# Stability-AI/stable-audio-tools

Hardware: AMD Instinct MI355X
Metric: train-step samples/sec (47s@44.1kHz) (higher is better)
Workload: dtype f32(bf16x3)

## Files before the change

### include/sat_amd.h

```cpp
#ifndef SAT_AMD_H
#define SAT_AMD_H

#ifdef __cplusplus
extern "C" {
#endif

int sat_abi_version(void);
int sat_is_simulator(void);
const char* sat_last_error(void);


int sat_conv1d(const float* x, const float* w_packed, const float* bias, const float* alpha, const float* beta,
               const float* res, float* y, const float* x2, const float* alpha2, const float* beta2,
               float* part_da, float* part_db, int B, int Cin, int Cout, int Tin, int Tout, int K, int stride,
               int dil, int pad, int tanh_out, void* stream);
int sat_conv1d_partial_rows(int B, int Tout);

int sat_conv1d_bf16x3(const float* x, const short* w_hi, const short* w_lo, const float* bias, const float* snake_a,
                      const float* snake_ib, const float* res, float* y, const float* x2, const float* alpha2,
                      const float* beta2, float* part_da, float* part_db, int B, int Cin, int Cout, int Tin, int Tout,
                      int K, int stride, int dil, int pad, int tanh_out, void* stream);
int sat_conv1d_bf16x3_emit(const float* x, const short* w_hi, const short* w_lo, const float* bias, const float* snake_a,
                      const float* snake_ib, const float* res, float* y, const float* x2, const float* alpha2,
                      const float* beta2, float* part_da, float* part_db, int B, int Cin, int Cout, int Tin, int Tout,
                      int K, int stride, int dil, int pad, int tanh_out, void* em_hi, void* em_lo,
                           const float* em_a, const float* em_ib, int em_rows, void* stream);
int sat_residual_unit_fwd(const short* xp_hi, const short* xp_lo, int rows, const short* w7_hi, const short* w7_lo,
                          const float* bias1, const float* a2, const float* ib2, const short* w1_hi, const short* w1_lo,
                          const float* bias2, const float* x, float* h, float* y, int B, int C, int T, int K, int dil, int pad,
                          void* em_hi, void* em_lo, const float* em_a, const float* em_ib, int em_rows, void* stream);
int sat_convtr1d_bf16x3(const float* x, const short* w_hi, const short* w_lo, const float* bias, const float* snake_a,
                        const float* snake_ib, const float* res, float* y, const float* x2, const float* alpha2,
                        const float* beta2, float* part_da, float* part_db, int B, int Cin, int Cout, int Tin, int Tout,
                        int K, int stride, int pad, int tanh_out, void* stream);
int sat_conv1d_bf16x3_partial_rows(int B, int Tout, int K, int stride);

int sat_rows_pack(const float* x, float* buf, int B, int C, int T, int W, int kh, int dil_t, int pad_t, int pad_w, int pitch, int lead,
                  void* stream);
int sat_rows_pack_bwd(const float* dbuf, float* dx, int B, int C, int T, int W, int kh, int dil_t, int pad_t, int pad_w, int pitch,
                      int lead, void* stream);
int sat_rows_unpack(const float* y, float* out, int B, int C, int T, int W, int pad_w, int pitch, float slope, void* stream);
int sat_rows_unpack_bwd(const float* dout, const float* out, float* dy, int B, int C, int T, int W, int pad_w, int pitch, float slope,
                        void* stream);

int sat_disc_geom(int frames, int W, int* P, int* L, int* lead, int* rows);
int sat_disc_planes(const float* src, const float* out, const signed char* fm_sign, const float* fm_coef, float* dst, void* hi, void* lo, int B,
                    int C, int frames, int W, int pitched, float slope, void* stream);
int sat_disc_l1_blocks(void);
int sat_disc_l1_sum(const float* a, const float* b, float* partial, signed char* sign, long long n, void* stream);
long long sat_disc_pack_size(int Cout, int Cin, int kh, int kw, int mode);
int sat_disc_pack_weights(const float* w, short* wq, int Cout, int Cin, int kh, int kw, int mode, void* stream);
int sat_disc_conv(const void* xp_hi, const void* xp_lo, const void* wq, const float* bias, float* y, void* em_hi,
                  void* em_lo, int B, int Cin, int Cout, int frames, int W, int kh, int kw, int dil_t, float slope, const float* lk_src,
                  float lk_slope, void* stream);
int sat_disc_wgrad_nsplit(int B, int M, int Cin, int kh, int frames, int W);
int sat_disc_wgrad(const float* dy, const float* x, float* partial, int B, int M, int Cin, int frames, int W, int kh, int kw, int dil_t,
                   void* stream);

int sat_conv1d_k7_plane_rows(int Tin, int Tout, int pad);
int sat_conv1d_k7_planes(const float* x, const float* snake_a, const float* snake_ib, short* xp_hi, short* xp_lo, int B, int Cin, int Tin,
                         int rows, void* stream);
long long sat_pack_weights_k7q_size(int D0, int D1, int K, int mode);
int sat_pack_weights_k7q(const float* w, short* hi, short* lo, int D0, int D1, int K, int mode, void* stream);
int sat_conv1d_bf16x3_planesq(const short* xp_hi, const short* xp_lo, int rows, const short* w_hi, const short* w_lo, const float* bias,
                             const float* res, float* y, const float* x2, const float* alpha2, const float* beta2, float* part_da,
                             float* part_db, int B, int Cin, int Cout, int Tin, int Tout, int K, int dil, int pad, int tanh_out,
                             int flags, void* stream);
int sat_convtr1d_bf16x3_partial_rows(int B, int Tout, int stride, int pad);
int sat_pack_weights_bf16x3(const float* w, short* hi, short* lo, int D0, int D1, int K, int stride, int mode, void* stream);
long long sat_pack_weights_bf16x3_size(int D0, int D1, int K, int stride, int mode);
int sat_snake_consts(const float* alpha, const float* beta, float* a, float* ib, int C, void* stream);

int sat_convtr1d(const float* x, const float* w_packed, const float* bias, const float* alpha, const float* beta,
                 const float* res, float* y, const float* x2, const float* alpha2, const float* beta2,
                 float* part_da, float* part_db, int B, int Cin, int Cout, int Tin, int Tout, int K, int stride,
                 int pad, int tanh_out, void* stream);
int sat_convtr1d_partial_rows(int B, int Tout, int stride, int pad);

int sat_conv_wgrad(const float* lo, const float* hi, const float* alpha, const float* beta, int snake_on,
                   float* partial, long long so_m, long long so_n, long long so_k, int B, int M, int N, int Tlo,
                   int Thi, int K, int stride, int dil, int pad, void* stream);
int sat_conv_wgrad_nsplit(int B, int M, int N, int Tlo, int K, int stride, int dil);

int sat_conv_wgrad7_bf16x3(const float* dy, const float* x, const float* alpha, const float* beta, float* partial,
                           long long so_m, long long so_n, long long so_k, int B, int M, int N, int T, int dil, int pad,
                           float* dy_rowsum, void* stream);
int sat_conv_wgrad7_bf16x3_nsplit(int B, int M, int N, int T);
int sat_conv_wgrad7_bf16x3_fuses_rowsum(int B, int M, int N, int T);

int sat_conv_wgrad7_planes_ok(int B, int M, int N, int T, int dil, int pad, int rows_dy, int rows_act);
int sat_conv_wgrad7_planes_nsplit(int B, int M, int N, int T);
int sat_conv_wgrad7_planes(const short* dy_hi, const short* dy_lo, int rows_dy, const short* act_hi, const short* act_lo, int rows_act,
                           float* partial, long long so_m, long long so_n, long long so_k, int B, int M, int N, int T, int dil, int pad,
                           void* stream);
int sat_lds_read_tr16_probe(const short* image, const int* lane_off, short* out, void* stream);

int sat_conv_wgrad_bf16x3(const float* lo, const float* hi, const float* alpha, const float* beta, int snake_on,
                          float* partial, long long so_m, long long so_n, long long so_k, int B, int M, int N, int Tlo,
                          int Thi, int K, int stride, int pad, float* lo_rowsum, void* stream);
int sat_conv_wgrad_bf16x3_nsplit(int B, int M, int N, int Tlo, int K, int stride);

int sat_ru_k1_bwd_nsplit(int B, int C, int T);
int sat_ru_k1_pack(const float* w, short* hi, short* lo, int C, void* stream);
int sat_ru_k1_bwd(const float* dy, const float* h, const short* wt_hi, const short* wt_lo, const float* alpha2, const float* beta2,
                  float* dh, short* em_hi, short* em_lo, int em_rows, float* dw_partial, float* part, int B, int C, int T,
                  void* stream);

int sat_reduce_splits(const float* partial, float* out, long long count, int nsplit, float scale, int accumulate,
                      void* stream);
int sat_rowsum(const float* x, float* partial, int B, int C, int T, void* stream);
int sat_rowsum_nsplit(int T);

int sat_wn_fold(const float* v, const float* g, float* w, float* norm, int D0, int R, void* stream);
int sat_wn_grad(const float* v, const float* g, const float* norm, const float* dw, float* dv, float* dg, int D0,
                int R, void* stream);
int sat_wn_grad_splits(const float* partial, int nsplit, long long count, long long so_m, long long so_n, long long so_k,
                       const float* v, const float* g, const float* norm, float* dv, float* dg, int D0, int N, int K,
                       const float* bias_partial, int bias_cols, float* dbias, void* stream);
int sat_edge_conv_ok(int cin, int cout, int k, int stride, int dil, int pad);
int sat_edge_conv_partial_rows(int B, int T);
int sat_edge_conv(const float* x, const float* w, const float* bias, const float* alpha, const float* beta, float* y, const float* x2,
                  const float* alpha2, const float* beta2, float* part_da, float* part_db, short* em_hi, short* em_lo,
                  const float* em_alpha, const float* em_beta, int em_rows, int B, int Cin, int Cout, int T, int K, int pad, int mode,
                  int tanh_out, void* stream);
int sat_edge_conv_wgrad_nsplit(int B, int M, int N, int T);
int sat_edge_conv_wgrad(const float* dy, const float* x, const float* alpha, const float* beta, float* partial, float* rowsum, int B,
                        int M, int N, int T, int K, int pad, void* stream);
int sat_pack_weights(const float* w, float* out, int D0, int D1, int K, int S, int mode, void* stream);

int sat_vae_nblocks(long long n);
int sat_vae_sample_fwd(const float* pre, const float* noise, float* z, float* kl_partial, int B, int C, int T,
                       void* stream);
int sat_vae_sample_bwd(const float* pre, const float* noise, const float* dz, const float* dkl, float* dpre, int B,
                       int C, int T, void* stream);

int sat_fir(const float* x, const float* taps, float* y, int N, int T, int ntaps, int adjoint, void* stream);
int sat_stft_tiles(int n_fft, int hop, int T);
int sat_stft_fwd(const float* x, const float* y, const float* views, float* partial, int NI, int C, int T, int NV,
                 int n_fft, int hop, void* stream);
int sat_stft_bwd(const float* x, const float* y, const float* views, const float* coef, float* dy, int NI, int C,
                 int T, int NV, int n_fft, int hop, int wrt_x, void* stream);

int sat_adamw_step(float* p, const float* g, float* m, float* v, long long n, float lr, float beta1, float beta2,
                   float eps, float weight_decay, int step, float grad_scale, float* ema, float ema_decay,
                   void* stream);
int sat_adamw_step_dev(float* p, const float* g, float* m, float* v, long long n, const float* hyper, float beta1, float beta2,
                       float eps, float weight_decay, float* ema, void* stream);

int sat_multi_copy(const void* entries, int nent, void* stream);

int sat_allreduce_available(void);
int sat_allreduce_unique_id(void* id128);
int sat_allreduce_init(const void* id128, int world, int rank, void** comm);
int sat_allreduce_bucket(void* comm, void* buf, long long count, int dtype, int mode, void* stream);
int sat_allreduce_finalize(void* comm);

int sat_attn_prepare(const void* src, long long sb, long long sh, long long sn, short* rm_hi, short* rm_lo,
                     short* tr_hi, short* tr_lo, int B, int H, int N, int Np, int dtype, void* stream);
int sat_attention_fwd(const short* q_hi, const short* q_lo, const short* k_hi, const short* k_lo, const short* vt_hi,
                      const short* vt_lo, void* o, float* lse, int B, int H, int Hkv, int Nq, int Nk, int Nqp, int Nkp,
                      int head_dim, float scale, int dtype, void* stream);
int sat_attention_rowdot(const void* dout, const void* out, float* dsum, int B, int H, int Nq, int dtype, void* stream);
int sat_attention_bwd(const short* const* planes, const float* lse, const float* dsum, void* dq, void* dk, void* dv,
                      int B, int H, int Hkv, int Nq, int Nk, int Nqp, int Nkp, int head_dim, float scale, int dtype,
                      void* stream);
int sat_attention_cross_ok(int H, int Hkv, int Nk, int head_dim, int dtype);
int sat_attention_cross_fwd(const short* q_rm, const short* k_rm, const short* v_tr, void* o, float* lse, int B, int H, int Hkv,
                            int Nq, int Nk, int Nqp, int Nkp, int head_dim, float scale, void* stream);
long long sat_attention_cross_bwd_ws(int B, int H, int Hkv, int Nq, int Nk);
int sat_attention_cross_bwd(const short* const* planes, const float* lse, const float* dsum, void* dq, void* dk, void* dv,
                            void* ws, long long ws_bytes, int B, int H, int Hkv, int Nq, int Nk, int Nqp, int Nkp, int head_dim,
                            float scale, void* stream);

int sat_layernorm_fwd(const void* x, const float* gamma, const float* beta, const void* scale, const void* shift,
                      long long mod_stride, void* y, float* mean, float* rstd, int rows, int D, int rows_per_batch,
                      float eps, int dtype, void* stream);
int sat_layernorm_fwd_fp8(const void* x, const float* gamma, const float* beta, const void* scale, const void* shift,
                          long long mod_stride, void* q, float* qscale, int rows, int D, int rows_per_batch, float eps,
                          int dtype, void* stream);
int sat_layernorm_bwd_nblocks(int rows, int rows_per_batch);
int sat_layernorm_bwd(const void* dy, const void* x, const float* gamma, const float* beta, const void* scale,
                      long long mod_stride, const float* mean, const float* rstd, void* dx, float* part, int rows, int D,
                      int rows_per_batch, int dtype, void* stream);
int sat_layernorm_bwd_res(const void* dy, const void* x, const float* gamma, const float* beta, const void* scale,
                          long long mod_stride, const float* mean, const float* rstd, const void* dres, void* dx, float* part,
                          int rows, int D, int rows_per_batch, int dtype, void* stream);

int sat_rope_tables(const float* inv_freq, float* cs, int N, int half, float pos_scale, void* stream);
int sat_rope_apply(void* t, const float* cs, long long sb, long long sn, long long sh, int B, int N, int H, int half,
                   int tab_off, int transpose, int dtype, void* stream);

int sat_qk_norm_fwd(const void* x, long long xs, void* y, long long ys, const float* q_gamma, const float* q_beta,
                    const float* k_gamma, const float* k_beta, const float* cs, int tab_off, float* stat, int tokens, int ntok,
                    int nh, int hq, int mode, float eps, int dtype, void* stream);
int sat_qk_norm_bwd_nblocks(long long rows);
int sat_qk_norm_bwd(void* dy, long long ys, const void* x, long long xs, const float* q_gamma, const float* k_gamma,
                    const float* cs, int tab_off, const float* stat, float* part, int tokens, int ntok, int nh, int hq,
                    int mode, int dtype, void* stream);

int sat_swiglu(const void* xin, const void* dout, void* out, long long rows, int F, int backward, int dtype,
               void* stream);
int sat_gate_residual(const void* x, const void* gate, long long gstride, const void* res, void* y, int B, int N, int D,
                      int dtype, void* stream);
int sat_gate_residual_bwd_nchunks(int N);
int sat_gate_residual_bwd(const void* dy, const void* x, const void* gate, long long gstride, void* dx, float* part,
                          int B, int N, int D, int dtype, void* stream);

int sat_cfg_step(const void* out2, const void* x, void* y0, void* y1, int B, int C, int T, int ncond, float scale,
                 float phi, float c0x, float c0v, float c1x, float c1v, int dtype, void* stream);
int sat_sampler_step(const void* out2, const void* x, const void* prev, void* y0, void* y1, int B, int C, int T, int ncond,
                     float scale, float phi, const float* coef, int dtype, void* stream);
int sat_sampler_step_dev(const void* out2, const void* x, const void* prev, void* y0, void* y1, int B, int C, int T, int ncond,
                         float scale, float phi, const float* coef, int dtype, void* stream);
int sat_spec_frames(int n_fft, int hop, int T);
int sat_spec_fwd(const float* x, float* z, int NI, int C, int T, int n_fft, int hop, void* stream);
int sat_spec_bwd(const float* dz, float* dx, int NI, int C, int T, int n_fft, int hop, void* stream);


int sat_gemm_bf16(const void* A, long long lda, const void* B, long long ldb, void* C, long long ldc, const float* bias,
                  const void* res, long long ldr, const void* gate, long long ldg, int rows_per_gate, void* pre,
                  long long ldp, const void* zeros, int M, int N, int K, int epilogue, int out_f32, int splits, int tile,
                  void* stream);

int sat_gemm_qkv_bf16(const void* A, long long lda, const void* B, long long ldb, const float* rope_cs, int rope_off,
                      void* q_rm, void* k_rm, void* v_tr, const void* zeros, int nb, int ntok, int npad, int heads,
                      int K, int sec0, int nsec, int tile, void* stream);
int sat_gemm_qkv_norm_bf16(const void* A, long long lda, const void* B, long long ldb, const float* rope_cs, int rope_off,
                           void* q_rm, void* k_rm, void* v_tr, const void* zeros, int nb, int ntok, int npad, int heads,
                           int K, int sec0, int nsec, int tile, int mode, const float* q_gamma, const float* q_beta,
                           const float* k_gamma, const float* k_beta, float eps, void* stream);

int sat_splitk_epilogue(const float* slabs, int S, const float* bias, const void* res, long long ldr, void* out, long long ldo,
                        int M, int N, int out_f32, void* stream);

int sat_gemm_fp8(const void* A, long long lda, const void* B, long long ldb, void* C, long long ldc, const float* bias,
                 const void* res, long long ldr, const void* gate, long long ldg, int rows_per_gate, void* pre,
                 long long ldp, const void* zeros, const float* alpha, const float* row_alpha, const float* col_alpha, int M, int N,
                 int K, int epilogue, int out_f32, int tile, void* stream);
int sat_gemm_qkv_fp8(const void* A, long long lda, const void* B, long long ldb, const float* rope_cs, int rope_off,
                     void* q_rm, void* k_rm, void* v_tr, const void* zeros, const float* alpha, const float* row_alpha,
                     const float* col_alpha, int nb, int ntok, int npad, int heads, int K, int sec0, int nsec, int tile, void* stream);
int sat_absmax_scale_blocks(int R, int C);
int sat_absmax_scale(const void* src, long long lds, float* work, float* scales, int R, int C, int src_f32, void* stream);
int sat_quant_fp8(const void* src, long long lds, void* dst, long long ldd, const float* qscale, int R, int C, int src_f32,
                  void* stream);
int sat_quant_fp8_rows(const void* src, long long lds, void* dst, long long ldd, float* scale, int R, int C, int src_f32,
                       void* stream);

int sat_cast_bf16(const void* src, long long lds, void* dst, long long ldd, int R, int C, int Rpad, int src_f32,
                  int transpose, void* stream);
int sat_cast_bf16_tpair(const void* src_a, long long lds_a, void* dst_a, long long ldd_a, int Ra, int Ca, int Rpad_a, int a_f32,
                        const void* src_b, long long lds_b, void* dst_b, long long ldd_b, int Rb, int Cb, int Rpad_b, int b_f32,
                        void* stream);
int sat_cast_bf16_dual(const void* src, long long lds, void* dst, long long ldd, void* dst_t, long long ldd_t, int R, int C, int Rpad,
                       int src_f32, void* stream);

int sat_split_bf16x3(const float* src, long long lds, void* dst, long long ldd, int R, int C, int side, void* stream);

#ifdef __cplusplus
}
#endif
#endif
```

### stable_audio_tools_amd/_lib.py

```python
import ctypes
import os

_P = ctypes.c_void_p
_I = ctypes.c_int
_L = ctypes.c_longlong
_F = ctypes.c_float

SIGNATURES = {
    "sat_abi_version": (_I, []),
    "sat_is_simulator": (_I, []),
    "sat_last_error": (ctypes.c_char_p, []),
    "sat_conv1d": (_I, [_P] * 12 + [_I] * 10 + [_P]),
    "sat_conv1d_partial_rows": (_I, [_I, _I]),
    "sat_conv1d_bf16x3": (_I, [_P] * 13 + [_I] * 10 + [_P]),
    "sat_conv1d_bf16x3_emit": (_I, [_P] * 13 + [_I] * 10 + [_P] * 4 + [_I, _P]),
    "sat_convtr1d_bf16x3": (_I, [_P] * 13 + [_I] * 9 + [_P]),
    "sat_conv1d_bf16x3_partial_rows": (_I, [_I] * 4),
    "sat_rows_pack": (_I, [_P, _P] + [_I] * 10 + [_P]),
    "sat_rows_pack_bwd": (_I, [_P, _P] + [_I] * 10 + [_P]),
    "sat_rows_unpack": (_I, [_P, _P] + [_I] * 6 + [_F, _P]),
    "sat_rows_unpack_bwd": (_I, [_P, _P, _P] + [_I] * 6 + [_F, _P]),
    "sat_disc_geom": (_I, [_I, _I, _P, _P, _P, _P]),
    "sat_disc_planes": (_I, [_P] * 7 + [_I] * 5 + [_F, _P]),
    "sat_disc_l1_blocks": (_I, []),
    "sat_disc_l1_sum": (_I, [_P, _P, _P, _P, _L, _P]),
    "sat_disc_pack_size": (_L, [_I] * 5),
    "sat_disc_pack_weights": (_I, [_P] * 2 + [_I] * 5 + [_P]),
    "sat_disc_conv": (_I, [_P] * 7 + [_I] * 8 + [_F, _P, _F, _P]),
    "sat_disc_wgrad_nsplit": (_I, [_I] * 6),
    "sat_disc_wgrad": (_I, [_P] * 3 + [_I] * 8 + [_P]),
    "sat_conv1d_k7_plane_rows": (_I, [_I] * 3),
    "sat_conv1d_k7_planes": (_I, [_P] * 5 + [_I] * 4 + [_P]),
    "sat_conv1d_bf16x3_planesq": (_I, [_P, _P, _I] + [_P] * 10 + [_I] * 10 + [_P]),
    "sat_pack_weights_k7q": (_I, [_P, _P, _P, _I, _I, _I, _I, _P]),
    "sat_residual_unit_fwd": (_I, [_P, _P, _I] + [_P] * 11 + [_I] * 6 + [_P] * 4 + [_I, _P]),
    "sat_pack_weights_k7q_size": (_L, [_I, _I, _I, _I]),
    "sat_convtr1d_bf16x3_partial_rows": (_I, [_I] * 4),
    "sat_pack_weights_bf16x3": (_I, [_P, _P, _P, _I, _I, _I, _I, _I, _P]),
    "sat_pack_weights_bf16x3_size": (_L, [_I, _I, _I, _I, _I]),
    "sat_snake_consts": (_I, [_P, _P, _P, _P, _I, _P]),
    "sat_conv_wgrad7_bf16x3": (_I, [_P] * 5 + [_L] * 3 + [_I] * 6 + [_P, _P]),
    "sat_conv_wgrad7_bf16x3_nsplit": (_I, [_I] * 4),
    "sat_conv_wgrad7_bf16x3_fuses_rowsum": (_I, [_I] * 4),
    "sat_conv_wgrad7_planes_ok": (_I, [_I] * 8),
    "sat_conv_wgrad7_planes_nsplit": (_I, [_I] * 4),
    "sat_conv_wgrad7_planes": (_I, [_P, _P, _I, _P, _P, _I, _P] + [_L] * 3 + [_I] * 6 + [_P]),
    "sat_lds_read_tr16_probe": (_I, [_P] * 4),
    "sat_conv_wgrad_bf16x3": (_I, [_P] * 4 + [_I, _P] + [_L] * 3 + [_I] * 8 + [_P, _P]),
    "sat_conv_wgrad_bf16x3_nsplit": (_I, [_I] * 6),
    "sat_convtr1d": (_I, [_P] * 12 + [_I] * 9 + [_P]),
    "sat_convtr1d_partial_rows": (_I, [_I, _I, _I, _I]),
    "sat_conv_wgrad": (_I, [_P, _P, _P, _P, _I, _P, _L, _L, _L] + [_I] * 9 + [_P]),
    "sat_conv_wgrad_nsplit": (_I, [_I] * 7),
    "sat_reduce_splits": (_I, [_P, _P, _L, _I, _F, _I, _P]),
    "sat_ru_k1_bwd_nsplit": (_I, [_I] * 3),
    "sat_ru_k1_pack": (_I, [_P, _P, _P, _I, _P]),
    "sat_ru_k1_bwd": (_I, [_P] * 9 + [_I, _P, _P, _I, _I, _I, _P]),
    "sat_rowsum": (_I, [_P, _P, _I, _I, _I, _P]),
    "sat_rowsum_nsplit": (_I, [_I]),
    "sat_wn_fold": (_I, [_P, _P, _P, _P, _I, _I, _P]),
    "sat_wn_grad": (_I, [_P, _P, _P, _P, _P, _P, _I, _I, _P]),
    "sat_wn_grad_splits": (_I, [_P, _I, _L, _L, _L, _L, _P, _P, _P, _P, _P, _I, _I, _I, _P, _I, _P, _P]),
    "sat_pack_weights": (_I, [_P, _P, _I, _I, _I, _I, _I, _P]),
    "sat_vae_nblocks": (_I, [_L]),
    "sat_vae_sample_fwd": (_I, [_P, _P, _P, _P, _I, _I, _I, _P]),
    "sat_vae_sample_bwd": (_I, [_P, _P, _P, _P, _P, _I, _I, _I, _P]),
    "sat_multi_copy": (_I, [_P, _I, _P]),
    "sat_adamw_step": (_I, [_P, _P, _P, _P, _L, _F, _F, _F, _F, _F, _I, _F, _P, _F, _P]),
    "sat_adamw_step_dev": (_I, [_P, _P, _P, _P, _L, _P, _F, _F, _F, _F, _P, _P]),
    "sat_allreduce_available": (_I, []),
    "sat_allreduce_unique_id": (_I, [_P]),
    "sat_allreduce_init": (_I, [_P, _I, _I, _P]),
    "sat_allreduce_bucket": (_I, [_P, _P, _L, _I, _I, _P]),
    "sat_allreduce_finalize": (_I, [_P]),
    "sat_fir": (_I, [_P, _P, _P, _I, _I, _I, _I, _P]),
    "sat_stft_tiles": (_I, [_I, _I, _I]),
    "sat_stft_fwd": (_I, [_P, _P, _P, _P, _I, _I, _I, _I, _I, _I, _P]),
    "sat_stft_bwd": (_I, [_P, _P, _P, _P, _P, _I, _I, _I, _I, _I, _I, _I, _P]),
    "sat_spec_frames": (_I, [_I, _I, _I]),
    "sat_spec_fwd": (_I, [_P, _P, _I, _I, _I, _I, _I, _P]),
    "sat_spec_bwd": (_I, [_P, _P, _I, _I, _I, _I, _I, _P]),
    "sat_attn_prepare": (_I, [_P, _L, _L, _L, _P, _P, _P, _P, _I, _I, _I, _I, _I, _P]),
    "sat_attention_fwd": (_I, [_P] * 8 + [_I] * 8 + [_F, _I, _P]),
    "sat_attention_rowdot": (_I, [_P, _P, _P, _I, _I, _I, _I, _P]),
    "sat_attention_bwd": (_I, [_P] * 6 + [_I] * 8 + [_F, _I, _P]),
    "sat_edge_conv_ok": (_I, [_I] * 6),
    "sat_edge_conv_partial_rows": (_I, [_I] * 2),
    "sat_edge_conv": (_I, [_P] * 15 + [_I] * 9 + [_P]),
    "sat_edge_conv_wgrad_nsplit": (_I, [_I] * 4),
    "sat_edge_conv_wgrad": (_I, [_P] * 6 + [_I] * 6 + [_P]),
    "sat_attention_cross_ok": (_I, [_I] * 5),
    "sat_attention_cross_fwd": (_I, [_P] * 5 + [_I] * 8 + [_F, _P]),
    "sat_attention_cross_bwd_ws": (_L, [_I] * 5),
    "sat_attention_cross_bwd": (_I, [_P] * 7 + [_L] + [_I] * 8 + [_F, _P]),
    "sat_gemm_bf16": (_I, [_P, _L, _P, _L, _P, _L, _P, _P, _L, _P, _L, _I, _P, _L, _P] + [_I] * 7 + [_P]),
    "sat_gemm_qkv_bf16": (_I, [_P, _L, _P, _L, _P, _I, _P, _P, _P, _P] + [_I] * 8 + [_P]),
    "sat_gemm_qkv_norm_bf16": (_I, [_P, _L, _P, _L, _P, _I, _P, _P, _P, _P] + [_I] * 9 + [_P] * 4 + [_F, _P]),
    "sat_gemm_fp8": (_I, [_P, _L, _P, _L, _P, _L, _P, _P, _L, _P, _L, _I, _P, _L, _P, _P, _P, _P] + [_I] * 6 + [_P]),
    "sat_gemm_qkv_fp8": (_I, [_P, _L, _P, _L, _P, _I, _P, _P, _P, _P, _P, _P, _P] + [_I] * 8 + [_P]),
    "sat_quant_fp8": (_I, [_P, _L, _P, _L, _P, _I, _I, _I, _P]),
    "sat_quant_fp8_rows": (_I, [_P, _L, _P, _L, _P, _I, _I, _I, _P]),
    "sat_absmax_scale": (_I, [_P, _L, _P, _P, _I, _I, _I, _P]),
    "sat_absmax_scale_blocks": (_I, [_I, _I]),
    "sat_splitk_epilogue": (_I, [_P, _I, _P, _P, _L, _P, _L, _I, _I, _I, _P]),
    "sat_cast_bf16": (_I, [_P, _L, _P, _L, _I, _I, _I, _I, _I, _P]),
    "sat_cast_bf16_tpair": (_I, [_P, _L, _P, _L, _I, _I, _I, _I, _P, _L, _P, _L, _I, _I, _I, _I, _P]),
    "sat_cast_bf16_dual": (_I, [_P, _L, _P, _L, _P, _L, _I, _I, _I, _I, _P]),
    "sat_split_bf16x3": (_I, [_P, _L, _P, _L, _I, _I, _I, _P]),
    "sat_layernorm_fwd": (_I, [_P] * 5 + [_L] + [_P] * 3 + [_I] * 3 + [_F, _I, _P]),
    "sat_layernorm_fwd_fp8": (_I, [_P] * 5 + [_L] + [_P] * 2 + [_I] * 3 + [_F, _I, _P]),
    "sat_layernorm_bwd_nblocks": (_I, [_I, _I]),
    "sat_layernorm_bwd": (_I, [_P] * 5 + [_L] + [_P] * 4 + [_I] * 4 + [_P]),
    "sat_layernorm_bwd_res": (_I, [_P] * 5 + [_L] + [_P] * 5 + [_I] * 4 + [_P]),
    "sat_rope_tables": (_I, [_P, _P, _I, _I, _F, _P]),
    "sat_rope_apply": (_I, [_P, _P, _L, _L, _L] + [_I] * 7 + [_P]),
    "sat_qk_norm_fwd": (_I, [_P, _L, _P, _L, _P, _P, _P, _P, _P, _I, _P] + [_I] * 5 + [_F, _I, _P]),
    "sat_qk_norm_bwd_nblocks": (_I, [_L]),
    "sat_qk_norm_bwd": (_I, [_P, _L, _P, _L, _P, _P, _P, _I, _P, _P] + [_I] * 6 + [_P]),
    "sat_swiglu": (_I, [_P, _P, _P, _L, _I, _I, _I, _P]),
    "sat_gate_residual": (_I, [_P, _P, _L, _P, _P, _I, _I, _I, _I, _P]),
    "sat_gate_residual_bwd_nchunks": (_I, [_I]),
    "sat_cfg_step": (_I, [_P, _P, _P, _P, _I, _I, _I, _I, _F, _F, _F, _F, _F, _F, _I, _P]),
    "sat_sampler_step": (_I, [_P, _P, _P, _P, _P, _I, _I, _I, _I, _F, _F, _P, _I, _P]),
    "sat_sampler_step_dev": (_I, [_P, _P, _P, _P, _P, _I, _I, _I, _I, _F, _F, _P, _I, _P]),
    "sat_gate_residual_bwd": (_I, [_P, _P, _P, _L, _P, _P, _I, _I, _I, _I, _P]),
}

LIB_PATH = os.path.join(os.path.dirname(os.path.abspath(__file__)), "csrc", "libsat_amd.so")


def bind(cdll):
    for name, (res, args) in SIGNATURES.items():
        fn = getattr(cdll, name)
        fn.restype = res
        fn.argtypes = args
    return cdll


_lib = None


def load():
    global _lib
    if _lib is not None:
        return _lib
    if not os.path.exists(LIB_PATH):
        raise RuntimeError(
            f"stable_audio_tools_amd: HIP library not built: {LIB_PATH} is missing. "
            "Run `python -c 'import __graft_entry__ as g; g.build()'` (hipcc --offload-arch=gfx950). "
            "There is no CPU fallback.")
    try:
        cdll = ctypes.CDLL(LIB_PATH)
    except OSError as e:
        raise RuntimeError(f"stable_audio_tools_amd: cannot load {LIB_PATH}: {e}. There is no CPU fallback.") from e
    bind(cdll)
    if cdll.sat_is_simulator():
        raise RuntimeError("stable_audio_tools_amd: refusing to use a simulator build as the product library")
    _lib = cdll
    return _lib
```

### stable_audio_tools_amd/csrc/conv1d_bf16x3.hip

```cpp
#include "conv_common.h"
#include <type_traits>

#define SAT_K7P_LEAD_ROWS 32
#define SAT_BF_AROWS1 192
#define SAT_BF_AROWSN 136

struct SatConvBfLaunch {
    SatConvParams p;
    const short* w_hi;
    const short* w_lo;
    int cout_pad;
    int cin_v, cout_v;
    int sin_log2;
    int sout_log2;
    int in_shift, out_shift;
    int nq;
    const short* xp_hi = nullptr;
    const short* xp_lo = nullptr;
    int xp_rows = 0, xp_c8 = 0;
    int wq = 0;
    int stagger = 0;
    int persist = 0;
    int dma_in_mfma = 0;
    short* em_hi = nullptr;
    short* em_lo = nullptr;
    const float* em_a = nullptr;
    const float* em_ib = nullptr;
    int em_rows = 0, em_c8 = 0;
    const short* ru_w1_hi = nullptr;
    const short* ru_w1_lo = nullptr;
    const float* ru_bias2 = nullptr;
    const float* ru_a2 = nullptr;
    const float* ru_ib2 = nullptr;
    float* ru_h = nullptr;
};

SAT_DEVICE void sat_split2(float x, short* hi, short* lo) {
    const short h = sat_f32_to_bf16(x);
    *hi = h;
    *lo = sat_f32_to_bf16(x - sat_bf16_to_f32(h));
}

template <int NG, int CS, bool GATHER>
__global__ void __launch_bounds__(256)
#if !defined(SAT_HIPEMU)
__attribute__((amdgpu_waves_per_eu(NG == 4 ? 3 : 2)))
#endif
sat_conv1d_bf16x3_kernel(SatConvBfLaunch a) {
    constexpr int KT = NG / CS;
    constexpr int KROW = NG * 8 + 8;
    constexpr int AROWS = (CS == 1) ? SAT_BF_AROWS1 : SAT_BF_AROWSN;
    constexpr int WPS = 4 / CS;
    constexpr int NU = (CS == 1) ? 1 : 128 / (64 * WPS);
    const SatConvParams& p = a.p;
    constexpr int W_BYTES = 2 * SAT_CO_T * KROW * 2, A_BYTES = 2 * CS * AROWS * 8 * 2, T_BYTES = 4 * 32 * 68 * 4;
    constexpr int POOL = (W_BYTES + A_BYTES) > T_BYTES ? (W_BYTES + A_BYTES) : T_BYTES;
    __shared__ __attribute__((aligned(16))) char lds_pool[POOL];
    short (*w_lds)[SAT_CO_T][KROW] = reinterpret_cast<short (*)[SAT_CO_T][KROW]>(lds_pool);
    short (*a_lds)[CS][AROWS][8] = reinterpret_cast<short (*)[CS][AROWS][8]>(lds_pool + W_BYTES);
    __shared__ float red_lds[2][2][SAT_CO_T];
    __shared__ float ep_lds[5][SAT_CO_T];
    constexpr int SN_MAX = (NG == 4) ? 1024 : 2048;
    __shared__ float sn_lds[2][SN_MAX];

    const int tid = threadIdx.x;
    const int lane = tid & 63, wave = tid >> 6;
    const int l31 = lane & 31, hi = lane >> 5;
    int co_tile, win;
    sat_xcd_tile(blockIdx.x + gridDim.x * (blockIdx.y + gridDim.y * blockIdx.z), gridDim.y, gridDim.x * gridDim.z, &co_tile, &win);
    const int b = win / (int)gridDim.x, t_tile = win - b * (int)gridDim.x;
    const int t0 = t_tile * SAT_T_T;
    const int co0 = co_tile * SAT_CO_T;
    const int co_w = (wave >> 1) * 64, t_w = (wave & 1) * 64;
    const int K = p.K, dil = p.dil;
    const int nrows = SAT_T_T + (K - 1) * dil;
    const int q_in0 = t0 - p.pad;
    const int si = GATHER ? a.sin_log2 : 0, so = a.sout_log2;
    const int smask_i = (1 << si) - 1, smask_o = (1 << so) - 1;
    const float* xb = p.x + (size_t)b * p.Cin * p.Tin;
    const bool wave_on = (co0 + co_w) < a.cout_v;
    const bool mi1_on = (co0 + co_w + 32) < a.cout_v;
    const bool has_snake = p.alpha != nullptr;

    f32x16 acc[2][2];
#pragma unroll
    for (int i = 0; i < 2; ++i)
#pragma unroll
        for (int j = 0; j < 2; ++j)
#pragma unroll
            for (int r = 0; r < 16; ++r) acc[i][j][r] = 0.0f;

    if (tid < SAT_CO_T) {
        const int m = co0 + tid;
        const bool ok = m < a.cout_v;
        const int co = m >> so;
        ep_lds[0][tid] = (ok && p.bias) ? p.bias[co] : 0.0f;
        ep_lds[1][tid] = (ok && p.x2) ? expf(p.alpha2[co]) : 1.0f;
        ep_lds[2][tid] = (ok && p.x2) ? expf(p.beta2[co]) : 1.0f;
        ep_lds[3][tid] = (ok && a.em_a) ? a.em_a[co] : 0.0f;
        ep_lds[4][tid] = (ok && a.em_a) ? a.em_ib[co] : 0.0f;
    }
    if (has_snake) {
        const int nsn = p.Cin < SN_MAX ? p.Cin : SN_MAX;
        for (int i = tid; i < nsn; i += 256) {
            sn_lds[0][i] = p.alpha[i];
            sn_lds[1][i] = p.beta[i];
        }
    }
    __syncthreads();

    const int nchunks = (a.cin_v + 8 * CS - 1) / (8 * CS);
    const int cs_w = SAT_UNIFORM(wave / WPS);
    const int row0 = (wave % WPS) * 64 + lane;
    const int nhalo = (CS > 1) ? (nrows - SAT_T_T) * 8 : 0;
    const bool halo_on = (CS > 1) && (wave % WPS) == 0 && lane < nhalo;
    const int h_row = SAT_T_T + (lane >> 3), h_e = lane & 7;
    constexpr bool DEEP = (NG == 8 && CS == 4);
    constexpr int NSET = DEEP ? 2 : 1;
    float av[NSET][NU][8];
    float hv[NSET];
    bf16x8 wv[NG];
#pragma unroll
    for (int s_ = 0; s_ < NSET; ++s_) hv[s_] = 0.0f;
    auto load_elem = [&](int v, int row, bool* okp) -> float {
        int ch = v >> si;
        ch = ch < p.Cin ? ch : p.Cin - 1;
        const int tin = ((q_in0 + row) << si) + (v & smask_i) - (GATHER ? a.in_shift : 0);
        const bool ok = (unsigned)tin < (unsigned)p.Tin;
        *okp = ok;
        return xb[(size_t)ch * p.Tin + (ok ? tin : 0)];
    };
    unsigned okm[NSET];
#pragma unroll
    for (int s_ = 0; s_ < NSET; ++s_) okm[s_] = 0u;
    auto issue_loads = [&](int c, auto set_c) {
        constexpr int ST = decltype(set_c)::value;
        const int v0 = (c * CS + cs_w) * 8;
        unsigned m = 0u;
#pragma unroll
        for (int u = 0; u < NU; ++u) {
            const int row = row0 + u * 64 * WPS;
            if (CS == 1 && row >= nrows) continue;
#pragma unroll
            for (int e = 0; e < 8; ++e) {
                bool ok;
                av[ST][u][e] = load_elem(v0 + e, row, &ok);
                m |= ok ? (1u << (u * 8 + e)) : 0u;
            }
        }
        static_assert(NU * 8 < 31, "the in-range flags of a staging set are one 32-bit mask (bit 31: the halo element)");
        if (CS > 1 && halo_on) {
            bool ok;
            hv[ST] = load_elem(v0 + h_e, h_row, &ok);
            m |= ok ? (1u << 31) : 0u;
        }
        okm[ST] = m;
    };
    auto issue_w = [&](int c) {
#pragma unroll
        for (int u = 0; u < NG; ++u) {
            const int idx = tid + u * 256;
            const int part = idx % NG, co = (idx / NG) & 127, pl = idx / (NG * 128);
            const short* src = (pl ? a.w_lo : a.w_hi) + (((size_t)c * a.cout_pad + co0 + co) * NG + part) * 8;
            wv[u] = *reinterpret_cast<const bf16x8*>(src);
        }
    };
    auto write_lds = [&](int c, auto set_c) {
        constexpr int ST = decltype(set_c)::value;
        const int v0 = (c * CS + cs_w) * 8;
        float sa[8], sib[8];
        if (has_snake) {
#pragma unroll
            for (int e = 0; e < 8; ++e) {
                int ch = (v0 + e) >> si;
                ch = ch < p.Cin ? ch : p.Cin - 1;
                sa[e] = sn_lds[0][ch];
                sib[e] = sn_lds[1][ch];
            }
        }
#pragma unroll
        for (int u = 0; u < NU; ++u) {
            const int row = row0 + u * 64 * WPS;
            if (CS == 1 && row >= nrows) continue;
            uint32_t ph[4], pl[4];
#pragma unroll
            for (int e = 0; e < 8; e += 2) {
                float o0 = (okm[ST] >> (u * 8 + e)) & 1u ? av[ST][u][e] : 0.0f, o1 = (okm[ST] >> (u * 8 + e + 1)) & 1u ? av[ST][u][e + 1] : 0.0f;
                if (has_snake) {
                    o0 = sat_snake(o0, sa[e], sib[e]);
                    o1 = sat_snake(o1, sa[e + 1], sib[e + 1]);
                }
                sat_split2_pk(o0, o1, &ph[e >> 1], &pl[e >> 1]);
            }
            *reinterpret_cast<u32x4*>(&a_lds[0][cs_w][row][0]) = u32x4{ph[0], ph[1], ph[2], ph[3]};
            *reinterpret_cast<u32x4*>(&a_lds[1][cs_w][row][0]) = u32x4{pl[0], pl[1], pl[2], pl[3]};
        }
        if (CS > 1 && halo_on) {
            float o = (okm[ST] >> 31) & 1u ? hv[ST] : 0.0f;
            if (has_snake) {
                int ch = (v0 + h_e) >> si;
                ch = ch < p.Cin ? ch : p.Cin - 1;
                o = sat_snake(o, sn_lds[0][ch], sn_lds[1][ch]);
            }
            short h, l;
            sat_split2(o, &h, &l);
            a_lds[0][cs_w][h_row][h_e] = h;
            a_lds[1][cs_w][h_row][h_e] = l;
        }
#pragma unroll
        for (int u = 0; u < NG; ++u) {
            const int idx = tid + u * 256;
            const int part = idx % NG, co = (idx / NG) & 127, pl = idx / (NG * 128);
            *reinterpret_cast<bf16x8*>(&w_lds[pl][co][part * 8]) = wv[u];
        }
    };
    auto mfma_chunk = [&]() {
        if (wave_on) {
            SAT_MFMA_PRIO(1);
#pragma unroll
            for (int ks = 0; ks < NG / 2; ++ks) {
                const int g = 2 * ks + hi;
                const int cs = g / KT;
                int tap = g - cs * KT;
                if (tap >= K) tap = K - 1;
                bf16x8 wa[2][2], xa[2][2];
#pragma unroll
                for (int pl = 0; pl < 2; ++pl) {
                    wa[0][pl] = *reinterpret_cast<const bf16x8*>(&w_lds[pl][co_w + l31][g * 8]);
                    wa[1][pl] = *reinterpret_cast<const bf16x8*>(&w_lds[pl][co_w + 32 + l31][g * 8]);
                    xa[0][pl] = *reinterpret_cast<const bf16x8*>(&a_lds[pl][cs][t_w + l31 + tap * dil][0]);
                    xa[1][pl] = *reinterpret_cast<const bf16x8*>(&a_lds[pl][cs][t_w + 32 + l31 + tap * dil][0]);
                }
#pragma unroll
                for (int mi = 0; mi < 2; ++mi) {
                    if (mi == 1 && !mi1_on) break;
#pragma unroll
                    for (int ni = 0; ni < 2; ++ni) {
                        acc[mi][ni] = sat_mfma_32x32x16_bf16(wa[mi][0], xa[ni][0], acc[mi][ni]);
                        acc[mi][ni] = sat_mfma_32x32x16_bf16(wa[mi][0], xa[ni][1], acc[mi][ni]);
                        acc[mi][ni] = sat_mfma_32x32x16_bf16(wa[mi][1], xa[ni][0], acc[mi][ni]);
                    }
                }
            }
            SAT_MFMA_PRIO(0);
        }
    };
    using SatSet0 = std::integral_constant<int, 0>;
    using SatSet1 = std::integral_constant<int, NSET - 1>;
    issue_loads(0, SatSet0{});
    issue_w(0);
    if constexpr (DEEP) {
        if (nchunks > 1) issue_loads(1, SatSet1{});
        for (int c = 0; c < nchunks; c += 2) {
            write_lds(c, SatSet0{});
            __syncthreads();
            if (c + 1 < nchunks) issue_w(c + 1);
            SAT_SCHED_FENCE();
            if (c + 2 < nchunks) issue_loads(c + 2, SatSet0{});
            SAT_SCHED_FENCE();
            mfma_chunk();
            __syncthreads();
            if (c + 1 < nchunks) {
                write_lds(c + 1, SatSet1{});
                __syncthreads();
                if (c + 2 < nchunks) issue_w(c + 2);
                SAT_SCHED_FENCE();
                if (c + 3 < nchunks) issue_loads(c + 3, SatSet1{});
                SAT_SCHED_FENCE();
                mfma_chunk();
                __syncthreads();
            }
        }
    } else {
        for (int c = 0; c < nchunks; ++c) {
            write_lds(c, SatSet0{});
            __syncthreads();
            if (c + 1 < nchunks) {
                issue_loads(c + 1, SatSet0{});
                issue_w(c + 1);
            }
            mfma_chunk();
            __syncthreads();
        }
    }

    const bool bwd = (p.x2 != nullptr);
    if (bwd) {
        for (int i = tid; i < 2 * 2 * SAT_CO_T; i += 256) (&red_lds[0][0][0])[i] = 0.0f;
        __syncthreads();
    }
    const bool vec4 = so == 0 && a.out_shift == 0 && (p.Tout & 3) == 0 &&
                      (((uintptr_t)p.y | (uintptr_t)p.x2 | (uintptr_t)p.res) & 15) == 0;
    if (vec4) {
        if (!bwd) __syncthreads();
        float (*tile)[68] = reinterpret_cast<float (*)[68]>(lds_pool) + wave * 32;
        const int lr = lane >> 4, t4 = (lane & 15) * 4;
#pragma unroll
        for (int mi = 0; mi < 2; ++mi) {
            const bool half_on = wave_on && (mi == 0 || mi1_on);
            if (mi == 1) __syncthreads();
            if (half_on) {
#pragma unroll
                for (int ni = 0; ni < 2; ++ni)
#pragma unroll
                    for (int r = 0; r < 16; ++r) tile[(r & 3) + 8 * (r >> 2) + 4 * hi][ni * 32 + l31] = acc[mi][ni][r];
            }
            __syncthreads();
            if (half_on) {
                const int tg = t0 + t_w + t4;
                f32x4 xv[8], rv[8];
                if (co0 + SAT_CO_T <= p.Cout && t0 + SAT_T_T <= p.Tout) {
                    const size_t o0 = ((size_t)b * p.Cout + co0 + co_w + mi * 32 + lr) * p.Tout + tg;
#pragma unroll
                    for (int j = 0; j < 8; ++j) {
                        xv[j] = f32x4{0.f, 0.f, 0.f, 0.f};
                        rv[j] = f32x4{0.f, 0.f, 0.f, 0.f};
                        if (bwd) xv[j] = *reinterpret_cast<const f32x4*>(p.x2 + o0 + (size_t)(j * 4) * p.Tout);
                        if (p.res) rv[j] = *reinterpret_cast<const f32x4*>(p.res + o0 + (size_t)(j * 4) * p.Tout);
                    }
                } else
#pragma unroll
                for (int j = 0; j < 8; ++j) {
                    const int co = co0 + co_w + mi * 32 + j * 4 + lr;
                    const bool ok = co < p.Cout && tg < p.Tout;
                    const size_t o = ((size_t)b * p.Cout + (ok ? co : 0)) * p.Tout + (ok ? tg : 0);
                    xv[j] = (bwd && ok) ? *reinterpret_cast<const f32x4*>(p.x2 + o) : f32x4{0.f, 0.f, 0.f, 0.f};
                    rv[j] = (p.res && ok) ? *reinterpret_cast<const f32x4*>(p.res + o) : f32x4{0.f, 0.f, 0.f, 0.f};
                }
#pragma unroll
                for (int j = 0; j < 8; ++j) {
                    const int row = j * 4 + lr;
                    const int col = co_w + mi * 32 + row;
                    const int co = co0 + col;
                    const bool ok = co < p.Cout && tg < p.Tout;
                    const f32x4 av = *reinterpret_cast<const f32x4*>(&tile[row][t4]);
                    const float bias = ep_lds[0][col];
                    const float a2 = ep_lds[1][col], b2 = ep_lds[2][col];
                    float pda = 0.f, pdb = 0.f;
                    f32x4 ov;
#pragma unroll
                    for (int e = 0; e < 4; ++e) {
                        float v = av[e] + bias;
                        if (bwd) {
                            const SatSnakeGrad g = sat_snake_grad(xv[j][e], a2, b2);
                            pda += v * g.dla;
                            pdb += v * g.dlb;
                            v *= g.dx;
                        }
                        v += rv[j][e];
                        if (p.tanh_out) v = tanhf(v);
                        ov[e] = v;
                    }
                    if (ok) *reinterpret_cast<f32x4*>(p.y + ((size_t)b * p.Cout + co) * p.Tout + tg) = ov;
                    if (a.em_hi) {
                        f32x4 ev = ov;
                        if (a.em_a) {
                            const float ea = ep_lds[3][col], eib = ep_lds[4][col];
#pragma unroll
                            for (int e = 0; e < 4; ++e) ev[e] = sat_snake(ov[e], ea, eib);
                        }
                        if (!ok) ev = f32x4{0.f, 0.f, 0.f, 0.f};
                        *reinterpret_cast<f32x4*>(&tile[row][t4]) = ev;
                    }
                    if (bwd) {
                        if (!ok) { pda = 0.f; pdb = 0.f; }
#pragma unroll
                        for (int m = 8; m >= 1; m >>= 1) {
                            pda += __shfl_xor(pda, m);
                            pdb += __shfl_xor(pdb, m);
                        }
                        if ((lane & 15) == 0) {
                            red_lds[0][wave & 1][col] = pda;
                            red_lds[1][wave & 1][col] = pdb;
                        }
                    }
                }
                if (a.em_hi) {
                    sat_wave_sync();
#pragma unroll
                    for (int it = 0; it < 4; ++it) {
                        const int tt = lane, g = it;
                        const int c8i = ((co0 + co_w + mi * 32) >> 3) + g;
                        const int tq = t0 + t_w + tt;
                        float v8[8];
#pragma unroll
                        for (int e = 0; e < 8; ++e) v8[e] = tile[g * 8 + e][tt];
                        uint32_t h[4], l[4];
#pragma unroll
                        for (int e = 0; e < 4; ++e) sat_split2_pk(v8[2 * e], v8[2 * e + 1], &h[e], &l[e]);
                        if (c8i < a.em_c8 && tq < p.Tout) {
                            const size_t o = (((size_t)b * a.em_c8 + c8i) * a.em_rows + SAT_K7P_LEAD_ROWS + tq) * 8;
                            *reinterpret_cast<u32x4*>(a.em_hi + o) = u32x4{h[0], h[1], h[2], h[3]};
                            *reinterpret_cast<u32x4*>(a.em_lo + o) = u32x4{l[0], l[1], l[2], l[3]};
                        }
                    }
                }
            }
        }
    } else
    if (wave_on && so >= 1 && ((t0 << so) - a.out_shift) >= 0 && (((t0 + SAT_T_T - 1) << so) + smask_o - a.out_shift) < p.Tout) {
        auto ep_vec = [&](auto lg_c) {
            constexpr int GL = 1 << decltype(lg_c)::value, NGP = 4 / GL;
            typedef float vecu __attribute__((ext_vector_type(GL), aligned(4)));
#pragma unroll
            for (int mi = 0; mi < 2; ++mi) {
                if (mi == 1 && !mi1_on) break;
                vecu xv[4][NGP][2], rv[4][NGP][2];
#pragma unroll
                for (int rg = 0; rg < 4; ++rg)
#pragma unroll
                    for (int gp = 0; gp < NGP; ++gp) {
                        const int m = co0 + co_w + mi * 32 + 8 * rg + 4 * hi + gp * GL;
                        const bool m_ok = m < a.cout_v;
                        const int co = m_ok ? m >> so : 0;
#pragma unroll
                        for (int ni = 0; ni < 2; ++ni) {
                            const int q = t0 + t_w + ni * 32 + l31;
                            const size_t o = ((size_t)b * p.Cout + co) * p.Tout + ((q << so) + (m & smask_o) - a.out_shift);
#pragma unroll
                            for (int e = 0; e < GL; ++e) { xv[rg][gp][ni][e] = 0.0f; rv[rg][gp][ni][e] = 0.0f; }
                            if (bwd) xv[rg][gp][ni] = *reinterpret_cast<const vecu*>(p.x2 + o);
                            if (p.res) rv[rg][gp][ni] = *reinterpret_cast<const vecu*>(p.res + o);
                        }
                    }
#pragma unroll
                for (int rg = 0; rg < 4; ++rg)
#pragma unroll
                    for (int gp = 0; gp < NGP; ++gp) {
                        const int col0 = co_w + mi * 32 + 8 * rg + 4 * hi + gp * GL;
                        const int m = co0 + col0;
                        const bool m_ok = m < a.cout_v;
                        const int co = m_ok ? m >> so : 0;
                        float pda[GL], pdb[GL];
#pragma unroll
                        for (int e = 0; e < GL; ++e) { pda[e] = 0.f; pdb[e] = 0.f; }
#pragma unroll
                        for (int ni = 0; ni < 2; ++ni) {
                            const int q = t0 + t_w + ni * 32 + l31;
                            vecu ov;
#pragma unroll
                            for (int e = 0; e < GL; ++e) {
                                const int col = col0 + e;
                                float v = acc[mi][ni][rg * 4 + gp * GL + e] + ep_lds[0][col];
                                if (bwd) {
                                    const SatSnakeGrad g = sat_snake_grad(xv[rg][gp][ni][e], ep_lds[1][col], ep_lds[2][col]);
                                    pda[e] += v * g.dla;
                                    pdb[e] += v * g.dlb;
                                    v *= g.dx;
                                }
                                v += rv[rg][gp][ni][e];
                                if (p.tanh_out) v = tanhf(v);
                                ov[e] = v;
                            }
                            if (m_ok) *reinterpret_cast<vecu*>(p.y + ((size_t)b * p.Cout + co) * p.Tout + ((q << so) + (m & smask_o) - a.out_shift)) = ov;
                        }
                        if (bwd) {
#pragma unroll
                            for (int e = 0; e < GL; ++e) {
                                const float sa_ = sat_half_sum(m_ok ? pda[e] : 0.f), sb_ = sat_half_sum(m_ok ? pdb[e] : 0.f);
                                if (l31 == 0) {
                                    red_lds[0][wave & 1][col0 + e] = sa_;
                                    red_lds[1][wave & 1][col0 + e] = sb_;
                                }
                            }
                        }
                    }
            }
        };
        if (so >= 2) ep_vec(std::integral_constant<int, 2>{});
        else ep_vec(std::integral_constant<int, 1>{});
    } else
    if (wave_on) {
#pragma unroll
        for (int mi = 0; mi < 2; ++mi) {
            if (mi == 1 && !mi1_on) break;
            float xv[16][2], rv[16][2];
            unsigned okb = 0u;
#pragma unroll
            for (int r = 0; r < 16; ++r) {
                const int col = co_w + mi * 32 + (r & 3) + 8 * (r >> 2) + 4 * hi;
                const int m = co0 + col;
                const bool m_ok = m < a.cout_v;
                const int co = m >> so;
#pragma unroll
                for (int ni = 0; ni < 2; ++ni) {
                    const int q = t0 + t_w + ni * 32 + l31;
                    const int t = (q << so) + (m & smask_o) - a.out_shift;
                    const bool ok = m_ok && t >= 0 && t < p.Tout;
                    okb |= ok ? (1u << (2 * r + ni)) : 0u;
                    const size_t o = ((size_t)b * p.Cout + (ok ? co : 0)) * p.Tout + (ok ? t : 0);
                    xv[r][ni] = bwd ? p.x2[o] : 0.0f;
                    rv[r][ni] = p.res ? p.res[o] : 0.0f;
                }
            }
#pragma unroll
            for (int r = 0; r < 16; ++r) {
                const int col = co_w + mi * 32 + (r & 3) + 8 * (r >> 2) + 4 * hi;
                const int m = co0 + col;
                const int co = m >> so;
                const float bias = ep_lds[0][col];
                const float a2 = ep_lds[1][col], b2 = ep_lds[2][col];
                float pda = 0.f, pdb = 0.f;
#pragma unroll
                for (int ni = 0; ni < 2; ++ni) {
                    const int q = t0 + t_w + ni * 32 + l31;
                    const int t = (q << so) + (m & smask_o) - a.out_shift;
                    const bool ok = (okb >> (2 * r + ni)) & 1u;
                    float v = acc[mi][ni][r] + bias;
                    if (bwd) {
                        const SatSnakeGrad g = sat_snake_grad(xv[r][ni], a2, b2);
                        pda += ok ? v * g.dla : 0.0f;
                        pdb += ok ? v * g.dlb : 0.0f;
                        v *= g.dx;
                    }
                    v += rv[r][ni];
                    if (p.tanh_out) v = tanhf(v);
                    if (ok) p.y[((size_t)b * p.Cout + co) * p.Tout + t] = v;
                }
                if (bwd) {
                    pda = sat_half_sum(pda);
                    pdb = sat_half_sum(pdb);
                    if (l31 == 0) {
                        red_lds[0][wave & 1][col] = pda;
                        red_lds[1][wave & 1][col] = pdb;
                    }
                }
            }
        }
    }
    if (bwd) {
        __syncthreads();
        const int m = co0 + tid;
        if (tid < SAT_CO_T && (tid & smask_o) == 0 && m < a.cout_v) {
            float sa = 0.f, sb = 0.f;
            for (int r = 0; r <= smask_o; ++r) {
                sa += red_lds[0][0][tid + r] + red_lds[0][1][tid + r];
                sb += red_lds[1][0][tid + r] + red_lds[1][1][tid + r];
            }
            const size_t row = (size_t)b * gridDim.x + t_tile;
            const size_t nrows_p = (size_t)p.B * gridDim.x;
            p.part_da[(size_t)(m >> so) * nrows_p + row] = sa;
            p.part_db[(size_t)(m >> so) * nrows_p + row] = sb;
        }
    }
}

struct SatBfPlan { int ng, cs, kv; };
static bool sat_bf_plan(int K, int stride, int mode, SatBfPlan* pl) {
    if (mode == 2 || stride > 1) {
        if (K != 2 * stride || (stride & (stride - 1)) || stride > 64) return false;
        *pl = SatBfPlan{8, 4, 2};
        return true;
    }
    if (stride != 1 || K < 1 || K > 8) return false;
    if (K == 1) *pl = SatBfPlan{4, 4, 1};
    else if (K == 2) *pl = SatBfPlan{8, 4, K};
    else if (K <= 4) *pl = SatBfPlan{8, 2, K};
    else *pl = SatBfPlan{8, 1, K};
    return true;
}
static int sat_log2i(int s) { int l = 0; while ((1 << l) < s) ++l; return l; }

struct SatPackBfParams {
    const float* w;
    short* hi;
    short* lo;
    int D0, D1, K, S, mode, ng, cs, kv, m_v, v_v, out_pad;
    long long total;
};
__global__ void __launch_bounds__(256) sat_pack_bf16x3_kernel(SatPackBfParams p) {
    const long long o = (long long)blockIdx.x * 256 + threadIdx.x;
    if (o >= p.total) return;
    const int e = (int)(o & 7);
    long long q = o >> 3;
    const int g = (int)(q % p.ng);
    q /= p.ng;
    const int m = (int)(q % p.out_pad), chunk = (int)(q / p.out_pad);
    const int kt = p.ng / p.cs;
    const int v = (chunk * p.cs + g / kt) * 8 + e, tap = g % kt;
    float val = 0.0f;
    if (tap < p.kv && m < p.m_v && v < p.v_v) {
        if (p.mode == 0) val = p.w[((size_t)m * p.D1 + v / p.S) * p.K + tap * p.S + v % p.S];
        else if (p.mode == 1) val = p.w[((size_t)v * p.D1 + m) * p.K + (p.K - 1 - tap)];
        else val = p.w[((size_t)v * p.D1 + m / p.S) * p.K + (m % p.S) + (tap == 0 ? p.S : 0)];
    }
    short h, l;
    sat_split2(val, &h, &l);
    p.hi[o] = h;
    p.lo[o] = l;
}

static bool sat_pack_bf_geometry(int D0, int D1, int K, int stride, int mode, SatPackBfParams* p) {
    SatBfPlan pl;
    if (mode < 0 || mode > 2 || D0 <= 0 || D1 <= 0 || !sat_bf_plan(K, stride, mode, &pl)) return false;
    if (mode == 1 && stride != 1) return false;
    p->D0 = D0; p->D1 = D1; p->K = K; p->S = stride; p->mode = mode;
    p->ng = pl.ng; p->cs = pl.cs; p->kv = pl.kv;
    if (mode == 0) { p->m_v = D0; p->v_v = D1 * stride; }
    else if (mode == 1) { p->m_v = D1; p->v_v = D0; }
    else { p->m_v = D1 * stride; p->v_v = D0; }
    p->out_pad = sat_cdiv(p->m_v, SAT_CO_T) * SAT_CO_T;
    p->total = (long long)sat_cdiv(p->v_v, 8 * pl.cs) * p->out_pad * pl.ng * 8;
    return true;
}
extern "C" long long sat_pack_weights_bf16x3_size(int D0, int D1, int K, int stride, int mode) {
    SatPackBfParams p{};
    return sat_pack_bf_geometry(D0, D1, K, stride, mode, &p) ? p.total : -1;
}
extern "C" int sat_pack_weights_bf16x3(const float* w, short* hi, short* lo, int D0, int D1, int K, int stride, int mode, void* stream) {
    SatPackBfParams p{};
    if (!sat_pack_bf_geometry(D0, D1, K, stride, mode, &p)) {
        sat_set_error("sat_pack_weights_bf16x3: needs stride 1 with K <= 8, or K == 2*stride with a power-of-two stride; mode 0|1|2");
        return 1;
    }
    p.w = w; p.hi = hi; p.lo = lo;
    SAT_LAUNCH(sat_pack_bf16x3_kernel, dim3((unsigned)sat_cdivll(p.total, 256)), dim3(256), stream, p);
    return sat_check_launch("sat_pack_weights_bf16x3");
}

struct SatSnakeConstParams { const float* alpha; const float* beta; float* a; float* ib; int C; };
__global__ void __launch_bounds__(256) sat_snake_consts_kernel(SatSnakeConstParams p) {
    const int i = blockIdx.x * 256 + threadIdx.x;
    if (i >= p.C) return;
    p.a[i] = expf(p.alpha[i]);
    p.ib[i] = 1.0f / (expf(p.beta[i]) + 1e-9f);
}
extern "C" int sat_snake_consts(const float* alpha, const float* beta, float* a, float* ib, int C, void* stream) {
    if (C <= 0) { sat_set_error("sat_snake_consts: empty"); return 1; }
    SatSnakeConstParams p{alpha, beta, a, ib, C};
    SAT_LAUNCH(sat_snake_consts_kernel, dim3(sat_cdiv(C, 256)), dim3(256), stream, p);
    return sat_check_launch("sat_snake_consts");
}

#include "conv1d_bf16x3_k7.h"
#include "conv1d_planes.h"
#include "conv1d_bf16x3_k7q.h"

static int sat_bf_launch(const char* what, SatConvBfLaunch& a, const SatBfPlan& pl, void* stream) {
    if (pl.ng == 8 && pl.cs == 1 && a.sin_log2 == 0 && a.sout_log2 == 0) {
        if (a.xp_hi && a.wq) sat_bf_launch_k7q(a, stream);
        else sat_bf_launch_k7(a, stream);
        return sat_check_launch(what);
    }
    if (a.p.alpha && a.p.Cin > ((pl.ng == 4) ? 1024 : 2048)) {
        sat_set_error("conv1d_bf16x3: an activated input of more than 2048 channels (1024 for K <= 4 at stride 1) is not served by the bf16x3 kernels (ops.use_bf16x3 = False takes the fp32-MFMA ones)");
        return 1;
    }
    dim3 grid(sat_cdiv(a.nq, SAT_T_T), a.cout_pad / SAT_CO_T, a.p.B);
    if (a.sin_log2 > 0) { SAT_LAUNCH((sat_conv1d_bf16x3_kernel<8, 4, true>), grid, dim3(256), stream, a); }
    else if (pl.ng == 8 && pl.cs == 1) { SAT_LAUNCH((sat_conv1d_bf16x3_kernel<8, 1, false>), grid, dim3(256), stream, a); }
    else if (pl.ng == 8 && pl.cs == 2) { SAT_LAUNCH((sat_conv1d_bf16x3_kernel<8, 2, false>), grid, dim3(256), stream, a); }
    else if (pl.ng == 8 && pl.cs == 4) { SAT_LAUNCH((sat_conv1d_bf16x3_kernel<8, 4, false>), grid, dim3(256), stream, a); }
    else { SAT_LAUNCH((sat_conv1d_bf16x3_kernel<4, 4, false>), grid, dim3(256), stream, a); }
    return sat_check_launch(what);
}

static int sat_conv1d_bf16x3_impl(const char* what, const float* x, const short* w_hi, const short* w_lo, const float* bias,
                                  const float* snake_a, const float* snake_ib, const float* res, float* y,
                                  const float* x2, const float* alpha2, const float* beta2, float* part_da,
                                  float* part_db, int B, int Cin, int Cout, int Tin, int Tout, int K, int stride, int dil,
                                  int pad, int tanh_out, short* em_hi, short* em_lo, const float* em_a, const float* em_ib, int em_rows,
                                  void* stream) {
    if (B <= 0 || Cin <= 0 || Cout <= 0 || Tin <= 0 || Tout <= 0) { sat_set_error("sat_conv1d_bf16x3: empty shape"); return 1; }
    SatBfPlan pl;
    if (!sat_bf_plan(K, stride, 0, &pl) || dil < 1 || (stride > 1 && dil != 1)) {
        sat_set_error("sat_conv1d_bf16x3: needs stride 1 with K <= 8, or K == 2*stride (power-of-two stride, dilation 1)");
        return 1;
    }
    if ((pl.kv - 1) * dil > (pl.cs == 1 ? 62 : SAT_BF_AROWSN - SAT_T_T)) { sat_set_error("sat_conv1d_bf16x3: receptive field too large for the LDS slab"); return 1; }
    if ((snake_a == nullptr) != (snake_ib == nullptr)) { sat_set_error("sat_conv1d_bf16x3: snake constants must both be given"); return 1; }
    if (x2 && (!alpha2 || !beta2 || !part_da || !part_db)) { sat_set_error("sat_conv1d_bf16x3: backward epilogue needs alpha2/beta2/partials"); return 1; }
    SatConvBfLaunch a;
    a.p = SatConvParams{x, nullptr, bias, snake_a, snake_ib, res, y, x2, alpha2, beta2, part_da, part_db,
                        B, Cin, Cout, Tin, Tout, pl.kv, 1, dil, stride == 1 ? pad : 0, tanh_out};
    a.w_hi = w_hi;
    a.w_lo = w_lo;
    a.cout_v = Cout;
    a.cout_pad = sat_cdiv(Cout, SAT_CO_T) * SAT_CO_T;
    a.cin_v = Cin * stride;
    a.sin_log2 = sat_log2i(stride);
    a.sout_log2 = 0;
    a.in_shift = stride == 1 ? 0 : pad;
    a.out_shift = 0;
    a.nq = Tout;
    if (em_hi) {
        const bool generic = !(pl.ng == 8 && pl.cs == 1);
        const bool vec4 = (Tout & 3) == 0 && (((uintptr_t)y | (uintptr_t)x2 | (uintptr_t)res) & 15) == 0;
        if (!generic || !vec4 || !em_lo || (em_a == nullptr) != (em_ib == nullptr) || em_rows < SAT_K7P_LEAD_ROWS + Tout ||
            (((uintptr_t)em_hi | (uintptr_t)em_lo) & 15)) {
            sat_set_error("sat_conv1d_bf16x3_emit: emission needs K <= 4 or a strided conv, Tout % 4 == 0, 16-byte aligned tensors, rows >= 32 + Tout");
            return 1;
        }
        a.em_hi = em_hi; a.em_lo = em_lo; a.em_a = em_a; a.em_ib = em_ib; a.em_rows = em_rows; a.em_c8 = sat_cdiv(Cout, 8);
    }
    return sat_bf_launch(what, a, pl, stream);
}
extern "C" int sat_conv1d_bf16x3(const float* x, const short* w_hi, const short* w_lo, const float* bias,
                                 const float* snake_a, const float* snake_ib, const float* res, float* y,
                                 const float* x2, const float* alpha2, const float* beta2, float* part_da,
                                 float* part_db, int B, int Cin, int Cout, int Tin, int Tout, int K, int stride, int dil,
                                 int pad, int tanh_out, void* stream) {
    return sat_conv1d_bf16x3_impl("sat_conv1d_bf16x3", x, w_hi, w_lo, bias, snake_a, snake_ib, res, y, x2, alpha2, beta2, part_da, part_db,
                                  B, Cin, Cout, Tin, Tout, K, stride, dil, pad, tanh_out, nullptr, nullptr, nullptr, nullptr, 0, stream);
}
extern "C" int sat_conv1d_bf16x3_emit(const float* x, const short* w_hi, const short* w_lo, const float* bias,
                                      const float* snake_a, const float* snake_ib, const float* res, float* y,
                                      const float* x2, const float* alpha2, const float* beta2, float* part_da,
                                      float* part_db, int B, int Cin, int Cout, int Tin, int Tout, int K, int stride, int dil,
                                      int pad, int tanh_out, void* em_hi, void* em_lo, const float* em_a, const float* em_ib, int em_rows,
                                      void* stream) {
    if (!em_hi) { sat_set_error("sat_conv1d_bf16x3_emit: planes missing"); return 1; }
    return sat_conv1d_bf16x3_impl("sat_conv1d_bf16x3_emit", x, w_hi, w_lo, bias, snake_a, snake_ib, res, y, x2, alpha2, beta2, part_da, part_db,
                                  B, Cin, Cout, Tin, Tout, K, stride, dil, pad, tanh_out, (short*)em_hi, (short*)em_lo, em_a, em_ib, em_rows, stream);
}

extern "C" int sat_conv1d_k7_plane_rows(int Tin, int Tout, int pad) {
    if (Tin <= 0 || Tout <= 0 || pad < 0 || pad > SAT_K7P_LEAD) return -1;
    const int need = sat_cdiv(Tout, SAT_K7_T) * SAT_K7_T - pad + SAT_K7_AROWS;
    const int body = need > Tin ? need : Tin;
    return SAT_K7P_LEAD + sat_cdiv(body, 64) * 64;
}
extern "C" int sat_conv1d_k7_planes(const float* x, const float* snake_a, const float* snake_ib, short* xp_hi, short* xp_lo, int B,
                                    int Cin, int Tin, int rows, void* stream) {
    if (B <= 0 || Cin <= 0 || Tin <= 0 || rows < SAT_K7P_LEAD + Tin) { sat_set_error("sat_conv1d_k7_planes: bad shape"); return 1; }
    if ((snake_a == nullptr) != (snake_ib == nullptr)) { sat_set_error("sat_conv1d_k7_planes: snake constants must both be given"); return 1; }
    SatK7PlaneParams p{x, snake_a, snake_ib, xp_hi, xp_lo, B, Cin, Tin, rows, sat_cdiv(Cin, 8)};
    SAT_LAUNCH(sat_k7_planes_kernel, dim3(sat_cdiv(rows, 256), p.c8, B), dim3(256), stream, p);
    return sat_check_launch("sat_conv1d_k7_planes");
}
extern "C" int sat_conv1d_bf16x3_planesq(const short* xp_hi, const short* xp_lo, int rows, const short* w_hi, const short* w_lo,
                                         const float* bias, const float* res, float* y, const float* x2, const float* alpha2,
                                         const float* beta2, float* part_da, float* part_db, int B, int Cin, int Cout, int Tin, int Tout,
                                         int K, int dil, int pad, int tanh_out, int flags, void* stream) {
    if (B <= 0 || Cin <= 0 || Cout <= 0 || Tin <= 0 || Tout <= 0) { sat_set_error("sat_conv1d_bf16x3_planesq: empty shape"); return 1; }
    if (K < 5 || K > SAT_K7Q_TAPS || dil < 1 || (K - 1) * dil > 62) {
        sat_set_error("sat_conv1d_bf16x3_planesq: needs stride 1, 5 <= K <= 7, (K-1)*dil <= 62");
        return 1;
    }
    if (rows < sat_conv1d_k7_plane_rows(Tin, Tout, pad)) { sat_set_error("sat_conv1d_bf16x3_planesq: rows must be >= sat_conv1d_k7_plane_rows(Tin, Tout, pad)"); return 1; }
    if (x2 && (!alpha2 || !beta2 || !part_da || !part_db)) { sat_set_error("sat_conv1d_bf16x3_planesq: backward epilogue needs alpha2/beta2/partials"); return 1; }
    SatConvBfLaunch a;
    a.p = SatConvParams{nullptr, nullptr, bias, nullptr, nullptr, res, y, x2, alpha2, beta2, part_da, part_db,
                        B, Cin, Cout, Tin, Tout, K, 1, dil, pad, tanh_out};
    a.w_hi = w_hi;
    a.w_lo = w_lo;
    a.cout_v = Cout;
    a.cout_pad = sat_cdiv(Cout, SAT_CO_T) * SAT_CO_T;
    a.cin_v = Cin;
    a.sin_log2 = 0;
    a.sout_log2 = 0;
    a.in_shift = 0;
    a.out_shift = 0;
    a.nq = Tout;
    a.xp_hi = xp_hi;
    a.xp_lo = xp_lo;
    a.xp_rows = rows;
    a.xp_c8 = sat_cdiv(Cin, 8);
    a.wq = 1;
    a.dma_in_mfma = (flags & 4) ? 1 : 0;
    a.persist = (flags & 1) ? 0 : ((flags & 2) ? 2 : 1);
    SatBfPlan pl{8, 1, K};
    return sat_bf_launch("sat_conv1d_bf16x3_planesq", a, pl, stream);
}

extern "C" int sat_residual_unit_fwd(const short* xp_hi, const short* xp_lo, int rows, const short* w7_hi, const short* w7_lo,
                                     const float* bias1, const float* a2, const float* ib2, const short* w1_hi, const short* w1_lo,
                                     const float* bias2, const float* x, float* h, float* y, int B, int C, int T, int K, int dil, int pad,
                                     void* em_hi, void* em_lo, const float* em_a, const float* em_ib, int em_rows, void* stream) {
    if (B <= 0 || C <= 0 || T <= 0 || C > SAT_K7_CO) { sat_set_error("sat_residual_unit_fwd: needs 1 <= C <= 128"); return 1; }
    if (K < 5 || K > SAT_K7Q_TAPS || dil < 1 || (K - 1) * dil > 62 || 2 * pad != (K - 1) * dil) {
        sat_set_error("sat_residual_unit_fwd: needs 5 <= K <= 7, (K-1)*dil <= 62, 'same' padding");
        return 1;
    }
    if (rows < sat_conv1d_k7_plane_rows(T, T, pad)) { sat_set_error("sat_residual_unit_fwd: rows must be >= sat_conv1d_k7_plane_rows(T, T, pad)"); return 1; }
    if (!xp_hi || !xp_lo || !w7_hi || !w7_lo || !w1_hi || !w1_lo || !a2 || !ib2 || !x || !y) { sat_set_error("sat_residual_unit_fwd: missing operand"); return 1; }
    if ((T & 3) || (((uintptr_t)y | (uintptr_t)x) & 15)) { sat_set_error("sat_residual_unit_fwd: T % 4 == 0 and 16-byte aligned x / y"); return 1; }
    SatConvBfLaunch a;
    a.p = SatConvParams{nullptr, nullptr, bias1, nullptr, nullptr, x, y, nullptr, nullptr, nullptr, nullptr, nullptr,
                        B, C, C, T, T, K, 1, dil, pad, 0};
    a.w_hi = w7_hi;
    a.w_lo = w7_lo;
    a.cout_v = C;
    a.cout_pad = SAT_CO_T;
    a.cin_v = C;
    a.sin_log2 = 0; a.sout_log2 = 0; a.in_shift = 0; a.out_shift = 0;
    a.nq = T;
    a.xp_hi = xp_hi; a.xp_lo = xp_lo; a.xp_rows = rows; a.xp_c8 = sat_cdiv(C, 8);
    a.wq = 1;
    a.ru_w1_hi = w1_hi; a.ru_w1_lo = w1_lo; a.ru_bias2 = bias2; a.ru_a2 = a2; a.ru_ib2 = ib2; a.ru_h = h;
    if (em_hi) {
        if (!em_lo || (em_a == nullptr) != (em_ib == nullptr) || em_rows < SAT_K7P_LEAD_ROWS + T || (((uintptr_t)em_hi | (uintptr_t)em_lo) & 15)) {
            sat_set_error("sat_residual_unit_fwd: bad emission planes");
            return 1;
        }
        a.em_hi = (short*)em_hi; a.em_lo = (short*)em_lo; a.em_a = em_a; a.em_ib = em_ib; a.em_rows = em_rows; a.em_c8 = sat_cdiv(C, 8);
    }
    SatBfPlan pl{8, 1, K};
    return sat_bf_launch("sat_residual_unit_fwd", a, pl, stream);
}

extern "C" int sat_convtr1d_bf16x3(const float* x, const short* w_hi, const short* w_lo, const float* bias,
                                   const float* snake_a, const float* snake_ib, const float* res, float* y,
                                   const float* x2, const float* alpha2, const float* beta2, float* part_da,
                                   float* part_db, int B, int Cin, int Cout, int Tin, int Tout, int K, int stride,
                                   int pad, int tanh_out, void* stream) {
    if (B <= 0 || Cin <= 0 || Cout <= 0 || Tin <= 0 || Tout <= 0) { sat_set_error("sat_convtr1d_bf16x3: empty shape"); return 1; }
    SatBfPlan pl;
    if (!sat_bf_plan(K, stride, 2, &pl) || pad < 0) { sat_set_error("sat_convtr1d_bf16x3: needs K == 2*stride with a power-of-two stride"); return 1; }
    if ((snake_a == nullptr) != (snake_ib == nullptr)) { sat_set_error("sat_convtr1d_bf16x3: snake constants must both be given"); return 1; }
    if (x2 && (!alpha2 || !beta2 || !part_da || !part_db)) { sat_set_error("sat_convtr1d_bf16x3: backward epilogue needs alpha2/beta2/partials"); return 1; }
    SatConvBfLaunch a;
    a.p = SatConvParams{x, nullptr, bias, snake_a, snake_ib, res, y, x2, alpha2, beta2, part_da, part_db,
                        B, Cin, Cout, Tin, Tout, 2, 1, 1, 1, tanh_out};
    a.w_hi = w_hi;
    a.w_lo = w_lo;
    a.cout_v = Cout * stride;
    a.cout_pad = sat_cdiv(a.cout_v, SAT_CO_T) * SAT_CO_T;
    a.cin_v = Cin;
    a.sin_log2 = 0;
    a.sout_log2 = sat_log2i(stride);
    a.in_shift = 0;
    a.out_shift = pad;
    a.nq = sat_cdiv(Tout + pad, stride);
    return sat_bf_launch("sat_convtr1d_bf16x3", a, pl, stream);
}
extern "C" int sat_conv1d_bf16x3_partial_rows(int B, int Tout, int K, int stride) {
    SatBfPlan pl;
    if (B <= 0 || Tout <= 0 || !sat_bf_plan(K, stride, 0, &pl)) return -1;
    const bool k7 = pl.ng == 8 && pl.cs == 1 && stride == 1;
    return B * sat_cdiv(Tout, k7 ? SAT_K7_T : SAT_T_T);
}
extern "C" int sat_convtr1d_bf16x3_partial_rows(int B, int Tout, int stride, int pad) {
    if (B <= 0 || Tout <= 0 || stride < 1 || pad < 0) return -1;
    return B * sat_cdiv(sat_cdiv(Tout + pad, stride), SAT_T_T);
}
```

### stable_audio_tools_amd/csrc/conv_wgrad_bf16x3.hip

```cpp
#include "conv_common.h"
#include <type_traits>

#define SAT_WB_TT 64
#define SAT_WB_LOROW (SAT_WB_TT + 8)
#define SAT_WB_HIROW 136

struct SatWgBfParams {
    const float* dy;
    const float* x;
    const float* alpha;
    const float* beta;
    float* out;
    long long so_split, so_m, so_n, so_k;
    int B, M, N, T, pad;
    int chunks_per_split, nchunks, nT;
    float* rowsum;
    int nsplit;
};

SAT_DEVICE unsigned sat_umulhi(unsigned a, unsigned b) { return (unsigned)(((unsigned long long)a * b) >> 32); }
SAT_DEVICE float sat_row16_sum(float4 q) {
    float s = (q.x + q.y) + (q.z + q.w);
#pragma unroll
    for (int m = 1; m <= 8; m <<= 1) s += __shfl_xor(s, m);
// ... 24 lines not shown
    const int l31 = lane & 31, hi = lane >> 5;
    int mn_tile, split;
    sat_xcd_tile(blockIdx.x + gridDim.x * (blockIdx.y + gridDim.y * blockIdx.z), gridDim.x * gridDim.y, gridDim.z, &mn_tile, &split);
    const int m0 = (mn_tile % (int)gridDim.x) * SAT_CO_T, n0 = (mn_tile / (int)gridDim.x) * 32;
    const int m_w = wave * 32;
    const bool wave_on = (m0 + m_w) < p.M;

    f32x16 acc[7];
#pragma unroll
    for (int k = 0; k < 7; ++k)
#pragma unroll
        for (int r = 0; r < 16; ++r) acc[k][r] = 0.0f;

    const bool want_rs = p.rowsum != nullptr && n0 == 0;
    float rs[8] = {0.f, 0.f, 0.f, 0.f, 0.f, 0.f, 0.f, 0.f};

    if (tid < 32) {
        const int c = n0 + tid;
        float sa = 1.f, sib = 0.f;
        if (p.alpha && c < p.N) {
            sa = expf(p.alpha[c]);
            sib = 1.0f / (expf(p.beta[c]) + 1e-9f);
        }
        sn_a[tid] = sa;
        sn_ib[tid] = sib;
    }
    for (int i = tid; i < 2 * 32 * SAT_WB_HIROW; i += 256) (&hi_lds[0][0][0])[i] = 0;
    __syncthreads();

    const int c_begin = split * p.chunks_per_split;
    int c_end = c_begin + p.chunks_per_split;
    if (c_end > p.nchunks) c_end = p.nchunks;
    constexpr int HSPAN = SAT_WB_TT + 6 * DIL;

    for (int ch = c_begin; ch < c_end; ++ch) {
        const int b = ch / p.nT;
        const int tt0 = (ch - b * p.nT) * SAT_WB_TT;
        {
            const float* src = p.dy + (size_t)b * p.M * p.T;
            for (int half = 0; half < 2; ++half) {
            float4 v[4];
#pragma unroll
            for (int u = 0; u < 4; ++u) {
                const int idx = tid + (half * 4 + u) * 256;
                const int row = idx >> 4, c4 = (idx & 15) * 4;
                const int m = m0 + row, t = tt0 + c4;
                float4 q = make_float4(0.f, 0.f, 0.f, 0.f);
                if (m < p.M) {
                    const float* s = src + (size_t)m * p.T + t;
                    if (t + 3 < p.T && ((p.T & 3) == 0)) {
                        q = *reinterpret_cast<const float4*>(s);
                    } else {
                        if (t + 0 < p.T) q.x = s[0];
                        if (t + 1 < p.T) q.y = s[1];
                        if (t + 2 < p.T) q.z = s[2];
                        if (t + 3 < p.T) q.w = s[3];
                    }
                }
                v[u] = q;
            }
#pragma unroll
            for (int u = 0; u < 4; ++u) {
                const int idx = tid + (half * 4 + u) * 256;
                const int row = idx >> 4, c4 = (idx & 15) * 4;
                if (want_rs) rs[half * 4 + u] += sat_row16_sum(v[u]);
                uint32_t h0, h1, l0, l1;
                sat_split2_pk(v[u].x, v[u].y, &h0, &l0);
                sat_split2_pk(v[u].z, v[u].w, &h1, &l1);
                typedef uint32_t u2 __attribute__((ext_vector_type(2)));
                *reinterpret_cast<u2*>(&lo_lds[0][row][c4]) = u2{h0, h1};
                *reinterpret_cast<u2*>(&lo_lds[1][row][c4]) = u2{l0, l1};
            }
            }
        }
        {
            const float* src = p.x + (size_t)b * p.N * p.T;
            const int th0 = tt0 - p.pad;
            constexpr int HP = HSPAN / 2;
            constexpr int TOTAL = 32 * HP;
            for (int base = tid; base < TOTAL; base += 8 * 256) {
                float v[8][2];
#pragma unroll
                for (int u = 0; u < 8; ++u) {
                    const int idx = base + u * 256;
                    const int row = idx / HP, col = (idx - row * HP) * 2;
                    const int n = n0 + row, t = th0 + col;
                    const bool ok = idx < TOTAL && n < p.N;
                    const float* s = src + (size_t)(ok ? n : 0) * p.T;
                    v[u][0] = (ok && t >= 0 && t < p.T) ? s[t] : 0.0f;
                    v[u][1] = (ok && t + 1 >= 0 && t + 1 < p.T) ? s[t + 1] : 0.0f;
                }
#pragma unroll
                for (int u = 0; u < 8; ++u) {
                    const int idx = base + u * 256;
                    if (idx < TOTAL) {
                        const int row = idx / HP, col = (idx - row * HP) * 2;
                        float o0 = v[u][0], o1 = v[u][1];
                        if (p.alpha) {
                            const float sa = sn_a[row], sib = sn_ib[row];
                            o0 = sat_snake(o0, sa, sib);
                            o1 = sat_snake(o1, sa, sib);
                        }
                        uint32_t h, l;
                        sat_split2_pk(o0, o1, &h, &l);
                        *reinterpret_cast<uint32_t*>(&hi_lds[0][row][col]) = h;
                        *reinterpret_cast<uint32_t*>(&hi_lds[1][row][col]) = l;
                    }
                }
            }
        }
        __syncthreads();
        if (wave_on) {
#pragma unroll
            for (int ks = 0; ks < SAT_WB_TT / 16; ++ks) {
                const int tb = 16 * ks + 8 * hi;
                bf16x8 af[2];
                af[0] = *reinterpret_cast<const bf16x8*>(&lo_lds[0][m_w + l31][tb]);
                af[1] = *reinterpret_cast<const bf16x8*>(&lo_lds[1][m_w + l31][tb]);
#pragma unroll
                for (int pl = 0; pl < 2; ++pl) {
                    u32x4 cw[NCH];
#if !defined(SAT_HIPEMU)
                    asm volatile("" ::: "memory");
#endif
#pragma unroll
                    for (int j = 0; j < NCH; ++j) cw[j] = *reinterpret_cast<const u32x4*>(&hi_lds[pl][l31][tb + 8 * j]);
#pragma unroll
                    for (int k = 0; k < 7; ++k) {
                        const int off = k * DIL;
                        const int wbase = (off >> 3) * 4 + ((off & 7) >> 1);
                        const bool odd = (off & 1) != 0;
                        u32x4 r;
#pragma unroll
                        for (int i = 0; i < 4; ++i) {
                            const int w0 = wbase + i, w1 = wbase + i + 1;
                            const unsigned a0 = cw[w0 >> 2][w0 & 3];
                            if (odd) {
                                const unsigned a1 = cw[w1 >> 2][w1 & 3];
                                r[i] = sat_alignbit(a1, a0, 16);
                            } else {
                                r[i] = a0;
                            }
                        }
                        const bf16x8 bf = __builtin_bit_cast(bf16x8, r);
                        acc[k] = sat_mfma_32x32x16_bf16(af[0], bf, acc[k]);
                        if (pl == 0) acc[k] = sat_mfma_32x32x16_bf16(af[1], bf, acc[k]);
                    }
                }
            }
        }
        __syncthreads();
    }

    if (want_rs && (tid & 15) == 0) {
#pragma unroll
        for (int i = 0; i < 8; ++i) {
            const int m = m0 + (tid >> 4) + 16 * i;
            if (m < p.M) p.rowsum[(size_t)m * p.nsplit + split] = rs[i];
        }
    }
    if (wave_on) {
        float* ob = p.out + (size_t)split * p.so_split;
        const int n = n0 + l31;
#pragma unroll
        for (int k = 0; k < 7; ++k)
#pragma unroll
            for (int r = 0; r < 16; ++r) {
                const int m = m0 + m_w + (r & 3) + 8 * (r >> 2) + 4 * hi;
                if (m < p.M && n < p.N) ob[(size_t)m * p.so_m + (size_t)n * p.so_n + (size_t)k * p.so_k] = acc[k][r];
            }
    }
}

#include "conv_wgrad7_bf16x3_pipe.h"

struct SatWgBfPlan { int nsplit, cps, nchunks, nT; bool pipe; };
static void sat_wgbf_plan(int B, int M, int N, int T, SatWgBfPlan* pl) {
    pl->nT = sat_cdiv(T, SAT_WB_TT);
    pl->nchunks = B * pl->nT;
    pl->pipe = N >= SAT_WP_NI && (T & 3) == 0;
    const int tiles = sat_cdiv(M, SAT_CO_T) * sat_cdiv(N, pl->pipe ? SAT_WP_NI : 32);
    int want = 512 / tiles;
    if (want > pl->nchunks) want = pl->nchunks;
    if (want < 1) want = 1;
    if (want > 512) want = 512;
    pl->cps = sat_cdiv(pl->nchunks, want);
    pl->nsplit = sat_cdiv(pl->nchunks, pl->cps);
}
extern "C" int sat_conv_wgrad7_bf16x3_nsplit(int B, int M, int N, int T) {
    SatWgBfPlan pl;
    sat_wgbf_plan(B, M, N, T, &pl);
    return pl.nsplit;
}
extern "C" int sat_conv_wgrad7_bf16x3_fuses_rowsum(int B, int M, int N, int T) {
    SatWgBfPlan pl;
    sat_wgbf_plan(B, M, N, T, &pl);
    return pl.pipe ? 0 : 1;
}
extern "C" int sat_conv_wgrad7_bf16x3(const float* dy, const float* x, const float* alpha, const float* beta, float* partial,
                                      long long so_m, long long so_n, long long so_k, int B, int M, int N, int T, int dil,
                                      int pad, float* dy_rowsum, void* stream) {
    if (B <= 0 || M <= 0 || N <= 0 || T <= 0) { sat_set_error("sat_conv_wgrad7_bf16x3: empty shape"); return 1; }
    if (dil != 1 && dil != 3 && dil != 9) { sat_set_error("sat_conv_wgrad7_bf16x3: dilation must be 1, 3 or 9 (the Oobleck ResidualUnits)"); return 1; }
    if ((alpha == nullptr) != (beta == nullptr)) { sat_set_error("sat_conv_wgrad7_bf16x3: alpha/beta must both be given"); return 1; }
    SatWgBfPlan pl;
    sat_wgbf_plan(B, M, N, T, &pl);
    SatWgBfParams p{dy, x, alpha, beta, partial, (long long)M * N * 7, so_m, so_n, so_k, B, M, N, T, pad, pl.cps, pl.nchunks, pl.nT,
                    dy_rowsum, pl.nsplit};
    if (pl.pipe) {
        dim3 grid(sat_cdiv(M, SAT_CO_T), sat_cdiv(N, SAT_WP_NI), pl.nsplit);
        if (dy_rowsum) { sat_set_error("sat_conv_wgrad7_bf16x3: this shape's kernel does not fuse the row sums (sat_conv_wgrad7_bf16x3_fuses_rowsum)"); return 1; }
        if (dil == 1) SAT_LAUNCH((sat_wgrad7_bf16x3_pipe_kernel<1>), grid, dim3(SAT_WP_NT), stream, p);
        else if (dil == 3) SAT_LAUNCH((sat_wgrad7_bf16x3_pipe_kernel<3>), grid, dim3(SAT_WP_NT), stream, p);
        else SAT_LAUNCH((sat_wgrad7_bf16x3_pipe_kernel<9>), grid, dim3(SAT_WP_NT), stream, p);
        return sat_check_launch("sat_conv_wgrad7_bf16x3");
    }
    dim3 grid(sat_cdiv(M, SAT_CO_T), sat_cdiv(N, 32), pl.nsplit);
    if (dil == 1) SAT_LAUNCH(sat_wgrad7_bf16x3_kernel<1>, grid, dim3(256), stream, p);
    else if (dil == 3) SAT_LAUNCH(sat_wgrad7_bf16x3_kernel<3>, grid, dim3(256), stream, p);
    else SAT_LAUNCH(sat_wgrad7_bf16x3_kernel<9>, grid, dim3(256), stream, p);
    return sat_check_launch("sat_conv_wgrad7_bf16x3");
}

#include "conv_wgrad7_planes.h"

struct SatTrProbeParams { const short* image; const int* lane_off; short* out; };
__global__ void __launch_bounds__(64) sat_lds_read_tr16_probe_kernel(SatTrProbeParams p) {
    __shared__ __attribute__((aligned(16))) short img[1024];
    const int lane = threadIdx.x;
    for (int i = lane; i < 1024; i += 64) img[i] = p.image[i];
    __syncthreads();
    const bf16x4 v = sat_lds_read_tr16_b64(reinterpret_cast<const char*>(img) + p.lane_off[lane]);
#pragma unroll
    for (int e = 0; e < 4; ++e) p.out[4 * lane + e] = v[e];
}
extern "C" int sat_lds_read_tr16_probe(const short* image, const int* lane_off, short* out, void* stream) {
    if (!image || !lane_off || !out) { sat_set_error("sat_lds_read_tr16_probe: missing buffer"); return 1; }
    SatTrProbeParams p{image, lane_off, out};
    SAT_LAUNCH(sat_lds_read_tr16_probe_kernel, dim3(1), dim3(64), stream, p);
    return sat_check_launch("sat_lds_read_tr16_probe");
}

extern "C" int sat_conv_wgrad7_planes_ok(int B, int M, int N, int T, int dil, int pad, int rows_dy, int rows_act) {
    if (B <= 0 || M <= 0 || N < SAT_WQ_NI || T <= 0) return 0;
    if ((dil != 1 && dil != 3 && dil != 9) || pad < 0 || pad > SAT_WQ_LEAD) return 0;
    const int nT = sat_cdiv(T, SAT_WB_TT);
    if (rows_dy < SAT_WQ_LEAD + nT * SAT_WB_TT) return 0;
    if (rows_act < SAT_WQ_LEAD + (nT - 1) * SAT_WB_TT - pad + 128) return 0;
    if (rows_act < SAT_WQ_LEAD + T + 6 * dil - pad) return 0;
    return 1;
}
static void sat_wgpl_plan(int B, int M, int N, int T, SatWgBfPlan* pl) {
    pl->nT = sat_cdiv(T, SAT_WB_TT);
    pl->nchunks = B * pl->nT;
    pl->pipe = true;
    const int tiles = sat_cdiv(M, SAT_CO_T) * sat_cdiv(N, SAT_WQ_NI);
    int want = 512 / tiles;
    if (want > pl->nchunks) want = pl->nchunks;
    if (want < 1) want = 1;
    pl->cps = sat_cdiv(pl->nchunks, want);
    pl->nsplit = sat_cdiv(pl->nchunks, pl->cps);
}
extern "C" int sat_conv_wgrad7_planes_nsplit(int B, int M, int N, int T) {
    if (B <= 0 || M <= 0 || N <= 0 || T <= 0) return -1;
    SatWgBfPlan pl;
    sat_wgpl_plan(B, M, N, T, &pl);
    return pl.nsplit;
}
extern "C" int sat_conv_wgrad7_planes(const short* dy_hi, const short* dy_lo, int rows_dy, const short* act_hi, const short* act_lo,
                                      int rows_act, float* partial, long long so_m, long long so_n, long long so_k, int B, int M, int N,
                                      int T, int dil, int pad, void* stream) {
    if (!dy_hi || !dy_lo || !act_hi || !act_lo || !partial) { sat_set_error("sat_conv_wgrad7_planes: missing buffer"); return 1; }
    if (!sat_conv_wgrad7_planes_ok(B, M, N, T, dil, pad, rows_dy, rows_act)) {
        sat_set_error("sat_conv_wgrad7_planes: shape outside the kernel's contract (sat_conv_wgrad7_planes_ok)");
        return 1;
    }
    if ((((uintptr_t)dy_hi | (uintptr_t)dy_lo | (uintptr_t)act_hi | (uintptr_t)act_lo) & 15) != 0) { sat_set_error("sat_conv_wgrad7_planes: planes must be 16-byte aligned"); return 1; }
    SatWgBfPlan pl;
    sat_wgpl_plan(B, M, N, T, &pl);
    SatWgPlParams p{dy_hi, dy_lo, act_hi, act_lo, partial, (long long)M * N * 7, so_m, so_n, so_k, B, M, N, T, pad, rows_dy, rows_act,
                    sat_cdiv(M, 8), sat_cdiv(N, 8), pl.cps, pl.nchunks, pl.nT};
    dim3 grid(sat_cdiv(M, SAT_CO_T), sat_cdiv(N, SAT_WQ_NI), pl.nsplit);
    if (dil == 1) SAT_LAUNCH((sat_wgrad7_planes_kernel<1>), grid, dim3(SAT_WQ_NT), stream, p);
    else if (dil == 3) SAT_LAUNCH((sat_wgrad7_planes_kernel<3>), grid, dim3(SAT_WQ_NT), stream, p);
    else SAT_LAUNCH((sat_wgrad7_planes_kernel<9>), grid, dim3(SAT_WQ_NT), stream, p);
    return sat_check_launch("sat_conv_wgrad7_planes");
}

#define SAT_WS_TT 64
#define SAT_WS_LOROW (SAT_WS_TT + 8)
#define SAT_WS_HIROW (SAT_WS_TT + 8)

struct SatWgSmallParams {
    const float* lo;
    const float* hi;
    const float* alpha;
    const float* beta;
    float* out;
    long long so_split, so_m, so_n, so_k;
    int B, M, N, Tlo, Thi, pad, snake_on, s_log2;
    int chunks_per_split, nchunks, nT;
    float* rowsum;
    int nsplit;
};

template <int NT>
__global__ void __launch_bounds__(256)
#if !defined(SAT_HIPEMU)
__attribute__((amdgpu_waves_per_eu(2, 2)))
#endif
sat_wgrad_small_bf16x3_kernel(SatWgSmallParams p) {
    constexpr int NCH = NT;
    __shared__ __attribute__((aligned(16))) short lo_lds[2][SAT_CO_T][SAT_WS_LOROW];
    __shared__ __attribute__((aligned(16))) short hi_lds[2][SAT_CO_T][SAT_WS_HIROW];
    __shared__ float sn_a[SAT_CO_T], sn_ib[SAT_CO_T];

    const int tid = threadIdx.x, lane = tid & 63, wave = tid >> 6;
    const int l31 = lane & 31, hi = lane >> 5;
    const int sl = p.s_log2, S = 1 << sl;
    int mn_tile, split;
    sat_xcd_tile(blockIdx.x + gridDim.x * (blockIdx.y + gridDim.y * blockIdx.z), gridDim.x * gridDim.y, gridDim.z, &mn_tile, &split);
    const int m0 = (mn_tile % (int)gridDim.x) * SAT_CO_T, v0 = (mn_tile / (int)gridDim.x) * SAT_CO_T;
    const int n_base = v0 >> sl, nc = SAT_CO_T >> sl;
    const int NV = p.N << sl;
    const int m_w = (wave >> 1) * 64, v_w = (wave & 1) * 64;
    const bool wave_on = (m0 + m_w) < p.M && (v0 + v_w) < NV;
    const bool snake_lo = p.alpha && p.snake_on == 1, snake_hi = p.alpha && p.snake_on == 2;

    f32x16 acc[2][2][NT];
#pragma unroll
    for (int i = 0; i < 2; ++i)
#pragma unroll
        for (int j = 0; j < 2; ++j)
#pragma unroll
            for (int k = 0; k < NT; ++k)
#pragma unroll
                for (int r = 0; r < 16; ++r) acc[i][j][k][r] = 0.0f;

    const bool want_rs = p.rowsum != nullptr && v0 == 0;
    float rsum[8] = {0.f, 0.f, 0.f, 0.f, 0.f, 0.f, 0.f, 0.f};

    if (tid < SAT_CO_T) {
        float sa = 1.f, sib = 0.f;
        const int c = snake_lo ? m0 + tid : n_base + tid;
        const bool ok = snake_lo ? c < p.M : (snake_hi && tid < nc && c < p.N);
        if (ok) {
            sa = expf(p.alpha[c]);
            sib = 1.0f / (expf(p.beta[c]) + 1e-9f);
        }
        sn_a[tid] = sa;
        sn_ib[tid] = sib;
    }
    __syncthreads();

    const int c_begin = split * p.chunks_per_split;
    int c_end = c_begin + p.chunks_per_split;
    if (c_end > p.nchunks) c_end = p.nchunks;
    const int rs = (SAT_WS_TT + NT - 1) << sl;
    const int up = rs >> 1;
    const int total_units = nc * up;

    auto mfma_stage = [&]() {
        if (wave_on) {
            SAT_MFMA_PRIO(1);
#pragma unroll
            for (int ks = 0; ks < SAT_WS_TT / 16; ++ks) {
                const int tb = 16 * ks + 8 * hi;
                bf16x8 af[2][2];
#pragma unroll
                for (int mi = 0; mi < 2; ++mi)
#pragma unroll
                    for (int pl = 0; pl < 2; ++pl)
                        af[mi][pl] = *reinterpret_cast<const bf16x8*>(&lo_lds[pl][m_w + mi * 32 + l31][tb]);
#pragma unroll
                for (int ni = 0; ni < 2; ++ni) {
#pragma unroll
                    for (int pl = 0; pl < 2; ++pl) {
                        u32x4 cw[NCH];
#pragma unroll
                        for (int j = 0; j < NCH; ++j) cw[j] = *reinterpret_cast<const u32x4*>(&hi_lds[pl][v_w + ni * 32 + l31][tb + 8 * j]);
#pragma unroll
                        for (int j = 0; j < NT; ++j) {
                            u32x4 r = cw[0];
                            if (j == 1) {
                                r[0] = sat_alignbit(cw[0][1], cw[0][0], 16);
                                r[1] = sat_alignbit(cw[0][2], cw[0][1], 16);
                                r[2] = sat_alignbit(cw[0][3], cw[0][2], 16);
                                r[3] = sat_alignbit(cw[NCH - 1][0], cw[0][3], 16);
                            }
                            const bf16x8 bf = __builtin_bit_cast(bf16x8, r);
#pragma unroll
                            for (int mi = 0; mi < 2; ++mi) {
                                acc[mi][ni][j] = sat_mfma_32x32x16_bf16(af[mi][0], bf, acc[mi][ni][j]);
                                if (pl == 0) acc[mi][ni][j] = sat_mfma_32x32x16_bf16(af[mi][1], bf, acc[mi][ni][j]);
                            }
                        }
                    }
                }
            }
            SAT_MFMA_PRIO(0);
        }
    };

    const bool fast1 = (NT == 1) && sl == 0 && p.pad == 0 && (p.Tlo & 3) == 0 && p.Thi == p.Tlo;
    if (fast1) {
        float4 vlo[8], vhi[8];
        const int row0 = tid >> 4, c4 = (tid & 15) * 4;
        auto issue = [&](int ch) {
            const int b = ch / p.nT;
            const int tt0 = (ch - b * p.nT) * SAT_WS_TT;
            const float* slo = p.lo + (size_t)b * p.M * p.Tlo;
            const float* shi = p.hi + (size_t)b * p.N * p.Thi;
            const bool t_ok = tt0 + c4 < p.Tlo;
#pragma unroll
            for (int u = 0; u < 8; ++u) {
                const int m = m0 + row0 + 16 * u, n = v0 + row0 + 16 * u;
                const bool okm = t_ok && m < p.M, okn = t_ok && n < p.N;
                const float4 a = *reinterpret_cast<const float4*>(slo + (size_t)(okm ? m : 0) * p.Tlo + (okm ? tt0 + c4 : 0));
                const float4 c = *reinterpret_cast<const float4*>(shi + (size_t)(okn ? n : 0) * p.Thi + (okn ? tt0 + c4 : 0));
                vlo[u] = okm ? a : make_float4(0.f, 0.f, 0.f, 0.f);
                vhi[u] = okn ? c : make_float4(0.f, 0.f, 0.f, 0.f);
            }
        };
        auto convert = [&]() {
            typedef uint32_t u2 __attribute__((ext_vector_type(2)));
#pragma unroll
            for (int u = 0; u < 8; ++u) {
                const int row = row0 + 16 * u;
                float4 q = vlo[u];
                if (want_rs) rsum[u] += sat_row16_sum(q);
                if (snake_lo) {
                    const float sa = sn_a[row], sib = sn_ib[row];
                    q.x = sat_snake(q.x, sa, sib); q.y = sat_snake(q.y, sa, sib);
                    q.z = sat_snake(q.z, sa, sib); q.w = sat_snake(q.w, sa, sib);
                }
                uint32_t h0, h1, l0, l1;
                sat_split2_pk(q.x, q.y, &h0, &l0);
                sat_split2_pk(q.z, q.w, &h1, &l1);
                *reinterpret_cast<u2*>(&lo_lds[0][row][c4]) = u2{h0, h1};
                *reinterpret_cast<u2*>(&lo_lds[1][row][c4]) = u2{l0, l1};
                q = vhi[u];
                if (snake_hi) {
                    const float sa = sn_a[row], sib = sn_ib[row];
                    q.x = sat_snake(q.x, sa, sib); q.y = sat_snake(q.y, sa, sib);
                    q.z = sat_snake(q.z, sa, sib); q.w = sat_snake(q.w, sa, sib);
                }
                sat_split2_pk(q.x, q.y, &h0, &l0);
                sat_split2_pk(q.z, q.w, &h1, &l1);
                *reinterpret_cast<u2*>(&hi_lds[0][row][c4]) = u2{h0, h1};
                *reinterpret_cast<u2*>(&hi_lds[1][row][c4]) = u2{l0, l1};
            }
        };
        issue(c_begin);
        for (int ch = c_begin; ch < c_end; ++ch) {
            convert();
            __syncthreads();
            if (ch + 1 < c_end) issue(ch + 1);
            mfma_stage();
            __syncthreads();
        }
    } else if ((NT == 2) && sl >= 1 && sl <= 3 && (p.Tlo & 3) == 0) {
        typedef float f4u __attribute__((ext_vector_type(4), aligned(4)));
        typedef uint32_t u2 __attribute__((ext_vector_type(2)));
        constexpr int NQ = 9;
        const int qpc = 33 << (sl - 1);
        const unsigned magic = 0xffffffffu / (unsigned)qpc + 1u;
        const int total_q = nc * qpc;
        const int qcl = sl >= 2 ? sl - 2 : 0, qc = 1 << qcl;
        auto load_quads = [&](int tv, const float* shi, int th0, bool interior, f4u* vq, auto ib, auto ie) {
            constexpr int IB = decltype(ib)::value, IE = decltype(ie)::value;
#pragma unroll
            for (int i = IB; i < IE; ++i) {
                f4u v = {0.f, 0.f, 0.f, 0.f};
                if (i < NQ - 1 || wave == 0) {
                    const int Q = tv + 256 * i;
                    const int cl = (int)sat_umulhi((unsigned)Q, magic), q = Q - cl * qpc;
                    const int n = n_base + cl, t = th0 + 4 * q;
                    const float* sp = shi + (size_t)(n < p.N ? n : p.N - 1) * p.Thi;
                    if (interior) {
                        v = *reinterpret_cast<const f4u*>(sp + t);
                    } else {
#pragma unroll
                        for (int e = 0; e < 4; ++e) {
                            const int te = t + e;
                            const int tc = te < 0 ? 0 : (te < p.Thi ? te : p.Thi - 1);
                            const float x = sp[tc];
                            v[e] = (te == tc) ? x : 0.0f;
                        }
                    }
                    if (n >= p.N) v = f4u{0.f, 0.f, 0.f, 0.f};
                }
                vq[i - IB] = v;
            }
        };
        auto store_quads = [&](int tv, const f4u* vq, auto ib, auto ie) {
            constexpr int IB = decltype(ib)::value, IE = decltype(ie)::value;
#pragma unroll
            for (int i = IB; i < IE; ++i) {
                const int Q = tv + 256 * i;
                if (i == NQ - 1 && Q >= total_q) break;
                const int cl = (int)sat_umulhi((unsigned)Q, magic), q = Q - cl * qpc;
                f4u o = vq[i - IB];
                if (snake_hi) {
                    const float sa = sn_a[cl], sib = sn_ib[cl];
#pragma unroll
                    for (int e = 0; e < 4; ++e) o[e] = sat_snake(o[e], sa, sib);
                }
                uint32_t h01, l01, h23, l23;
                sat_split2_pk(o[0], o[1], &h01, &l01);
                sat_split2_pk(o[2], o[3], &h23, &l23);
                int row, col;
                uint32_t wh0, wh1, wl0, wl1;
                if (sl == 1) {
                    row = cl << 1;
                    col = 2 * q;
                    wh0 = (h01 & 0xffffu) | (h23 << 16); wh1 = (h01 >> 16) | (h23 & 0xffff0000u);
                    wl0 = (l01 & 0xffffu) | (l23 << 16); wl1 = (l01 >> 16) | (l23 & 0xffff0000u);
                } else {
                    const int colq = q >> qcl, part = q & (qc - 1);
                    const bool odd = colq & 1;
                    const uint32_t rh = __shfl_xor(odd ? h01 : h23, qc), rl = __shfl_xor(odd ? l01 : l23, qc);
                    row = (cl << sl) + 4 * part + (odd ? 2 : 0);
                    col = colq & ~1;
                    if (!odd) {
                        wh0 = (h01 & 0xffffu) | (rh << 16); wh1 = (h01 >> 16) | (rh & 0xffff0000u);
                        wl0 = (l01 & 0xffffu) | (rl << 16); wl1 = (l01 >> 16) | (rl & 0xffff0000u);
                    } else {
                        wh0 = (rh & 0xffffu) | (h23 << 16); wh1 = (rh >> 16) | (h23 & 0xffff0000u);
                        wl0 = (rl & 0xffffu) | (l23 << 16); wl1 = (rl >> 16) | (l23 & 0xffff0000u);
                    }
                }
                *reinterpret_cast<uint32_t*>(&hi_lds[0][row][col]) = wh0;
                *reinterpret_cast<uint32_t*>(&hi_lds[0][row + 1][col]) = wh1;
                *reinterpret_cast<uint32_t*>(&hi_lds[1][row][col]) = wl0;
                *reinterpret_cast<uint32_t*>(&hi_lds[1][row + 1][col]) = wl1;
            }
        };
        using I0 = std::integral_constant<int, 0>; using IN = std::integral_constant<int, NQ>;
        f4u vq[NQ];
        auto issue_hi = [&](int ch) {
            const int b = ch / p.nT;
            const int tt0 = (ch - b * p.nT) * SAT_WS_TT;
            const int th0 = (tt0 << sl) - p.pad;
            const bool interior = th0 >= 0 && th0 + (66 << sl) <= p.Thi;
            int tv = tid;
#if !defined(SAT_HIPEMU)
            asm volatile("" : "+v"(tv));
#endif
            load_quads(tv, p.hi + (size_t)b * p.N * p.Thi, th0, interior, vq, I0{}, IN{});
        };
#if !defined(SAT_WGS_NOCARRY)
        issue_hi(c_begin);
#endif
        for (int ch = c_begin; ch < c_end; ++ch) {
            const int b = ch / p.nT;
            const int tt0 = (ch - b * p.nT) * SAT_WS_TT;
            const float* slo = p.lo + (size_t)b * p.M * p.Tlo;
            int tv = tid;
#if !defined(SAT_HIPEMU)
            asm volatile("" : "+v"(tv));
#endif
            const int row0 = tv >> 4, c4 = (tv & 15) * 4;
            float4 vlo[8];
#if defined(SAT_WGS_NOCARRY)
            issue_hi(ch);
#endif
            {
                const bool t_ok = tt0 + c4 < p.Tlo;
#pragma unroll
                for (int u = 0; u < 8; ++u) {
                    const int m = m0 + row0 + 16 * u;
                    const bool okm = t_ok && m < p.M;
                    const float4 a = *reinterpret_cast<const float4*>(slo + (size_t)(okm ? m : 0) * p.Tlo + (okm ? tt0 + c4 : 0));
                    vlo[u] = okm ? a : make_float4(0.f, 0.f, 0.f, 0.f);
                }
            }
            SAT_SCHED_FENCE();
            store_quads(tv, vq, I0{}, IN{});
            SAT_SCHED_FENCE();
#pragma unroll
            for (int u = 0; u < 8; ++u) {
                const int row = row0 + 16 * u;
                float4 q = vlo[u];
                if (want_rs) rsum[u] += sat_row16_sum(q);
                if (snake_lo) {
                    const float sa = sn_a[row], sib = sn_ib[row];
                    q.x = sat_snake(q.x, sa, sib); q.y = sat_snake(q.y, sa, sib);
                    q.z = sat_snake(q.z, sa, sib); q.w = sat_snake(q.w, sa, sib);
                }
                uint32_t h0, h1, l0, l1;
                sat_split2_pk(q.x, q.y, &h0, &l0);
                sat_split2_pk(q.z, q.w, &h1, &l1);
                *reinterpret_cast<u2*>(&lo_lds[0][row][c4]) = u2{h0, h1};
                *reinterpret_cast<u2*>(&lo_lds[1][row][c4]) = u2{l0, l1};
            }
            __syncthreads();
#if !defined(SAT_WGS_NOCARRY)
            if (ch + 1 < c_end) issue_hi(ch + 1);
#endif
            mfma_stage();
            __syncthreads();
        }
    } else
    for (int ch = c_begin; ch < c_end; ++ch) {
        const int b = ch / p.nT;
        const int tt0 = (ch - b * p.nT) * SAT_WS_TT;
        {
            const float* src = p.lo + (size_t)b * p.M * p.Tlo;
            for (int half = 0; half < 2; ++half) {
                float4 v[4];
#pragma unroll
                for (int u = 0; u < 4; ++u) {
                    const int idx = tid + (half * 4 + u) * 256;
                    const int row = idx >> 4, c4 = (idx & 15) * 4;
                    const int m = m0 + row, t = tt0 + c4;
                    float4 q = make_float4(0.f, 0.f, 0.f, 0.f);
                    if (m < p.M) {
                        const float* s = src + (size_t)m * p.Tlo + t;
                        if (t + 3 < p.Tlo && ((p.Tlo & 3) == 0)) {
                            q = *reinterpret_cast<const float4*>(s);
                        } else {
                            if (t + 0 < p.Tlo) q.x = s[0];
                            if (t + 1 < p.Tlo) q.y = s[1];
                            if (t + 2 < p.Tlo) q.z = s[2];
                            if (t + 3 < p.Tlo) q.w = s[3];
                        }
                    }
                    v[u] = q;
                }
#pragma unroll
                for (int u = 0; u < 4; ++u) {
                    const int idx = tid + (half * 4 + u) * 256;
                    const int row = idx >> 4, c4 = (idx & 15) * 4;
                    float4 q = v[u];
                    if (want_rs) rsum[half * 4 + u] += sat_row16_sum(q);
                    if (snake_lo) {
                        const float sa = sn_a[row], sib = sn_ib[row];
                        q.x = sat_snake(q.x, sa, sib);
                        q.y = sat_snake(q.y, sa, sib);
                        q.z = sat_snake(q.z, sa, sib);
                        q.w = sat_snake(q.w, sa, sib);
                    }
                    uint32_t h0, h1, l0, l1;
                    sat_split2_pk(q.x, q.y, &h0, &l0);
                    sat_split2_pk(q.z, q.w, &h1, &l1);
                    typedef uint32_t u2 __attribute__((ext_vector_type(2)));
                    *reinterpret_cast<u2*>(&lo_lds[0][row][c4]) = u2{h0, h1};
                    *reinterpret_cast<u2*>(&lo_lds[1][row][c4]) = u2{l0, l1};
                }
            }
        }
        {
            const float* src = p.hi + (size_t)b * p.N * p.Thi;
            const int th0 = (tt0 << sl) - p.pad;
            for (int base = tid; base < total_units; base += 8 * 256) {
                float v[8][2];
#pragma unroll
                for (int u = 0; u < 8; ++u) {
                    const int idx = base + u * 256;
                    const int cl = idx / up, uu = (idx - cl * up) * 2;
                    const int n = n_base + cl, t = th0 + uu;
                    const bool ok = idx < total_units && n < p.N;
                    const float* s = src + (size_t)(ok ? n : 0) * p.Thi;
                    v[u][0] = (ok && t >= 0 && t < p.Thi) ? s[t] : 0.0f;
                    v[u][1] = (ok && t + 1 >= 0 && t + 1 < p.Thi) ? s[t + 1] : 0.0f;
                }
#pragma unroll
                for (int u = 0; u < 8; ++u) {
                    const int idx = base + u * 256;
                    if (idx < total_units) {
                        const int cl = idx / up, uu = (idx - cl * up) * 2;
                        float o0 = v[u][0], o1 = v[u][1];
                        if (snake_hi) {
                            const float sa = sn_a[cl], sib = sn_ib[cl];
                            o0 = sat_snake(o0, sa, sib);
                            o1 = sat_snake(o1, sa, sib);
                        }
                        uint32_t h, l;
                        sat_split2_pk(o0, o1, &h, &l);
                        if (sl == 0) {
                            *reinterpret_cast<uint32_t*>(&hi_lds[0][cl][uu]) = h;
                            *reinterpret_cast<uint32_t*>(&hi_lds[1][cl][uu]) = l;
                        } else {
                            const int row = (cl << sl) + (uu & (S - 1)), col = uu >> sl;
                            hi_lds[0][row][col] = (short)(h & 0xffffu);
                            hi_lds[0][row + 1][col] = (short)(h >> 16);
                            hi_lds[1][row][col] = (short)(l & 0xffffu);
                            hi_lds[1][row + 1][col] = (short)(l >> 16);
                        }
                    }
                }
            }
        }
        __syncthreads();
        mfma_stage();
        __syncthreads();
    }

    if (want_rs && (tid & 15) == 0) {
#pragma unroll
        for (int i = 0; i < 8; ++i) {
            const int m = m0 + (tid >> 4) + 16 * i;
            if (m < p.M) p.rowsum[(size_t)m * p.nsplit + split] = rsum[i];
        }
    }
    if (wave_on) {
        float* ob = p.out + (size_t)split * p.so_split;
#pragma unroll
        for (int mi = 0; mi < 2; ++mi)
#pragma unroll
            for (int ni = 0; ni < 2; ++ni) {
                const int v = v0 + v_w + ni * 32 + l31;
                const int n = v >> sl, ph = v & (S - 1);
#pragma unroll
                for (int j = 0; j < NT; ++j)
#pragma unroll
                    for (int r = 0; r < 16; ++r) {
                        const int m = m0 + m_w + mi * 32 + (r & 3) + 8 * (r >> 2) + 4 * hi;
                        if (m < p.M && n < p.N)
                            ob[(size_t)m * p.so_m + (size_t)n * p.so_n + (size_t)(j * S + ph) * p.so_k] = acc[mi][ni][j][r];
                    }
            }
    }
}

static bool sat_wgs_plan(int B, int M, int N, int Tlo, int K, int stride, SatWgBfPlan* pl, int* s_log2, int* nt) {
    if (B <= 0 || M <= 0 || N <= 0 || Tlo <= 0) return false;
    if (K == 1 && stride == 1) { *s_log2 = 0; *nt = 1; }
    else if (K == 2 * stride && stride >= 2 && stride <= 64 && (stride & (stride - 1)) == 0) {
        int l = 0;
        while ((1 << l) < stride) ++l;
        *s_log2 = l;
        *nt = 2;
    } else return false;
    pl->nT = sat_cdiv(Tlo, SAT_WS_TT);
    pl->nchunks = B * pl->nT;
    const int tiles = sat_cdiv(M, SAT_CO_T) * sat_cdiv(N << *s_log2, SAT_CO_T);
    int want = 512 / tiles;
    if (want > pl->nchunks) want = pl->nchunks;
    if (want < 1) want = 1;
    if (want > 1024) want = 1024;
    pl->cps = sat_cdiv(pl->nchunks, want);
    pl->nsplit = sat_cdiv(pl->nchunks, pl->cps);
    return true;
}
extern "C" int sat_conv_wgrad_bf16x3_nsplit(int B, int M, int N, int Tlo, int K, int stride) {
    SatWgBfPlan pl;
    int sl, nt;
    return sat_wgs_plan(B, M, N, Tlo, K, stride, &pl, &sl, &nt) ? pl.nsplit : -1;
}
extern "C" int sat_conv_wgrad_bf16x3(const float* lo, const float* hi, const float* alpha, const float* beta, int snake_on,
                                     float* partial, long long so_m, long long so_n, long long so_k, int B, int M, int N,
                                     int Tlo, int Thi, int K, int stride, int pad, float* lo_rowsum, void* stream) {
    SatWgBfPlan pl;
    int sl, nt;
    if (!sat_wgs_plan(B, M, N, Tlo, K, stride, &pl, &sl, &nt)) {
        sat_set_error("sat_conv_wgrad_bf16x3: needs K == 1 (stride 1) or K == 2*stride with a power-of-two stride");
        return 1;
    }
    if (Thi <= 0 || pad < 0) { sat_set_error("sat_conv_wgrad_bf16x3: bad shape"); return 1; }
    if (alpha && (snake_on != 1 && snake_on != 2)) { sat_set_error("sat_conv_wgrad_bf16x3: snake_on must be 1 (lo) or 2 (hi)"); return 1; }
    if ((alpha == nullptr) != (beta == nullptr)) { sat_set_error("sat_conv_wgrad_bf16x3: alpha/beta must both be given"); return 1; }
    SatWgSmallParams p{lo, hi, alpha, beta, partial, (long long)M * N * K, so_m, so_n, so_k,
                       B, M, N, Tlo, Thi, pad, alpha ? snake_on : 0, sl, pl.cps, pl.nchunks, pl.nT, lo_rowsum, pl.nsplit};
    dim3 grid(sat_cdiv(M, SAT_CO_T), sat_cdiv(N << sl, SAT_CO_T), pl.nsplit);
    if (nt == 1) SAT_LAUNCH(sat_wgrad_small_bf16x3_kernel<1>, grid, dim3(256), stream, p);
    else SAT_LAUNCH(sat_wgrad_small_bf16x3_kernel<2>, grid, dim3(256), stream, p);
    return sat_check_launch("sat_conv_wgrad_bf16x3");
}
```

### stable_audio_tools_amd/functional.py

```python
import torch

from . import ops as _ops_mod
from .ops import PACK_CONV_DGRAD, PACK_CONV_FWD, PACK_POLYPHASE


def _ops(ops):
    return ops if ops is not None else _ops_mod.get_ops()


class SumAllFn(torch.autograd.Function):

    @staticmethod
    def forward(ctx, x, ops=None):
        ctx.in_shape, ctx.in_dtype = x.shape, x.dtype
        return _ops(ops).sum_all(x.detach())

    @staticmethod
    def backward(ctx, g):
        return g.to(ctx.in_dtype).expand(ctx.in_shape), None


def sum_all(x, ops=None):
    return SumAllFn.apply(x, ops)


def mean_all(x, ops=None):
    return SumAllFn.apply(x, ops) / x.numel()


class DerivedCache:

    def __init__(self):
        self.items = {}

    def get(self, name, sources, make):
        from . import _caches
        if not _caches.trackable(*sources):
            return make()
        key = tuple((t.data_ptr(), _caches.version_of(t), t.device) for t in sources if t is not None) + _caches.epoch_of(*sources)
        hit = self.items.get(name)
        if hit is None or hit[0] != key:
            hit = (key, make())
            self.items[name] = hit
        return hit[1]


def _cached(cache, name, sources, make):
    return make() if cache is None else cache.get(name, sources, make)


class WeightNormFn(torch.autograd.Function):
    @staticmethod
    def forward(ctx, v, g, ops=None):
        ops = _ops(ops)
        v = v.contiguous()
        gf = g.contiguous().view(-1)
        w, norm = ops.wn_fold(v, gf)
        ctx.save_for_backward(v, gf, norm)
        ctx.ops = ops
        ctx.g_shape = g.shape
        return w

    @staticmethod
    def backward(ctx, dw):
        v, gf, norm = ctx.saved_tensors
        dv, dg = ctx.ops.wn_grad(v, gf, norm, dw.contiguous())
        return dv, dg.view(ctx.g_shape), None


def _conv_dgrad(ops, dy, w, k, stride, dil, pad, cin, tin, dsnake, res=None, out=None, emit=None):
    if stride == 1:
        if (res is None and out is None and not emit and ops.edge_ok(w.shape[0], cin, k, 1, dil, (k - 1) * dil - pad) and tin == dy.shape[2]
                and (dsnake is None or w.shape[0] <= 2)):
            return ops.edge_conv(dy, w, (k - 1) * dil - pad, mode=1, dsnake=dsnake)
        if ops.bf16x3_ok(k, 1, dil):
            q = ops.k7q_applicable(w.shape[0], k, 1, dil, (k - 1) * dil - pad, cin)
            return ops.conv1d_bf16x3(dy, ops.pack_bf16x3(w, mode=1, q=q), cin, k, 1, dil, (k - 1) * dil - pad, tout=tin,
                                     dsnake=dsnake, res=res, out=out, emit=emit)
        wpb = ops.pack(w, PACK_CONV_DGRAD)
        return ops.conv1d(dy, wpb, cin, k, 1, dil, (k - 1) * dil - pad, tout=tin, dsnake=dsnake, res=res, out=out)
    if out is not None:
        raise NotImplementedError("_conv_dgrad(out=...) is only plumbed through the stride-1 kernels")
    if ops.bf16x3_ok(k, stride, dil, transposed=True):
        return ops.convtr1d_bf16x3(dy, ops.pack_bf16x3(w, mode=2, stride=stride), cin, k, stride, pad, tout=tin,
                                   dsnake=dsnake, res=res)
    wpb = ops.pack(w, PACK_POLYPHASE, stride)
    return ops.convtr1d(dy, wpb, cin, k, stride, pad, tout=tin, dsnake=dsnake, res=res)


def _conv_wgrad(ops, dy, x, k, stride, dil, pad, snake, bias_grad=False, raw=False):
    if ops.edge_ok(x.shape[1], dy.shape[1], k, stride, dil, pad) and dy.shape[2] == x.shape[2] and (snake is None or dy.shape[1] <= 2):
        return ops.edge_conv_wgrad(dy, x, k, pad, snake=snake, dy_rowsum=bias_grad, raw=raw)
    if ops.wgrad7_bf16x3_ok(x.shape[1], k, stride, dil):
        return ops.conv_wgrad7_bf16x3(dy, x, dil, pad, snake=snake, dy_rowsum=bias_grad, raw=raw)
    return ops.conv_wgrad(dy, x, k, stride, dil, pad, snake=snake, snake_on=2, lo_rowsum=bias_grad, raw=raw)


def _wn_forward(ops, v, g):
    v = v.contiguous()
    gf = g.contiguous().view(-1)
    w, norm = ops.wn_fold(v, gf)
    return w, (v, gf, norm)


def _wn_backward(ops, slabs, saved, g_shape, bias_partial=None):
    v, gf, norm = saved
    out = ops.wn_grad_splits(slabs, v, gf, norm, bias_partial=bias_partial)
    return (out[0], out[1].view(g_shape)) + tuple(out[2:])


def _conv_fwd(ops, x, w, stride, dil, pad, bias=None, snake=None, res=None, tanh_out=False, dsnake=None, tout=None, cache=None, emit=None,
              keep_planes=False):
    cout, cin, k = w.shape
    if (res is None and ops.edge_ok(cin, cout, k, stride, dil, pad) and (tout is None or tout == x.shape[2])
            and (snake is None or cout <= 2) and (dsnake is None or cin <= 2) and (not emit or cin <= 2)):
        y = ops.edge_conv(x, w, pad, bias=bias, snake=snake, tanh_out=tanh_out, dsnake=dsnake, emit=emit)
    elif ops.bf16x3_ok(k, stride, dil):
        q = ops.k7q_applicable(cin, k, stride, dil, pad, cout)
        planes = _cached(cache, "pack_fwd_q" if q else "pack_fwd", (w,), lambda: ops.pack_bf16x3(w, stride=stride, q=q))
        sconsts = _cached(cache, "snake", snake, lambda: ops.snake_consts(snake[0], snake[1])) if snake is not None else None
        return ops.conv1d_bf16x3(x, planes, cout, k, stride, dil, pad, tout=tout, bias=bias,
                                 snake=snake, res=res, tanh_out=tanh_out, dsnake=dsnake, sconsts=sconsts, emit=emit, keep_planes=keep_planes)
    else:
        y = ops.conv1d(x, _cached(cache, "pack_fwd32", (w,), lambda: ops.pack(w, PACK_CONV_FWD)), cout, k, stride, dil, pad, tout=tout,
                       bias=bias, snake=snake, res=res, tanh_out=tanh_out, dsnake=dsnake)
    return (y, None) if keep_planes else y


def _convtr_fwd(ops, x, w, stride, pad, bias=None, snake=None, cache=None):
    cin, cout, k = w.shape
    if ops.bf16x3_ok(k, stride, 1, transposed=True):
        planes = _cached(cache, "pack_tr", (w,), lambda: ops.pack_bf16x3(w, mode=2, stride=stride))
        sconsts = _cached(cache, "snake", snake, lambda: ops.snake_consts(snake[0], snake[1])) if snake is not None else None
        return ops.convtr1d_bf16x3(x, planes, cout, k, stride, pad, bias=bias, snake=snake, sconsts=sconsts)
    return ops.convtr1d(x, _cached(cache, "pack_tr32", (w,), lambda: ops.pack(w, PACK_POLYPHASE, stride)), cout, k, stride, pad,
                        bias=bias, snake=snake)


class SnakeConv1dFn(torch.autograd.Function):

    @staticmethod
    def forward(ctx, x, alpha, beta, w, bias, res, stride, dil, pad, tanh_out, ops=None, cache=None, next_snake=None, g=None):
        ops = _ops(ops)
        x = x.contiguous()
        wn = ()
        if g is not None:
            w, wn = _wn_forward(ops, w, g)
        w = w.contiguous()
        cout, cin, k = w.shape
        snake = (alpha.contiguous(), beta.contiguous()) if alpha is not None else None
        emit = None
        if next_snake is not None and not tanh_out:
            tout_ = (x.shape[2] + 2 * pad - dil * (k - 1) - 1) // stride + 1
            if ((ops.emit_ok(cout, k, stride, tout_, next_snake[2]) and ops.bf16x3_ok(k, stride, dil))
                    or (res is None and snake is None and ops.edge_emit_ok(cin, cout, k, stride, dil, pad, next_snake[2]))):
                emit = (next_snake[0].detach(), next_snake[1].detach())
        y = _conv_fwd(ops, x, w, stride, dil, pad, bias=bias, snake=snake,
                      res=res.contiguous() if res is not None else None, tanh_out=tanh_out, cache=cache, emit=emit)
        ctx.ops = ops
        ctx.cfg = (stride, dil, pad, tanh_out, bias is not None, res is not None, alpha is not None)
        ctx.g_shape = g.shape if g is not None else None
        ctx.save_for_backward(x, alpha, beta, w, y if tanh_out else None, *wn)
        return y

    @staticmethod
    def backward(ctx, dy):
        ops = ctx.ops
        stride, dil, pad, tanh_out, has_bias, has_res, has_snake = ctx.cfg
        x, alpha, beta, w, y = ctx.saved_tensors[:5]
        wn = ctx.saved_tensors[5:]
        cout, cin, k = w.shape
        dy = dy.contiguous()
        if tanh_out:
            dy = dy * (1.0 - y * y)
        snake = (alpha, beta) if has_snake else None
        dres = dy if has_res else None
        dw = dbias = dg = None
        if ctx.needs_input_grad[3] or (wn and ctx.needs_input_grad[13]):
            dw = _conv_wgrad(ops, dy, x, k, stride, dil, pad, snake, bias_grad=has_bias, raw=bool(wn))
            if has_bias:
                dw, dbias = dw
            if wn:
                dw, dg, *rest = _wn_backward(ops, dw, wn, ctx.g_shape, bias_partial=dbias)
                if has_bias:
                    dbias = rest[0]
        elif has_bias:
            dbias = ops.rowsum(dy)
        dx = da = db = None
        if has_snake:
            dx, da, db = _conv_dgrad(ops, dy, w, k, stride, dil, pad, cin, x.shape[2], (x, alpha, beta))
        elif ctx.needs_input_grad[0]:
            dx = _conv_dgrad(ops, dy, w, k, stride, dil, pad, cin, x.shape[2], None)
        return dx, da, db, dw, dbias, dres, None, None, None, None, None, None, None, dg


class SnakeConvTr1dFn(torch.autograd.Function):

    @staticmethod
    def forward(ctx, x, alpha, beta, w, bias, stride, pad, ops=None, cache=None, g=None):
        ops = _ops(ops)
        x = x.contiguous()
        wn = ()
        if g is not None:
            w, wn = _wn_forward(ops, w, g)
        w = w.contiguous()
        cin, cout, k = w.shape
        snake = (alpha.contiguous(), beta.contiguous()) if alpha is not None else None
        y = _convtr_fwd(ops, x, w, stride, pad, bias=bias, snake=snake, cache=cache)
        ctx.ops = ops
        ctx.cfg = (stride, pad, bias is not None, alpha is not None)
        ctx.g_shape = g.shape if g is not None else None
        ctx.save_for_backward(x, alpha, beta, w, *wn)
        return y

    @staticmethod
    def backward(ctx, dy):
        ops = ctx.ops
        stride, pad, has_bias, has_snake = ctx.cfg
        x, alpha, beta, w = ctx.saved_tensors[:4]
        wn = ctx.saved_tensors[4:]
        cin, cout, k = w.shape
        dy = dy.contiguous()
        snake = (alpha, beta) if has_snake else None
        dbias = ops.rowsum(dy) if has_bias else None
        dw = ops.conv_wgrad(x, dy, k, stride, 1, pad, snake=snake, snake_on=1, raw=bool(wn))
        dg = None
        if wn:
            dw, dg = _wn_backward(ops, dw, wn, ctx.g_shape)
        dx = da = db = None
        if has_snake:
            dx, da, db = _conv_fwd(ops, dy, w, stride, 1, pad, dsnake=(x, alpha, beta), tout=x.shape[2])
        elif ctx.needs_input_grad[0]:
            dx = _conv_fwd(ops, dy, w, stride, 1, pad, tout=x.shape[2])
        return dx, da, db, dw, dbias, None, None, None, None, dg


class ResidualUnitFn(torch.autograd.Function):

    @staticmethod
    def forward(ctx, x, a1, b1, w1, bias1, a2, b2, w2, bias2, dil, ops=None, recompute=False, caches=None, next_snake=None, fuse=False,
                g1=None, g2=None):
        ops = _ops(ops)
        x = x.contiguous()
        wn1 = wn2 = ()
        if g1 is not None:
            w1, wn1 = _wn_forward(ops, w1, g1)
        if g2 is not None:
            w2, wn2 = _wn_forward(ops, w2, g2)
        w1 = w1.contiguous()
        w2 = w2.contiguous()
        c = x.shape[1]
        k1 = w1.shape[2]
        pad = dil * (k1 - 1) // 2
        c1, c2 = caches if caches is not None else (None, None)
        emit = ctx.k7_planes = None
        if next_snake is not None and ops.emit_ok(c, w2.shape[2], 1, x.shape[2], next_snake[2]):
            emit = (next_snake[0].detach(), next_snake[1].detach())
        if fuse and w2.shape[2] == 1 and w1.shape[0] == c and ops.ru_fused_ok(c, k1, dil, x.shape[2]):
            w7q = _cached(c1, "pack_q7", (w1,), lambda: ops.pack_k7q(w1))
            w1q = _cached(c2, "pack_q1", (w2,), lambda: ops.pack_k7q(w2))
            sc = None
            if c1 is not None and c2 is not None:
                sc = (_cached(c1, "snake", (a1, b1), lambda: ops.snake_consts(a1, b1)), _cached(c2, "snake", (a2, b2), lambda: ops.snake_consts(a2, b2)))
            h, y = ops.residual_unit_fwd(x, (a1, b1), w7q, bias1, (a2, b2), w1q, bias2, k1, dil, keep_h=ctx is not None and not recompute and fuse != "nokeep",
                                         emit=emit, sconsts=sc)
        else:
            keep = bool(ops.wgrad7_planes and not recompute and any(ctx.needs_input_grad))
            h = _conv_fwd(ops, x, w1, 1, dil, pad, bias=bias1, snake=(a1, b1), cache=c1, keep_planes=keep)
            if keep:
                h, ctx.k7_planes = h
            y = _conv_fwd(ops, h, w2, 1, 1, 0, bias=bias2, snake=(a2, b2), res=x, cache=c2, emit=emit)
        ctx.ops = ops
        ctx.dil = dil
        ctx.recompute = bool(recompute)
        ctx.g_shapes = (g1.shape if g1 is not None else None, g2.shape if g2 is not None else None)
        ctx.save_for_backward(x, None if recompute else h, a1, b1, w1, a2, b2, w2, bias1 if recompute else None, *wn1, *wn2)
        return y

    @staticmethod
    def backward(ctx, dy):
        ops = ctx.ops
        x, h, a1, b1, w1, a2, b2, w2, bias1 = ctx.saved_tensors[:9]
        gs1, gs2 = ctx.g_shapes
        rest = ctx.saved_tensors[9:]
        wn1 = rest[:3] if gs1 is not None else ()
        wn2 = rest[len(wn1):] if gs2 is not None else ()
        dil = ctx.dil
        c = x.shape[1]
        k1, k2 = w1.shape[2], w2.shape[2]
        pad1 = dil * (k1 - 1) // 2
        t = x.shape[2]
        dy = dy.contiguous()
        if ctx.recompute:
            h = _conv_fwd(ops, x, w1, 1, dil, pad1, bias=bias1, snake=(a1, b1))
        want_emit = ops.emit_ok(w1.shape[0], k2, 1, t, dil) and ops.k7q_applicable(w1.shape[0], k1, 1, dil, pad1, c)
        kept = ctx.k7_planes if not ctx.recompute and want_emit and ops.kept_planes_valid(ctx.k7_planes, x, (a1, b1), dil, pad1) else None
        skip_dh = False

        def wgrad1(dh, bias_grad):
            dw = ops.conv_wgrad7_from_planes(dh, kept, x, (a1, b1), dil, pad1, raw=bool(wn1))
            if dw is None:
                return _conv_wgrad(ops, dh, x, k1, 1, dil, pad1, (a1, b1), bias_grad=bias_grad, raw=bool(wn1))
            return (dw, ops.rowsum(dh, partial=bool(wn1))) if bias_grad else dw
        if k2 == 1 and w2.shape[0] == c and w1.shape[0] == c and ops.ru_k1_bwd_ok(dy.shape[0], c, t):
            skip_dh = bool(kept is not None and ops.ru_k1_bwd_skip_dh)
            dh, da2, db2, dw2, dbias2, dbias1 = ops.ru_k1_bwd(dy, h, w2, (a2, b2), emit=want_emit, raw=bool(wn2), skip_dh=skip_dh)
            try:
                dw1 = wgrad1(dh, False)
                if skip_dh:
                    dx, da1, db1 = _conv_dgrad(ops, dh, w1, k1, 1, dil, pad1, c, t, (x, a1, b1), res=dy)
            finally:
                ops.dh_written()
        else:
            dw2, dbias2 = ops.conv_wgrad(dy, h, k2, 1, 1, 0, snake=(a2, b2), snake_on=2, lo_rowsum=True, raw=bool(wn2))
            dh, da2, db2 = _conv_dgrad(ops, dy, w2, k2, 1, 1, 0, c, t, (h, a2, b2), emit=want_emit)
            dw1, dbias1 = wgrad1(dh, True)
        dg1 = dg2 = None
        if wn1:
            if dbias1.dim() == 2:
                dw1, dg1, dbias1 = _wn_backward(ops, dw1, wn1, gs1, bias_partial=dbias1)
            else:
                dw1, dg1 = _wn_backward(ops, dw1, wn1, gs1)
        if wn2:
            if dbias2.dim() == 2:
                dw2, dg2, dbias2 = _wn_backward(ops, dw2, wn2, gs2, bias_partial=dbias2)
            else:
                dw2, dg2 = _wn_backward(ops, dw2, wn2, gs2)
        if not skip_dh:
            dx, da1, db1 = _conv_dgrad(ops, dh, w1, k1, 1, dil, pad1, c, t, (x, a1, b1), res=dy)
        return dx, da1, db1, dw1, dbias1, da2, db2, dw2, dbias2, None, None, None, None, None, None, dg1, dg2


class VaeSampleFn(torch.autograd.Function):

    @staticmethod
    def forward(ctx, pre, noise, ops=None):
        ops = _ops(ops)
        pre = pre.contiguous()
        noise = noise.contiguous()
        z, kl = ops.vae_sample_fwd(pre, noise)
        ctx.ops = ops
        ctx.save_for_backward(pre, noise)
        return z, kl

    @staticmethod
    def backward(ctx, dz, dkl):
        pre, noise = ctx.saved_tensors
        dpre = ctx.ops.vae_sample_bwd(pre, noise, dz.contiguous() if dz is not None else None,
                                      dkl.contiguous() if dkl is not None else None)
        return dpre, None, None
```

### stable_audio_tools_amd/ops.py

```python
import ctypes

import torch

from . import _caches, _lib

PACK_CONV_FWD = 0
PACK_CONV_DGRAD = 1
PACK_POLYPHASE = 2


def _ptr(t):
    if t is None:
        return None
    return ctypes.c_void_p(t.data_ptr())


def _keep_zeros(shape, dtype, device):
    with torch.inference_mode(False):
        return torch.zeros(shape, dtype=dtype, device=device)


def _keep_empty(shape, dtype, device):
    with torch.inference_mode(False):
        return torch.empty(shape, dtype=dtype, device=device)


class WgradSlabs:
    __slots__ = ("partial", "nsplit", "dims", "strides")

    def __init__(self, partial, nsplit, dims, strides):
        self.partial, self.nsplit, self.dims, self.strides = partial, int(nsplit), tuple(int(d) for d in dims), tuple(int(x) for x in strides)

    @property
    def count(self):
        return self.partial.shape[1]

    def reduce(self, ops):
        m, n, k = self.dims
        part = self.partial if self.count == m * n * k else self.partial[:, :m * n * k].contiguous()
        flat = ops._reduce_rows(part, self.nsplit, m * n * k)
        if self.strides == (n * k, k, 1):
            return flat.view(m, n, k)
        if self.strides == (n, 1, m * n):
            return flat.view(k, m, n).permute(1, 2, 0).contiguous()
        raise ValueError("WgradSlabs.reduce: unknown slab layout %s" % (self.strides,))


def _snake_key(snake):
    return None if snake is None else (snake[0].data_ptr(), snake[1].data_ptr(), _caches.version_of(snake[0]), _caches.version_of(snake[1]))


class Planes:
    __slots__ = ("hi", "lo", "rows", "own", "gen", "ptr", "shape", "ver", "snake")

    def __init__(self, hi, lo, rows, own=None):
        self.hi, self.lo, self.rows, self.own, self.gen = hi, lo, rows, own, own.gen if own is not None else None
        self.ptr = self.shape = self.ver = self.snake = None

    def __getitem__(self, name):
        return getattr(self, name)

    def of(self, x, snake):
        self.ptr, self.shape, self.ver, self.snake = x.data_ptr(), tuple(x.shape), _caches.version_of(x), _snake_key(snake)
        return self

    def holds(self, x, snake):
        return (self.ptr == x.data_ptr() and self.shape == tuple(x.shape) and _caches.trackable(x) and self.ver == _caches.version_of(x)
                and self.snake == _snake_key(snake) and (self.own is None or self.gen == self.own.gen))


class OwnedPlanes:
    __slots__ = ("hi", "lo", "rows", "gen", "stream")

    def __init__(self, n, rows, device, stream):
        self.hi, self.lo, self.rows, self.gen, self.stream = _keep_zeros(n, torch.int16, device), _keep_zeros(n, torch.int16, device), rows, 0, stream

    def rewrite(self):
        self.gen += 1
        return Planes(self.hi, self.lo, self.rows, self)


class SatOps:
    def __init__(self, cdll):
        self.lib = cdll
        self.simulator = bool(cdll.sat_is_simulator())
        self._planes = {}
        self._own_planes = {}
        self._emitted = None
        self._dh_unwritten = None
        self._zpage = None
        self._disc_pool, self._disc_gen, self._disc_geoms = {}, {}, {}
        self._disc_emitted = None

    def _stream(self, t):
        if self.simulator:
            return None
        return ctypes.c_void_p(torch.cuda.current_stream(t.device).cuda_stream)

    def _workspace(self, key, shape, dtype, device, zero=False, grow=False):
        shape = (shape,) if isinstance(shape, int) else tuple(shape)
        ws = self._planes.get(key)
        if ws is None or ws.device != device or (ws.numel() < shape[0] if grow else tuple(ws.shape) != shape):
            ws = self._planes[key] = (_keep_zeros if zero else _keep_empty)(shape, dtype, device)
        return ws

    def _chk(self, status):
        if status != 0:
            raise RuntimeError(self.lib.sat_last_error().decode())

    def _f32(self, *tensors):
        for t in tensors:
            if t is None:
                continue
            if t.dtype != torch.float32:
                raise TypeError(f"expected float32 tensor, got {t.dtype}")
            if not t.is_contiguous():
                raise ValueError("expected contiguous tensor")
            if not self.simulator and not t.is_cuda:
                raise RuntimeError("stable_audio_tools_amd kernels need CUDA(HIP) tensors; there is no CPU path")

    def wn_fold(self, v, g):
        self._f32(v, g)
        d0 = v.shape[0]
        r = v.numel() // d0
        w = torch.empty_like(v)
        norm = torch.empty(d0, dtype=torch.float32, device=v.device)
        self._chk(self.lib.sat_wn_fold(_ptr(v), _ptr(g), _ptr(w), _ptr(norm), d0, r, self._stream(v)))
        return w, norm

    def wn_grad(self, v, g, norm, dw):
        self._f32(v, g, norm, dw)
        d0 = v.shape[0]
        r = v.numel() // d0
        dv = torch.empty_like(v)
        dg = torch.empty_like(g)
        self._chk(self.lib.sat_wn_grad(_ptr(v), _ptr(g), _ptr(norm), _ptr(dw), _ptr(dv), _ptr(dg), d0, r, self._stream(v)))
        return dv, dg

    wn_fused = True

    def wn_grad_splits(self, slabs, v, g, norm, bias_partial=None):
        self._f32(v, g, norm, slabs.partial, bias_partial)
        m, n, k = slabs.dims
        if tuple(v.shape) != (m, n, k):
            raise ValueError("wn_grad_splits: slabs of a %s weight gradient for a %s weight" % ((m, n, k), tuple(v.shape)))
        dv = torch.empty_like(v)
        dg = torch.empty_like(g)
        dbias, cols = None, 0
        if bias_partial is not None:
            if bias_partial.dim() != 2 or bias_partial.shape[0] != m:
                raise ValueError("wn_grad_splits: bias_partial must be (D0, R)")
            cols = bias_partial.shape[1]
            dbias = torch.empty(m, dtype=torch.float32, device=v.device)
        so_m, so_n, so_k = slabs.strides
        self._chk(self.lib.sat_wn_grad_splits(_ptr(slabs.partial), slabs.nsplit, slabs.count, so_m, so_n, so_k, _ptr(v), _ptr(g), _ptr(norm),
                                              _ptr(dv), _ptr(dg), m, n, k, _ptr(bias_partial), cols, _ptr(dbias), self._stream(v)))
        return (dv, dg) if bias_partial is None else (dv, dg, dbias)

    def pack(self, w, mode, stride=1):
        self._f32(w)
        d0, d1, k = w.shape
        out = torch.empty(w.numel(), dtype=torch.float32, device=w.device)
        self._chk(self.lib.sat_pack_weights(_ptr(w), _ptr(out), d0, d1, k, stride, mode, self._stream(w)))
        return out

    def _reduce_rows(self, partial, rows, count, scale=1.0):
        out = torch.empty(count, dtype=torch.float32, device=partial.device)
        self._chk(self.lib.sat_reduce_splits(_ptr(partial), _ptr(out), count, rows, scale, 0, self._stream(partial)))
        return out

    def _sum_pair(self, pda, pdb):
        c, r = pda.shape
        both = self.rowsum(pda._base.view(1, 2 * c, r) if pda._base is not None else torch.stack([pda, pdb]).view(1, 2 * c, r))
        return both[:c], both[c:]

    def _sum_last(self, partial):
        c, r = partial.shape
        return self.rowsum(partial.view(1, c, r))

    def _dsnake_args(self, dsnake, cout, rows, device):
        if dsnake is None:
            return None, None, None, None, None
        x2, a2, b2 = dsnake
        self._f32(x2, a2, b2)
        return (x2, a2, b2, *torch.empty(2, cout, rows, dtype=torch.float32, device=device).unbind(0))

    def _dsnake_result(self, y, pda, pdb):
        return y if pda is None else (y, *self._sum_pair(pda, pdb))

    def conv1d(self, x, w_packed, cout, k, stride=1, dil=1, pad=0, tout=None, bias=None, snake=None, res=None,
               tanh_out=False, dsnake=None, out=None):
        b, cin, tin = x.shape
        if tout is None:
            tout = (tin + 2 * pad - dil * (k - 1) - 1) // stride + 1
        alpha, beta = snake if snake is not None else (None, None)
        self._f32(x, w_packed, bias, alpha, beta, res)
        y = self._conv_out(out, b, cout, tout, x.device)
        rows = self.lib.sat_conv1d_partial_rows(b, tout) if dsnake is not None else 0
        x2, a2, b2, pda, pdb = self._dsnake_args(dsnake, cout, rows, x.device)
        self._chk(self.lib.sat_conv1d(_ptr(x), _ptr(w_packed), _ptr(bias), _ptr(alpha), _ptr(beta), _ptr(res), _ptr(y),
                                      _ptr(x2), _ptr(a2), _ptr(b2), _ptr(pda), _ptr(pdb),
                                      b, cin, cout, tin, tout, k, stride, dil, pad, int(tanh_out), self._stream(x)))
        return self._dsnake_result(y, pda, pdb)

    use_bf16x3 = True

    edge_convs = True

    def edge_ok(self, cin, cout, k, stride, dil, pad):
        return bool(self.edge_convs) and bool(self.lib.sat_edge_conv_ok(cin, cout, k, stride, dil, pad))

    def edge_conv(self, x, w, pad, mode=0, bias=None, snake=None, tanh_out=False, dsnake=None, emit=None):
        b, cin, t = x.shape
        k = w.shape[2]
        cout = w.shape[0] if mode == 0 else w.shape[1]
        alpha, beta = snake if snake is not None else (None, None)
        self._f32(x, w, bias, alpha, beta)
        y = torch.empty(b, cout, t, dtype=torch.float32, device=x.device)
        rows = self.lib.sat_edge_conv_partial_rows(b, t) if dsnake is not None else 0
        x2, a2, b2, pda, pdb = self._dsnake_args(dsnake, cout, rows, x.device)
        ep, ela, elb = self._emit_args(emit, b, cout, t, x.device, self._stream(x), consts=False)
        self._chk(self.lib.sat_edge_conv(_ptr(x), _ptr(w), _ptr(bias), _ptr(alpha), _ptr(beta), _ptr(y), _ptr(x2), _ptr(a2), _ptr(b2),
                                         _ptr(pda), _ptr(pdb), _ptr(ep.hi), _ptr(ep.lo), _ptr(ela), _ptr(elb), ep.rows, b, cin, cout, t, k, pad, mode,
                                         int(tanh_out), self._stream(x)))
        self._emit_done(emit, y, ep)
        return self._dsnake_result(y, pda, pdb)

    def edge_conv_wgrad(self, dy, x, k, pad, snake=None, dy_rowsum=False, raw=False):
        b, m, t = dy.shape
        n = x.shape[1]
        alpha, beta = snake if snake is not None else (None, None)
        self._f32(dy, x, alpha, beta)
        nsplit = self.lib.sat_edge_conv_wgrad_nsplit(b, m, n, t)
        partial = torch.empty(nsplit, m * n * k, dtype=torch.float32, device=dy.device)
        fused = dy_rowsum and n <= 2
        rs = torch.empty(m, nsplit, dtype=torch.float32, device=dy.device) if fused else None
        self._chk(self.lib.sat_edge_conv_wgrad(_ptr(dy), _ptr(x), _ptr(alpha), _ptr(beta), _ptr(partial), _ptr(rs), b, m, n, t, k, pad,
                                               self._stream(dy)))
        return self._wgrad_result(WgradSlabs(partial, nsplit, (m, n, k), (n * k, k, 1)), raw, dy, dy_rowsum, rs)

    def _wgrad_result(self, slabs, raw, dy, dy_rowsum, rs):
        dw = slabs if raw else slabs.reduce(self)
        if not dy_rowsum:
            return dw
        if raw:
            return dw, (rs if rs is not None else self.rowsum(dy, partial=True))
        return dw, (self._sum_last(rs) if rs is not None else self.rowsum(dy))

    def bf16x3_ok(self, k, stride, dil, transposed=False):
        if not self.use_bf16x3:
            return False
        if transposed or stride > 1:
            return k == 2 * stride and stride & (stride - 1) == 0 and dil == 1
        return k == 1 or (2 <= k <= 4 and dil == 1) or (5 <= k <= 8 and (k - 1) * dil <= 62)

    k7q = True
    k7q_persist = True
    k7q_dma_in_mfma = True
    k7q_min_cin = 64
    k7q_min_cout = 128
    k7q_wide_cin = 512

    def k7q_applicable(self, cin, k, stride, dil, pad, cout=None):
        return (self.k7q and self.use_bf16x3 and stride == 1 and 5 <= k <= 7 and 0 <= pad <= 32
                and (k - 1) * dil <= 62 and cin >= self.k7q_min_cin
                and (cout is None or cout >= self.k7q_min_cout or cin >= self.k7q_wide_cin))

    def pack_bf16x3(self, w, mode=0, stride=1, q=False):
        if q:
            if stride != 1:
                raise RuntimeError("sat_pack_weights_k7q: unsupported shape")
            return (*self.pack_k7q(w, mode), "q")
        self._f32(w)
        d0, d1, k = w.shape
        n = self.lib.sat_pack_weights_bf16x3_size(d0, d1, k, stride, mode)
        if n <= 0:
            raise RuntimeError("sat_pack_weights_bf16x3: unsupported shape")
        hi = torch.empty(n, dtype=torch.int16, device=w.device)
        lo = torch.empty(n, dtype=torch.int16, device=w.device)
        self._chk(self.lib.sat_pack_weights_bf16x3(_ptr(w), _ptr(hi), _ptr(lo), d0, d1, k, stride, mode, self._stream(w)))
        return hi, lo

    def snake_consts(self, alpha, beta):
        self._f32(alpha, beta)
        a = torch.empty_like(alpha)
        ib = torch.empty_like(beta)
        self._chk(self.lib.sat_snake_consts(_ptr(alpha), _ptr(beta), _ptr(a), _ptr(ib), alpha.numel(), self._stream(alpha)))
        return a, ib

    def _conv_out(self, out, b, cout, tout, device):
        if out is None:
            return torch.empty(b, cout, tout, dtype=torch.float32, device=device)
        if tuple(out.shape) != (b, cout, tout) or not out.is_contiguous():
            raise ValueError("conv out= must be a dense (B, Cout, Tout) tensor")
        self._f32(out)
        return out

    def _bf16x3_call(self, fn, rows, x, w_planes, cout, tout, dims, bias, snake, res, tanh_out, dsnake, out=None, sconsts=None, emit=None):
        b, cin, tin = x.shape
        self._f32(x, bias, res)
        sa = sib = None
        if snake is not None:
            sa, sib = sconsts if sconsts is not None else self.snake_consts(snake[0], snake[1])
        y = self._conv_out(out, b, cout, tout, x.device)
        x2, a2, b2, pda, pdb = self._dsnake_args(dsnake, cout, rows, x.device)
        ep, ea, eib = self._emit_args(emit, b, cout, tout, x.device, self._stream(x))
        args = (_ptr(x), _ptr(w_planes[0]), _ptr(w_planes[1]), _ptr(bias), _ptr(sa), _ptr(sib),
                _ptr(res), _ptr(y), _ptr(x2), _ptr(a2), _ptr(b2), _ptr(pda), _ptr(pdb),
                b, cin, cout, tin, tout, *dims, int(tanh_out))
        if emit:
            self._chk(self.lib.sat_conv1d_bf16x3_emit(*args, _ptr(ep.hi), _ptr(ep.lo), _ptr(ea), _ptr(eib), ep.rows, self._stream(x)))
        else:
            self._chk(fn(*args, self._stream(x)))
        self._emit_done(emit, y, ep)
        return self._dsnake_result(y, pda, pdb)

    ru_fused = True

    def ru_fused_ok(self, c, k, dil, t):
        return (self.ru_fused and self.use_bf16x3 and self.k7q and self.k7q_min_cin <= c <= 128
                and 5 <= k <= 7 and (k - 1) * dil <= 62 and (k - 1) * dil % 2 == 0 and (k - 1) * dil // 2 <= 32 and t % 4 == 0)

    def pack_k7q(self, w, mode=0):
        self._f32(w)
        d0, d1, k = w.shape
        n = self.lib.sat_pack_weights_k7q_size(d0, d1, k, mode)
        if n <= 0:
            raise RuntimeError("sat_pack_weights_k7q: unsupported shape")
        hi = torch.empty(n, dtype=torch.int16, device=w.device)
        lo = torch.empty(n, dtype=torch.int16, device=w.device)
        self._chk(self.lib.sat_pack_weights_k7q(_ptr(w), _ptr(hi), _ptr(lo), d0, d1, k, mode, self._stream(w)))
        return hi, lo

    def residual_unit_fwd(self, x, snake1, w7q, bias1, snake2, w1q, bias2, k, dil, keep_h=True, emit=None, sconsts=None):
        b, c, t = x.shape
        self._f32(x, bias1, bias2)
        pad = (k - 1) * dil // 2
        st = self._stream(x)
        sa1, sib1 = sconsts[0] if sconsts is not None else self.snake_consts(snake1[0], snake1[1])
        sa2, sib2 = sconsts[1] if sconsts is not None else self.snake_consts(snake2[0], snake2[1])
        xp = self._take_emitted(x, snake1) or self._k7_prepass(x, sa1, sib1, t, pad, st)
        h = torch.empty_like(x) if keep_h else None
        y = torch.empty_like(x)
        ep, ea, eib = self._emit_args(emit, b, c, t, x.device, st, owned=False)
        if emit and ep.hi.data_ptr() == xp.hi.data_ptr():
            ep = self._emit_planes(b, c, t, x.device, st, alt=True)
        self._chk(self.lib.sat_residual_unit_fwd(_ptr(xp.hi), _ptr(xp.lo), xp.rows, _ptr(w7q[0]), _ptr(w7q[1]), _ptr(bias1), _ptr(sa2), _ptr(sib2),
                                                 _ptr(w1q[0]), _ptr(w1q[1]), _ptr(bias2), _ptr(x), _ptr(h), _ptr(y), b, c, t, k, dil, pad,
                                                 _ptr(ep.hi), _ptr(ep.lo), _ptr(ea), _ptr(eib), ep.rows, st))
        self._emit_done(emit, y, ep)
        return h, y

    _NO_PLANES = Planes(None, None, 0)
    k7_emit = True
    wgrad7_planes = True
    wgrad7_planes_budget_gib = 16.0
    ru_k1_bwd_skip_dh = True

    def emit_ok(self, cout, k, stride, tout, consumer_dil):
        if not (self.k7_emit and self.use_bf16x3 and self.k7q_applicable(cout, 7, 1, consumer_dil, 3 * consumer_dil, cout)):
            return False
        generic = (stride == 1 and k <= 4) or stride > 1
        return generic and tout % 4 == 0

    def edge_emit_ok(self, cin, cout, k, stride, dil, pad, consumer_dil):
        return (self.k7_emit and self.use_bf16x3 and cin <= 2 and self.edge_ok(cin, cout, k, stride, dil, pad)
                and self.k7q_applicable(cout, 7, 1, consumer_dil, 3 * consumer_dil, cout))

    def _emit_args(self, emit, b, c, t, device, st, consts=True, owned=True):
        if not emit:
            return self._NO_PLANES, None, None
        snake = None if emit is True else emit
        ea, eb = (None, None) if snake is None else self.snake_consts(*snake) if consts else snake
        self._f32(ea, eb)
        return self._emit_planes(b, c, t, device, st, owner=snake if owned else None), ea, eb

    def _emit_done(self, emit, y, planes):
        if emit:
            snake = None if emit is True else emit
            self._emitted = planes.of(y, snake) if _caches.trackable(y, *(snake or ())) else None

    def _take_emitted(self, x, snake, peek=False):
        e = self._emitted
        if not peek:
            self._emitted = None
        return e if e is not None and e.holds(x, snake) else None

    def _emit_planes(self, b, c, t, device, st, alt=False, owner=None):
        own = self._owned_planes(owner, b, c, t, device, st)
        if own is not None:
            return own.rewrite()
        rows = self.lib.sat_conv1d_k7_plane_rows(t, t, 0)
        key = ("emit", b, c, t, device, st.value if st is not None else 0, alt)
        n = b * ((c + 7) // 8) * rows * 8
        return Planes(self._workspace(key + ("hi",), n, torch.int16, device, zero=True),
                      self._workspace(key + ("lo",), n, torch.int16, device, zero=True), rows)

    def _k7_prepass(self, x, sa, sib, tout, pad, st):
        b, c, t = x.shape
        rows = self.lib.sat_conv1d_k7_plane_rows(t, tout, pad)
        need = 2 * b * ((c + 7) // 8) * rows * 8
        ws = self._workspace(("k7p", x.device, st.value if st is not None else 0), need, torch.int16, x.device, grow=True)
        hi, lo = ws[:need // 2], ws[need // 2:need]
        self._chk(self.lib.sat_conv1d_k7_planes(_ptr(x), _ptr(sa), _ptr(sib), _ptr(hi), _ptr(lo), b, c, t, rows, st))
        return Planes(hi, lo, rows)

    def _owned_planes(self, snake, b, c, t, device, st, create=False):
        if snake is None or not self.wgrad7_planes:
            return None
        key = (snake[0].data_ptr(), snake[1].data_ptr(), b, c, t, device)
        own = self._own_planes.get(key)
        capturing = device.type == "cuda" and torch.cuda.is_current_stream_capturing()
        sv = st.value if st is not None else 0
        if own is not None and own.stream != sv and not capturing:
            return None
        if own is None and create and not capturing:
            rows = self.lib.sat_conv1d_k7_plane_rows(t, t, 0)
            n = b * ((c + 7) // 8) * rows * 8
            if sum(4 * o.hi.numel() for o in self._own_planes.values()) + 4 * n <= self.wgrad7_planes_budget_gib * 2 ** 30:
                own = self._own_planes[key] = OwnedPlanes(n, rows, device, sv)
        return own

    def release_owned_planes(self):
        self._own_planes.clear()

    def kept_planes_valid(self, kept, x, snake, dil, pad):
        b, c, t = x.shape
        return bool(kept is not None and self.wgrad7_planes and kept.holds(x, snake) and self.conv_wgrad7_planes_ok(b, c, c, t, dil, pad, kept.rows, kept.rows))

    def conv_wgrad7_from_planes(self, dh, kept, x, snake, dil, pad, raw=False):
        em = self._take_emitted(dh, None, peek=True) if kept is not None and self.wgrad7_planes and kept.holds(x, snake) else None
        b, c, t = x.shape
        if em is None or not self.conv_wgrad7_planes_ok(b, c, c, t, dil, pad, em.rows, kept.rows):
            return None
        return self.conv_wgrad7_planes((em.hi, em.lo, em.rows), (kept.hi, kept.lo, kept.rows), b, c, c, t, dil, pad, raw=raw)

    def _check_written(self, t):
        if t is not None and self._dh_unwritten is not None and t.data_ptr() == self._dh_unwritten:
            raise RuntimeError("this tensor is a dh that sat_ru_k1_bwd did not write (skip_dh): only its planes exist")

    def dh_written(self):
        self._dh_unwritten = None

    def conv1d_bf16x3(self, x, w_planes, cout, k, stride=1, dil=1, pad=0, tout=None, bias=None, snake=None, res=None,
                      tanh_out=False, dsnake=None, out=None, sconsts=None, emit=None, keep_planes=False):
        b, cin, tin = x.shape
        if tout is None:
            tout = (tin + 2 * pad - dil * (k - 1) - 1) // stride + 1
        rows = self.lib.sat_conv1d_bf16x3_partial_rows(b, tout, k, stride)
        if len(w_planes) == 3:
            if not (stride == 1 and 5 <= k <= 7 and 0 <= pad <= 32 and (k - 1) * dil <= 62):
                raise ValueError("conv1d_bf16x3: q-packed weights need stride 1, 5 <= K <= 7, pad <= 32, (K-1)*dil <= 62")
            return self._k7_planes_call(rows, x, w_planes, cout, tout, k, dil, pad, bias, snake, res, tanh_out, dsnake, out, sconsts, keep_planes)
        y = self._bf16x3_call(self.lib.sat_conv1d_bf16x3, rows, x, w_planes, cout, tout, (k, stride, dil, pad),
                              bias, snake, res, tanh_out, dsnake, out, sconsts, emit)
        return (y, None) if keep_planes else y

    def _k7_planes_call(self, prows, x, w_planes, cout, tout, k, dil, pad, bias, snake, res, tanh_out, dsnake, out=None, sconsts=None,
                        keep_planes=False):
        b, cin, tin = x.shape
        self._f32(x, bias, res)
        sa = sib = None
        if snake is not None:
            sa, sib = sconsts if sconsts is not None else self.snake_consts(snake[0], snake[1])
        st = self._stream(x)
        xp = self._take_emitted(x, snake)
        if xp is None:
            self._check_written(x)
        own = self._owned_planes(snake, b, cin, tin, x.device, st, create=True) if keep_planes and tin == tout and _caches.trackable(x) else None
        if xp is None and own is not None:
            xp = own.rewrite().of(x, snake)
            self._chk(self.lib.sat_conv1d_k7_planes(_ptr(x), _ptr(sa), _ptr(sib), _ptr(xp.hi), _ptr(xp.lo), b, cin, tin, xp.rows, st))
        elif xp is None:
            xp = self._k7_prepass(x, sa, sib, tout, pad, st)
        kept = xp if own is not None and xp.own is own and k == 7 and cout == cin else None
        y = self._conv_out(out, b, cout, tout, x.device)
        x2, a2, b2, pda, pdb = self._dsnake_args(dsnake, cout, prows, x.device)
        self._chk(self.lib.sat_conv1d_bf16x3_planesq(_ptr(xp.hi), _ptr(xp.lo), xp.rows, _ptr(w_planes[0]), _ptr(w_planes[1]), _ptr(bias), _ptr(res),
                                                     _ptr(y), _ptr(x2), _ptr(a2), _ptr(b2), _ptr(pda), _ptr(pdb), b, cin, cout, tin, tout,
                                                     k, dil, pad, int(tanh_out), {True: 0, False: 1, "force": 2}[self.k7q_persist] | (4 if self.k7q_dma_in_mfma else 0), st))
        y = self._dsnake_result(y, pda, pdb)
        return (y, kept) if keep_planes else y

    def convtr1d_bf16x3(self, x, w_planes, cout, k, stride, pad, tout=None, bias=None, snake=None, res=None,
                        tanh_out=False, dsnake=None, sconsts=None):
        b, cin, tin = x.shape
        if tout is None:
            tout = (tin - 1) * stride - 2 * pad + k
        rows = self.lib.sat_convtr1d_bf16x3_partial_rows(b, tout, stride, pad)
        return self._bf16x3_call(self.lib.sat_convtr1d_bf16x3, rows, x, w_planes, cout, tout, (k, stride, pad),
                                 bias, snake, res, tanh_out, dsnake, None, sconsts)

    def convtr1d(self, x, w_packed, cout, k, stride, pad, tout=None, bias=None, snake=None, res=None,
                 tanh_out=False, dsnake=None):
        b, cin, tin = x.shape
        if tout is None:
            tout = (tin - 1) * stride - 2 * pad + k
        alpha, beta = snake if snake is not None else (None, None)
        self._f32(x, w_packed, bias, alpha, beta, res)
        y = torch.empty(b, cout, tout, dtype=torch.float32, device=x.device)
        rows = self.lib.sat_convtr1d_partial_rows(b, tout, stride, pad) if dsnake is not None else 0
        if rows < 0:
            raise RuntimeError("sat_convtr1d: unsupported stride")
        x2, a2, b2, pda, pdb = self._dsnake_args(dsnake, cout, rows, x.device)
        self._chk(self.lib.sat_convtr1d(_ptr(x), _ptr(w_packed), _ptr(bias), _ptr(alpha), _ptr(beta), _ptr(res), _ptr(y),
                                        _ptr(x2), _ptr(a2), _ptr(b2), _ptr(pda), _ptr(pdb),
                                        b, cin, cout, tin, tout, k, stride, pad, int(tanh_out), self._stream(x)))
        return self._dsnake_result(y, pda, pdb)

    def conv_wgrad(self, lo, hi, k, stride=1, dil=1, pad=0, snake=None, snake_on=0, lo_rowsum=False, raw=False):
        bsz, m, tlo = lo.shape
        _, n, thi = hi.shape
        alpha, beta = snake if snake is not None else (None, None)
        self._f32(lo, hi, alpha, beta)
        x3 = self.use_bf16x3 and dil == 1 and self.lib.sat_conv_wgrad_bf16x3_nsplit(bsz, m, n, tlo, k, stride) > 0
        if x3:
            nsplit = self.lib.sat_conv_wgrad_bf16x3_nsplit(bsz, m, n, tlo, k, stride)
        else:
            nsplit = self.lib.sat_conv_wgrad_nsplit(bsz, m, n, tlo, k, stride, dil)
        if nsplit < 0:
            raise RuntimeError("sat_conv_wgrad: receptive field too large")
        partial = torch.empty(nsplit, m * n * k, dtype=torch.float32, device=lo.device)
        so_m, so_n, so_k = n * k, k, 1
        rs = None
        if x3:
            fused = lo_rowsum and not (snake is not None and snake_on == 1)
            rs = torch.empty(m, nsplit, dtype=torch.float32, device=lo.device) if fused else None
            self._chk(self.lib.sat_conv_wgrad_bf16x3(_ptr(lo), _ptr(hi), _ptr(alpha), _ptr(beta),
                                                     snake_on if snake is not None else 0, _ptr(partial), so_m, so_n, so_k,
                                                     bsz, m, n, tlo, thi, k, stride, pad, _ptr(rs), self._stream(lo)))
        else:
            self._chk(self.lib.sat_conv_wgrad(_ptr(lo), _ptr(hi), _ptr(alpha), _ptr(beta), snake_on if snake is not None else 0,
                                              _ptr(partial), so_m, so_n, so_k, bsz, m, n, tlo, thi, k, stride, dil, pad,
                                              self._stream(lo)))
        return self._wgrad_result(WgradSlabs(partial, nsplit, (m, n, k), (so_m, so_n, so_k)), raw, lo, lo_rowsum, rs)

    ru_k1_fused = True

    def ru_k1_bwd_ok(self, b, c, t):
        return self.ru_k1_fused and self.use_bf16x3 and self.lib.sat_ru_k1_bwd_nsplit(b, c, t) > 0

    def ru_k1_pack(self, w2):
        self._f32(w2)
        c = w2.shape[0]
        planes = torch.empty(2, c * c, dtype=torch.int16, device=w2.device)
        self._chk(self.lib.sat_ru_k1_pack(_ptr(w2), _ptr(planes[0]), _ptr(planes[1]), c, self._stream(w2)))
        return planes[0], planes[1]

    def ru_k1_bwd(self, dy, h, w2, snake2, emit=False, wt=None, raw=False, skip_dh=False):
        b, c, t = dy.shape
        a2, b2 = snake2
        self._f32(dy, h, w2, a2, b2)
        ns = self.lib.sat_ru_k1_bwd_nsplit(b, c, t)
        if ns <= 0:
            raise RuntimeError("ru_k1_bwd: shape not served by the fused kernel (ru_k1_bwd_ok)")
        st = self._stream(dy)
        wt_hi, wt_lo = wt if wt is not None else self.ru_k1_pack(w2)
        dh = torch.empty_like(dy)
        slabs = torch.empty(ns, c * c, dtype=torch.float32, device=dy.device)
        part = torch.empty(4 * c, ns, dtype=torch.float32, device=dy.device)
        if emit not in (None, False, True) or (skip_dh and not emit):
            raise ValueError("ru_k1_bwd: emit is True or nothing (dh has no activation), and skip_dh needs emit=True")
        ep = self._emit_planes(b, c, t, dy.device, st) if emit else self._NO_PLANES
        self._dh_unwritten = dh.data_ptr() if skip_dh else None
        self._chk(self.lib.sat_ru_k1_bwd(_ptr(dy), _ptr(h), _ptr(wt_hi), _ptr(wt_lo), _ptr(a2), _ptr(b2), None if skip_dh else _ptr(dh),
                                         _ptr(ep.hi), _ptr(ep.lo), ep.rows, _ptr(slabs), _ptr(part), b, c, t, st))
        self._emit_done(emit, dh, ep)
        if skip_dh and self._emitted is None:
            raise RuntimeError("ru_k1_bwd: dh was skipped but its planes cannot be tracked")
        dw2 = WgradSlabs(slabs, ns, (c, c, 1), (c, 1, 1))
        if not raw:
            dw2 = dw2.reduce(self)
        sums = self._sum_last(part)
        return dh, sums[:c], sums[c:2 * c], dw2, sums[3 * c:], sums[2 * c:3 * c]

    def wgrad7_bf16x3_ok(self, n_in, k, stride, dil):
        return self.use_bf16x3 and stride == 1 and k == 7 and dil in (1, 3, 9)

    def conv_wgrad7_bf16x3(self, dy, x, dil, pad, snake=None, dy_rowsum=False, raw=False):
        b, m, t = dy.shape
        n = x.shape[1]
        alpha, beta = snake if snake is not None else (None, None)
        self._f32(dy, x, alpha, beta)
        self._check_written(dy)
        nsplit = self.lib.sat_conv_wgrad7_bf16x3_nsplit(b, m, n, t)
        partial = torch.empty(nsplit, m * n * 7, dtype=torch.float32, device=dy.device)
        fused = dy_rowsum and self.lib.sat_conv_wgrad7_bf16x3_fuses_rowsum(b, m, n, t) == 1
        rs = torch.empty(m, nsplit, dtype=torch.float32, device=dy.device) if fused else None
        self._chk(self.lib.sat_conv_wgrad7_bf16x3(_ptr(dy), _ptr(x), _ptr(alpha), _ptr(beta), _ptr(partial), n, 1, m * n,
                                                  b, m, n, t, dil, pad, _ptr(rs), self._stream(dy)))
        return self._wgrad_result(WgradSlabs(partial, nsplit, (m, n, 7), (n, 1, m * n)), raw, dy, dy_rowsum, rs)

    def conv_wgrad7_planes_ok(self, b, m, n, t, dil, pad, rows_dy, rows_act):
        return self.use_bf16x3 and self.wgrad7_planes and self.lib.sat_conv_wgrad7_planes_ok(b, m, n, t, dil, pad, rows_dy, rows_act) == 1

    def conv_wgrad7_planes(self, dy_planes, act_planes, b, m, n, t, dil, pad, raw=False):
        dhi, dlo, drows = dy_planes
        ahi, alo, arows = act_planes
        if self.lib.sat_conv_wgrad7_planes_ok(b, m, n, t, dil, pad, drows, arows) != 1:
            raise RuntimeError("conv_wgrad7_planes: shape not served by the planes kernel (conv_wgrad7_planes_ok)")
        nsplit = self.lib.sat_conv_wgrad7_planes_nsplit(b, m, n, t)
        partial = torch.empty(nsplit, m * n * 7, dtype=torch.float32, device=dhi.device)
        self._chk(self.lib.sat_conv_wgrad7_planes(_ptr(dhi), _ptr(dlo), drows, _ptr(ahi), _ptr(alo), arows, _ptr(partial), n, 1, m * n,
                                                  b, m, n, t, dil, pad, self._stream(dhi)))
        slabs = WgradSlabs(partial, nsplit, (m, n, 7), (n, 1, m * n))
        return slabs if raw else slabs.reduce(self)

    def rowsum(self, x, partial=False):
        self._f32(x)
        self._check_written(x)
        b, c, t = x.shape
        while True:
            ns = self.lib.sat_rowsum_nsplit(t)
            part = torch.empty(c, ns, dtype=torch.float32, device=x.device)
            self._chk(self.lib.sat_rowsum(_ptr(x), _ptr(part), b, c, t, self._stream(x)))
            if partial:
                return part
            if ns == 1:
                return part.view(c)
            x, b, t = part, 1, ns

    def sum_all(self, x):
        x = x.contiguous()
        if x.dtype != torch.float32:
            x = x.float()
        n = x.numel()
        if n == 0:
            return torch.zeros((), dtype=torch.float32, device=x.device)
        if n > 1 << 29:
            flat = x.view(-1)
            return torch.stack([self.sum_all(piece) for piece in flat.split(1 << 29)]).sum()
        if x.data_ptr() % 16:
            x = x.clone()
        return self.rowsum(x.view(1, 1, n)).view(())

    def vae_sample_fwd(self, pre, noise):
        self._f32(pre, noise)
        b, c2, t = pre.shape
        c = c2 // 2
        z = torch.empty(b, c, t, dtype=torch.float32, device=pre.device)
        nb = self.lib.sat_vae_nblocks(b * c * t)
        klp = torch.empty(nb, dtype=torch.float32, device=pre.device)
        self._chk(self.lib.sat_vae_sample_fwd(_ptr(pre), _ptr(noise), _ptr(z), _ptr(klp), b, c, t, self._stream(pre)))
        kl = (self._sum_last(klp.view(1, nb)) * (1.0 / (b * t))).view(())
        return z, kl

    def vae_sample_bwd(self, pre, noise, dz, dkl):
        self._f32(pre, noise, dz, dkl)
        b, c2, t = pre.shape
        c = c2 // 2
        dpre = torch.empty_like(pre)
        self._chk(self.lib.sat_vae_sample_bwd(_ptr(pre), _ptr(noise), _ptr(dz), _ptr(dkl), _ptr(dpre), b, c, t,
                                              self._stream(pre)))
        return dpre

    def fir(self, x, taps, adjoint=False):
        self._f32(x, taps)
        n, t = x.shape
        y = torch.empty_like(x)
        self._chk(self.lib.sat_fir(_ptr(x), _ptr(taps), _ptr(y), n, t, taps.numel(), int(adjoint), self._stream(x)))
        return y

    def stft_sums(self, x, y, views, n_fft, hop):
        self._f32(x, y, views)
        ni, c, t = x.shape
        nv = views.shape[0]
        tiles = self.lib.sat_stft_tiles(n_fft, hop, t)
        if tiles < 0:
            raise RuntimeError(f"sat_stft: unsupported n_fft={n_fft} hop={hop} T={t}")
        partial = torch.empty(ni * nv * 3, tiles, dtype=torch.float32, device=x.device)
        self._chk(self.lib.sat_stft_fwd(_ptr(x), _ptr(y), _ptr(views), _ptr(partial), ni, c, t, nv, n_fft, hop, self._stream(x)))
        return self._sum_last(partial).view(ni, nv, 3)

    def stft_backward(self, x, y, views, coef, planes, n_fft, hop, wrt_x=False):
        self._f32(x, y, views, coef, planes)
        ni, c, t = x.shape
        nv = views.shape[0]
        if tuple(planes.shape) != (4, ni, c, t):
            raise ValueError("stft_backward: planes must be (4, NI, C, T)")
        self._chk(self.lib.sat_stft_bwd(_ptr(x), _ptr(y), _ptr(views), _ptr(coef), _ptr(planes), ni, c, t, nv, n_fft, hop,
                                        int(wrt_x), self._stream(x)))

    def rows_pack(self, x, kh, dil_t, pad_t, pad_w, pitch, lead):
        self._f32(x)
        b, c, t, w = x.shape
        buf = torch.empty(2 * lead + b * c * kh * t * pitch, dtype=torch.float32, device=x.device)
        self._chk(self.lib.sat_rows_pack(_ptr(x), _ptr(buf), b, c, t, w, kh, dil_t, pad_t, pad_w, pitch, lead, self._stream(x)))
        return buf

    def rows_pack_bwd(self, dbuf, shape, kh, dil_t, pad_t, pad_w, pitch, lead):
        self._f32(dbuf)
        b, c, t, w = shape
        dx = torch.empty(shape, dtype=torch.float32, device=dbuf.device)
        self._chk(self.lib.sat_rows_pack_bwd(_ptr(dbuf), _ptr(dx), b, c, t, w, kh, dil_t, pad_t, pad_w, pitch, lead, self._stream(dbuf)))
        return dx

    def release_workspaces(self):
        for d in (self._planes, self._own_planes, self._disc_pool, self._disc_gen, self._disc_geoms):
            d.clear()
        self._emitted = None
        self._disc_emitted = None

    def disc_geom(self, frames, w):
        key = ("disc_geom", frames, w)
        cache = self._disc_geoms
        g = cache.get(key)
        if g is None:
            out = [ctypes.c_int() for _ in range(4)]
            self._chk(self.lib.sat_disc_geom(frames, w, *[ctypes.byref(o) for o in out]))
            g = cache[key] = tuple(o.value for o in out)
        return g

    def _disc_plane_buf(self, b, c, frames, w, device, slot):
        P, L, lead, rows = self.disc_geom(frames, w)
        c8 = (c + 7) // 8
        n = b * c8 * rows * 8
        key = (device, 0 if c8 == 1 else 1, slot)
        self._disc_gen[key] = self._disc_gen.get(key, 0) + 1
        pool = self._disc_pool
        e = pool.get(key)
        if e is None or e["cap"] < n:
            e = pool[key] = {"hi": _keep_zeros(n, torch.int16, device), "lo": _keep_zeros(n, torch.int16, device),
                             "cap": n, "geom": (b, c8, frames, w)}
        elif e["geom"] != (b, c8, frames, w):
            for t in (e["hi"], e["lo"]):
                v = t[:n].view(b * c8, rows, 8)
                v[:, :lead].zero_()
                v[:, lead + L:].zero_()
            e["geom"] = (b, c8, frames, w)
        return e["hi"][:n], e["lo"][:n]

    def disc_register(self, t, planes, c, frames, w, slot):
        key = (t.device, 0 if (c + 7) // 8 == 1 else 1, slot)
        if not _caches.trackable(t):
            self._disc_emitted = None
            return
        self._disc_emitted = {"ptr": t.data_ptr(), "ver": _caches.version_of(t), "key": key, "gen": self._disc_gen.get(key, 0),
                              "geom": (t.shape[0], (c + 7) // 8, frames, w), "planes": planes, "slot": slot}

    def disc_take(self, h, c, frames, w):
        e = self._disc_emitted
        self._disc_emitted = None
        if (e is not None and e["ptr"] == h.data_ptr() and _caches.trackable(h) and e["ver"] == _caches.version_of(h) and e["geom"] == (h.shape[0], (c + 7) // 8, frames, w)
                and self._disc_gen.get(e["key"], 0) == e["gen"]):
            return e["planes"], e["slot"]
        return self.disc_planes(h, frames, w, slot=0)[1], 0

    def disc_planes(self, src, frames, w, out=None, slope=1.0, want_dst=False, want_planes=True, slot=0, fm_sign=None, fm_coef=None):
        self._f32(src, out, fm_coef)
        if fm_sign is not None and (fm_sign.dtype != torch.int8 or not fm_sign.is_contiguous() or fm_sign.numel() != src.numel()):
            raise ValueError("disc_planes: fm_sign must be a contiguous int8 tensor of src's size")
        b, c = src.shape[0], src.shape[1]
        P, L, lead, rows = self.disc_geom(frames, w)
        pitched = src.dim() == 3
        if pitched and src.shape[2] != L or not pitched and tuple(src.shape[2:]) != (frames, w):
            raise ValueError("disc_planes: shape does not match (frames, w)")
        dst = torch.empty(b, c, L, dtype=torch.float32, device=src.device) if want_dst else None
        pl = self._disc_plane_buf(b, c, frames, w, src.device, slot) if want_planes else None
        self._chk(self.lib.sat_disc_planes(_ptr(src), _ptr(out), _ptr(fm_sign), _ptr(fm_coef), _ptr(dst), _ptr(pl[0]) if pl else None,
                                           _ptr(pl[1]) if pl else None, b, c, frames, w, 1 if pitched else 0, float(slope), self._stream(src)))
        return dst, pl

    def disc_l1_sum(self, a, b, want_sign=False):
        self._f32(a, b)
        partial = torch.empty(self.lib.sat_disc_l1_blocks(), dtype=torch.float32, device=a.device)
        sign = torch.empty(a.shape, dtype=torch.int8, device=a.device) if want_sign else None
        self._chk(self.lib.sat_disc_l1_sum(_ptr(a), _ptr(b), _ptr(partial), _ptr(sign), a.numel(), self._stream(a)))
        return (partial.sum(), sign) if want_sign else partial.sum()

    def disc_pack(self, w4, mode):
        self._f32(w4)
        cout, cin, kh, kw = w4.shape
        n = self.lib.sat_disc_pack_size(cout, cin, kh, kw, mode)
        if n < 0:
            raise ValueError("disc_pack: unsupported kernel shape")
        wq = torch.empty(n, dtype=torch.int16, device=w4.device)
        self._chk(self.lib.sat_disc_pack_weights(_ptr(w4), _ptr(wq), cout, cin, kh, kw, mode, self._stream(w4)))
        return wq

    def disc_conv(self, planes, wq, bias, b, cin, cout, frames, w, kh, kw, dil_t, slope, emit_slot=None, lk_src=None, lk_slope=1.0):
        self._f32(bias, lk_src)
        L = self.disc_geom(frames, w)[1]
        y = torch.empty(b, cout, L, dtype=torch.float32, device=planes[0].device)
        em = self._disc_plane_buf(b, cout, frames, w, y.device, emit_slot) if emit_slot is not None else None
        self._chk(self.lib.sat_disc_conv(_ptr(planes[0]), _ptr(planes[1]), _ptr(wq), _ptr(bias), _ptr(y),
                                         _ptr(em[0]) if em else None, _ptr(em[1]) if em else None, b, cin, cout, frames, w, kh, kw, dil_t,
                                         float(slope), _ptr(lk_src), float(lk_slope), self._stream(y)))
        return y, em

    def disc_wgrad(self, dy, x, frames, w, kh, kw, dil_t):
        self._f32(dy, x)
        b, m, _ = dy.shape
        cin = x.shape[1]
        nsplit = self.lib.sat_disc_wgrad_nsplit(b, m, cin, kh, frames, w)
        mp, npad = (m + 63) // 64 * 64, (kh * cin + 63) // 64 * 64
        partial = torch.empty(nsplit, kw * mp * npad, dtype=torch.float32, device=dy.device)
        self._chk(self.lib.sat_disc_wgrad(_ptr(dy), _ptr(x), _ptr(partial), b, m, cin, frames, w, kh, kw, dil_t, self._stream(dy)))
        dw = self._reduce_rows(partial, nsplit, kw * mp * npad).view(kw, mp, npad)[:, :m, :kh * cin]
        return dw.reshape(kw, m, kh, cin).permute(1, 3, 2, 0).contiguous()

    def rows_unpack(self, y, t, w, pad_w, pitch, slope):
        self._f32(y)
        b, c = y.shape[0], y.shape[1]
        out = torch.empty(b, c, t, w, dtype=torch.float32, device=y.device)
        self._chk(self.lib.sat_rows_unpack(_ptr(y), _ptr(out), b, c, t, w, pad_w, pitch, float(slope), self._stream(y)))
        return out

    def rows_unpack_bwd(self, dout, out, pad_w, pitch, slope):
        self._f32(dout, out)
        b, c, t, w = dout.shape
        dy = torch.empty(b, c, t * pitch, dtype=torch.float32, device=dout.device)
        self._chk(self.lib.sat_rows_unpack_bwd(_ptr(dout), _ptr(out), _ptr(dy), b, c, t, w, pad_w, pitch, float(slope), self._stream(dout)))
        return dy

    def spec_fwd(self, x, n_fft, hop):
        self._f32(x)
        ni, c, t = x.shape
        frames = self.lib.sat_spec_frames(n_fft, hop, t)
        if frames < 0:
            raise RuntimeError(f"sat_spec: unsupported n_fft={n_fft} hop={hop} T={t}")
        z = torch.empty(ni, 2 * c, frames, n_fft // 2 + 1, dtype=torch.float32, device=x.device)
        self._chk(self.lib.sat_spec_fwd(_ptr(x), _ptr(z), ni, c, t, n_fft, hop, self._stream(x)))
        return z

    def spec_bwd(self, dz, c, t, n_fft, hop):
        self._f32(dz)
        ni = dz.shape[0]
        planes = torch.zeros(2, ni, c, t, dtype=torch.float32, device=dz.device)
        self._chk(self.lib.sat_spec_bwd(_ptr(dz), _ptr(planes), ni, c, t, n_fft, hop, self._stream(dz)))
        return planes[0] + planes[1]

    def _dt(self, *tensors):
        dt = None
        for t in tensors:
            if t is None:
                continue
            if t.dtype not in (torch.float32, torch.bfloat16):
                raise TypeError(f"DiT kernels take float32 or bfloat16 tensors, got {t.dtype}")
# ... 598 lines not shown
```

Measured before the change: 8.195.

## Fuse bias-grad row sums into dgrad epilogue and wgrad loads; skip dh store

Adds a dgrad entry point for the bf16x3 conv that also reduces per-channel row sums of the data gradient in its backward snake epilogue. It can skip the fp32 y store when only bf16 planes are consumed. Adds a wgrad variant that accumulates row sums of the 'hi' operand while staging it, so the bias gradient no longer needs separate rowsum passes. The cost is extra register and LDS pressure and more complex bookkeeping for unwritten tensors.

```diff
diff --git a/include/sat_amd.h b/include/sat_amd.h
--- a/include/sat_amd.h
+++ b/include/sat_amd.h
@@ -25,6 +25,11 @@
                       const float* beta2, float* part_da, float* part_db, int B, int Cin, int Cout, int Tin, int Tout,
                       int K, int stride, int dil, int pad, int tanh_out, void* em_hi, void* em_lo,
                            const float* em_a, const float* em_ib, int em_rows, void* stream);
+int sat_conv1d_bf16x3_dgrad(const float* x, const short* w_hi, const short* w_lo, const float* bias, const float* snake_a,
+                            const float* snake_ib, const float* res, float* y, const float* x2, const float* alpha2,
+                            const float* beta2, float* part_da, float* part_db, int B, int Cin, int Cout, int Tin, int Tout,
+                            int K, int stride, int dil, int pad, int tanh_out, void* em_hi, void* em_lo,
+                            const float* em_a, const float* em_ib, int em_rows, float* part_rs, void* stream);
 int sat_residual_unit_fwd(const short* xp_hi, const short* xp_lo, int rows, const short* w7_hi, const short* w7_lo,
                           const float* bias1, const float* a2, const float* ib2, const short* w1_hi, const short* w1_lo,
                           const float* bias2, const float* x, float* h, float* y, int B, int C, int T, int K, int dil, int pad,
@@ -98,6 +103,9 @@
 int sat_conv_wgrad_bf16x3(const float* lo, const float* hi, const float* alpha, const float* beta, int snake_on,
                           float* partial, long long so_m, long long so_n, long long so_k, int B, int M, int N, int Tlo,
                           int Thi, int K, int stride, int pad, float* lo_rowsum, void* stream);
+int sat_conv_wgrad_bf16x3_rs(const float* lo, const float* hi, const float* alpha, const float* beta, int snake_on,
+                             float* partial, long long so_m, long long so_n, long long so_k, int B, int M, int N, int Tlo,
+                             int Thi, int K, int stride, int pad, float* lo_rowsum, float* hi_rowsum, void* stream);
 int sat_conv_wgrad_bf16x3_nsplit(int B, int M, int N, int Tlo, int K, int stride);
 
 int sat_ru_k1_bwd_nsplit(int B, int C, int T);
diff --git a/stable_audio_tools_amd/_lib.py b/stable_audio_tools_amd/_lib.py
--- a/stable_audio_tools_amd/_lib.py
+++ b/stable_audio_tools_amd/_lib.py
@@ -14,6 +14,7 @@
     "sat_conv1d_partial_rows": (_I, [_I, _I]),
     "sat_conv1d_bf16x3": (_I, [_P] * 13 + [_I] * 10 + [_P]),
     "sat_conv1d_bf16x3_emit": (_I, [_P] * 13 + [_I] * 10 + [_P] * 4 + [_I, _P]),
+    "sat_conv1d_bf16x3_dgrad": (_I, [_P] * 13 + [_I] * 10 + [_P] * 4 + [_I, _P, _P]),
     "sat_convtr1d_bf16x3": (_I, [_P] * 13 + [_I] * 9 + [_P]),
     "sat_conv1d_bf16x3_partial_rows": (_I, [_I] * 4),
     "sat_rows_pack": (_I, [_P, _P] + [_I] * 10 + [_P]),
@@ -47,6 +48,7 @@
     "sat_conv_wgrad7_planes": (_I, [_P, _P, _I, _P, _P, _I, _P] + [_L] * 3 + [_I] * 6 + [_P]),
     "sat_lds_read_tr16_probe": (_I, [_P] * 4),
     "sat_conv_wgrad_bf16x3": (_I, [_P] * 4 + [_I, _P] + [_L] * 3 + [_I] * 8 + [_P, _P]),
+    "sat_conv_wgrad_bf16x3_rs": (_I, [_P] * 4 + [_I, _P] + [_L] * 3 + [_I] * 8 + [_P, _P, _P]),
     "sat_conv_wgrad_bf16x3_nsplit": (_I, [_I] * 6),
     "sat_convtr1d": (_I, [_P] * 12 + [_I] * 9 + [_P]),
     "sat_convtr1d_partial_rows": (_I, [_I, _I, _I, _I]),
diff --git a/stable_audio_tools_amd/csrc/conv1d_bf16x3.hip b/stable_audio_tools_amd/csrc/conv1d_bf16x3.hip
--- a/stable_audio_tools_amd/csrc/conv1d_bf16x3.hip
+++ b/stable_audio_tools_amd/csrc/conv1d_bf16x3.hip
@@ -27,6 +27,7 @@
     const float* em_a = nullptr;
     const float* em_ib = nullptr;
     int em_rows = 0, em_c8 = 0;
+    float* part_rs = nullptr;
     const short* ru_w1_hi = nullptr;
     const short* ru_w1_lo = nullptr;
     const float* ru_bias2 = nullptr;
@@ -58,7 +59,7 @@
     __shared__ __attribute__((aligned(16))) char lds_pool[POOL];
     short (*w_lds)[SAT_CO_T][KROW] = reinterpret_cast<short (*)[SAT_CO_T][KROW]>(lds_pool);
     short (*a_lds)[CS][AROWS][8] = reinterpret_cast<short (*)[CS][AROWS][8]>(lds_pool + W_BYTES);
-    __shared__ float red_lds[2][2][SAT_CO_T];
+    __shared__ float red_lds[3][2][SAT_CO_T];
     __shared__ float ep_lds[5][SAT_CO_T];
     constexpr int SN_MAX = (NG == 4) ? 1024 : 2048;
     __shared__ float sn_lds[2][SN_MAX];
@@ -285,8 +286,9 @@
     }
 
     const bool bwd = (p.x2 != nullptr);
+    const bool want_rs = bwd && a.part_rs != nullptr;
     if (bwd) {
-        for (int i = tid; i < 2 * 2 * SAT_CO_T; i += 256) (&red_lds[0][0][0])[i] = 0.0f;
+        for (int i = tid; i < 3 * 2 * SAT_CO_T; i += 256) (&red_lds[0][0][0])[i] = 0.0f;
         __syncthreads();
     }
     const bool vec4 = so == 0 && a.out_shift == 0 && (p.Tout & 3) == 0 &&
@@ -336,7 +338,7 @@
                     const f32x4 av = *reinterpret_cast<const f32x4*>(&tile[row][t4]);
                     const float bias = ep_lds[0][col];
                     const float a2 = ep_lds[1][col], b2 = ep_lds[2][col];
-                    float pda = 0.f, pdb = 0.f;
+                    float pda = 0.f, pdb = 0.f, prs = 0.f;
                     f32x4 ov;
 #pragma unroll
                     for (int e = 0; e < 4; ++e) {
@@ -346,12 +348,13 @@
                             pda += v * g.dla;
                             pdb += v * g.dlb;
                             v *= g.dx;
+                            prs += v;
                         }
                         v += rv[j][e];
                         if (p.tanh_out) v = tanhf(v);
                         ov[e] = v;
                     }
-                    if (ok) *reinterpret_cast<f32x4*>(p.y + ((size_t)b * p.Cout + co) * p.Tout + tg) = ov;
+                    if (ok && p.y) *reinterpret_cast<f32x4*>(p.y + ((size_t)b * p.Cout + co) * p.Tout + tg) = ov;
                     if (a.em_hi) {
                         f32x4 ev = ov;
                         if (a.em_a) {
@@ -372,6 +375,12 @@
                         if ((lane & 15) == 0) {
                             red_lds[0][wave & 1][col] = pda;
                             red_lds[1][wave & 1][col] = pdb;
+                        }
+                        if (want_rs) {
+                            if (!ok) prs = 0.f;
+#pragma unroll
+                            for (int m = 8; m >= 1; m >>= 1) prs += __shfl_xor(prs, m);
+                            if ((lane & 15) == 0) red_lds[2][wave & 1][col] = prs;
                         }
                     }
                 }
@@ -500,7 +509,7 @@
                 const int co = m >> so;
                 const float bias = ep_lds[0][col];
                 const float a2 = ep_lds[1][col], b2 = ep_lds[2][col];
-                float pda = 0.f, pdb = 0.f;
+                float pda = 0.f, pdb = 0.f, prs = 0.f;
 #pragma unroll
                 for (int ni = 0; ni < 2; ++ni) {
                     const int q = t0 + t_w + ni * 32 + l31;
@@ -512,6 +521,7 @@
                         pda += ok ? v * g.dla : 0.0f;
                         pdb += ok ? v * g.dlb : 0.0f;
                         v *= g.dx;
+                        prs += ok ? v : 0.0f;
                     }
                     v += rv[r][ni];
                     if (p.tanh_out) v = tanhf(v);
@@ -524,6 +534,10 @@
                         red_lds[0][wave & 1][col] = pda;
                         red_lds[1][wave & 1][col] = pdb;
                     }
+                    if (want_rs) {
+                        prs = sat_half_sum(prs);
+                        if (l31 == 0) red_lds[2][wave & 1][col] = prs;
+                    }
                 }
             }
         }
@@ -532,15 +546,17 @@
         __syncthreads();
         const int m = co0 + tid;
         if (tid < SAT_CO_T && (tid & smask_o) == 0 && m < a.cout_v) {
-            float sa = 0.f, sb = 0.f;
+            float sa = 0.f, sb = 0.f, sr = 0.f;
             for (int r = 0; r <= smask_o; ++r) {
                 sa += red_lds[0][0][tid + r] + red_lds[0][1][tid + r];
                 sb += red_lds[1][0][tid + r] + red_lds[1][1][tid + r];
+                sr += red_lds[2][0][tid + r] + red_lds[2][1][tid + r];
             }
             const size_t row = (size_t)b * gridDim.x + t_tile;
             const size_t nrows_p = (size_t)p.B * gridDim.x;
             p.part_da[(size_t)(m >> so) * nrows_p + row] = sa;
             p.part_db[(size_t)(m >> so) * nrows_p + row] = sb;
+            if (want_rs) a.part_rs[(size_t)(m >> so) * nrows_p + row] = sr;
         }
     }
 }
@@ -660,7 +676,7 @@
                                   const float* x2, const float* alpha2, const float* beta2, float* part_da,
                                   float* part_db, int B, int Cin, int Cout, int Tin, int Tout, int K, int stride, int dil,
                                   int pad, int tanh_out, short* em_hi, short* em_lo, const float* em_a, const float* em_ib, int em_rows,
-                                  void* stream) {
+                                  float* part_rs, void* stream) {
     if (B <= 0 || Cin <= 0 || Cout <= 0 || Tin <= 0 || Tout <= 0) { sat_set_error("sat_conv1d_bf16x3: empty shape"); return 1; }
     SatBfPlan pl;
     if (!sat_bf_plan(K, stride, 0, &pl) || dil < 1 || (stride > 1 && dil != 1)) {
@@ -670,9 +686,12 @@
     if ((pl.kv - 1) * dil > (pl.cs == 1 ? 62 : SAT_BF_AROWSN - SAT_T_T)) { sat_set_error("sat_conv1d_bf16x3: receptive field too large for the LDS slab"); return 1; }
     if ((snake_a == nullptr) != (snake_ib == nullptr)) { sat_set_error("sat_conv1d_bf16x3: snake constants must both be given"); return 1; }
     if (x2 && (!alpha2 || !beta2 || !part_da || !part_db)) { sat_set_error("sat_conv1d_bf16x3: backward epilogue needs alpha2/beta2/partials"); return 1; }
+    if (part_rs && (!x2 || (pl.ng == 8 && pl.cs == 1))) { sat_set_error("sat_conv1d_bf16x3_dgrad: the row sums belong to the backward epilogue of the K <= 4 / strided plans"); return 1; }
+    if (!y && !em_hi) { sat_set_error("sat_conv1d_bf16x3: y missing (only a launch that emits planes may skip the fp32 store)"); return 1; }
     SatConvBfLaunch a;
     a.p = SatConvParams{x, nullptr, bias, snake_a, snake_ib, res, y, x2, alpha2, beta2, part_da, part_db,
                         B, Cin, Cout, Tin, Tout, pl.kv, 1, dil, stride == 1 ? pad : 0, tanh_out};
+    a.part_rs = part_rs;
     a.w_hi = w_hi;
     a.w_lo = w_lo;
     a.cout_v = Cout;
@@ -701,7 +720,7 @@
                                  float* part_db, int B, int Cin, int Cout, int Tin, int Tout, int K, int stride, int dil,
                                  int pad, int tanh_out, void* stream) {
     return sat_conv1d_bf16x3_impl("sat_conv1d_bf16x3", x, w_hi, w_lo, bias, snake_a, snake_ib, res, y, x2, alpha2, beta2, part_da, part_db,
-                                  B, Cin, Cout, Tin, Tout, K, stride, dil, pad, tanh_out, nullptr, nullptr, nullptr, nullptr, 0, stream);
+                                  B, Cin, Cout, Tin, Tout, K, stride, dil, pad, tanh_out, nullptr, nullptr, nullptr, nullptr, 0, nullptr, stream);
 }
 extern "C" int sat_conv1d_bf16x3_emit(const float* x, const short* w_hi, const short* w_lo, const float* bias,
                                       const float* snake_a, const float* snake_ib, const float* res, float* y,
@@ -710,8 +729,19 @@
                                       int pad, int tanh_out, void* em_hi, void* em_lo, const float* em_a, const float* em_ib, int em_rows,
                                       void* stream) {
     if (!em_hi) { sat_set_error("sat_conv1d_bf16x3_emit: planes missing"); return 1; }
+    if (!y) { sat_set_error("sat_conv1d_bf16x3_emit: y missing"); return 1; }
     return sat_conv1d_bf16x3_impl("sat_conv1d_bf16x3_emit", x, w_hi, w_lo, bias, snake_a, snake_ib, res, y, x2, alpha2, beta2, part_da, part_db,
-                                  B, Cin, Cout, Tin, Tout, K, stride, dil, pad, tanh_out, (short*)em_hi, (short*)em_lo, em_a, em_ib, em_rows, stream);
+                                  B, Cin, Cout, Tin, Tout, K, stride, dil, pad, tanh_out, (short*)em_hi, (short*)em_lo, em_a, em_ib, em_rows, nullptr, stream);
+}
+extern "C" int sat_conv1d_bf16x3_dgrad(const float* x, const short* w_hi, const short* w_lo, const float* bias,
+                                       const float* snake_a, const float* snake_ib, const float* res, float* y,
+                                       const float* x2, const float* alpha2, const float* beta2, float* part_da,
+                                       float* part_db, int B, int Cin, int Cout, int Tin, int Tout, int K, int stride, int dil,
+                                       int pad, int tanh_out, void* em_hi, void* em_lo, const float* em_a, const float* em_ib, int em_rows,
+                                       float* part_rs, void* stream) {
+    if (!x2) { sat_set_error("sat_conv1d_bf16x3_dgrad: x2 missing (a forward conv takes sat_conv1d_bf16x3 / _emit)"); return 1; }
+    return sat_conv1d_bf16x3_impl("sat_conv1d_bf16x3_dgrad", x, w_hi, w_lo, bias, snake_a, snake_ib, res, y, x2, alpha2, beta2, part_da, part_db,
+                                  B, Cin, Cout, Tin, Tout, K, stride, dil, pad, tanh_out, (short*)em_hi, (short*)em_lo, em_a, em_ib, em_rows, part_rs, stream);
 }
 
 extern "C" int sat_conv1d_k7_plane_rows(int Tin, int Tout, int pad) {
diff --git a/stable_audio_tools_amd/csrc/conv_wgrad_bf16x3.hip b/stable_audio_tools_amd/csrc/conv_wgrad_bf16x3.hip
--- a/stable_audio_tools_amd/csrc/conv_wgrad_bf16x3.hip
+++ b/stable_audio_tools_amd/csrc/conv_wgrad_bf16x3.hip
@@ -350,6 +350,7 @@
     int chunks_per_split, nchunks, nT;
     float* rowsum;
     int nsplit;
+    float* hi_rowsum;
 };
 
 template <int NT>
@@ -387,6 +388,9 @@
 
     const bool want_rs = p.rowsum != nullptr && v0 == 0;
     float rsum[8] = {0.f, 0.f, 0.f, 0.f, 0.f, 0.f, 0.f, 0.f};
+    const bool want_hrs = (NT == 2) && p.hi_rowsum != nullptr && m0 == 0;
+    float* const hs_lds = reinterpret_cast<float*>(&hi_lds[0][0][0]);
+    int hs_per = 0;
 
     if (tid < SAT_CO_T) {
         float sa = 1.f, sib = 0.f;
@@ -515,6 +519,7 @@
         const unsigned magic = 0xffffffffu / (unsigned)qpc + 1u;
         const int total_q = nc * qpc;
         const int qcl = sl >= 2 ? sl - 2 : 0, qc = 1 << qcl;
+        float hs8 = 0.f;
         auto load_quads = [&](int tv, const float* shi, int th0, bool interior, f4u* vq, auto ib, auto ie) {
             constexpr int IB = decltype(ib)::value, IE = decltype(ie)::value;
 #pragma unroll
@@ -541,7 +546,7 @@
                 vq[i - IB] = v;
             }
         };
-        auto store_quads = [&](int tv, const f4u* vq, auto ib, auto ie) {
+        auto store_quads = [&](int tv, const f4u* vq, bool last_stage, auto ib, auto ie) {
             constexpr int IB = decltype(ib)::value, IE = decltype(ie)::value;
 #pragma unroll
             for (int i = IB; i < IE; ++i) {
@@ -549,6 +554,7 @@
                 if (i == NQ - 1 && Q >= total_q) break;
                 const int cl = (int)sat_umulhi((unsigned)Q, magic), q = Q - cl * qpc;
                 f4u o = vq[i - IB];
+                if (want_hrs && (last_stage || q < (16 << sl))) (i < 8 ? rsum[i & 7] : hs8) += (o[0] + o[1]) + (o[2] + o[3]);
                 if (snake_hi) {
                     const float sa = sn_a[cl], sib = sn_ib[cl];
 #pragma unroll
@@ -624,7 +630,7 @@
                 }
             }
             SAT_SCHED_FENCE();
-            store_quads(tv, vq, I0{}, IN{});
+            store_quads(tv, vq, ch - b * p.nT == p.nT - 1, I0{}, IN{});
             SAT_SCHED_FENCE();
 #pragma unroll
             for (int u = 0; u < 8; ++u) {
@@ -649,7 +655,17 @@
             mfma_stage();
             __syncthreads();
         }
-    } else
+        if (want_hrs) {
+            hs_per = qpc;
+#pragma unroll
+            for (int i = 0; i < NQ; ++i)
+                if (tid + 256 * i < total_q) hs_lds[tid + 256 * i] = i < 8 ? rsum[i & 7] : hs8;
+        }
+    } else {
+    constexpr int NHP = (NT == 2) ? 24 : 8;
+    float hsx[NHP - 7];
+#pragma unroll
+    for (int i = 0; i < NHP - 7; ++i) hsx[i] = 0.f;
     for (int ch = c_begin; ch < c_end; ++ch) {
         const int b = ch / p.nT;
         const int tt0 = (ch - b * p.nT) * SAT_WS_TT;
@@ -701,7 +717,8 @@
         {
             const float* src = p.hi + (size_t)b * p.N * p.Thi;
             const int th0 = (tt0 << sl) - p.pad;
-            for (int base = tid; base < total_units; base += 8 * 256) {
+            int round = 0;
+            for (int base = tid; base < total_units; base += 8 * 256, ++round) {
                 float v[8][2];
 #pragma unroll
                 for (int u = 0; u < 8; ++u) {
@@ -719,6 +736,14 @@
                     if (idx < total_units) {
                         const int cl = idx / up, uu = (idx - cl * up) * 2;
                         float o0 = v[u][0], o1 = v[u][1];
+                        if constexpr (NT == 2) {
+                            if (want_hrs && (tt0 + SAT_WS_TT >= p.nT * SAT_WS_TT || uu < (SAT_WS_TT << sl))) {
+                                const float s2 = o0 + o1;
+                                if (round == 0) rsum[u] += s2;
+                                else if (round == 1) hsx[u] += s2;
+                                else hsx[8 + u] += s2;
+                            }
+                        }
                         if (snake_hi) {
                             const float sa = sn_a[cl], sib = sn_ib[cl];
                             o0 = sat_snake(o0, sa, sib);
@@ -744,12 +769,32 @@
         mfma_stage();
         __syncthreads();
     }
+    if constexpr (NT == 2) {
+        if (want_hrs) {
+            hs_per = up;
+#pragma unroll
+            for (int i = 0; i < NHP; ++i)
+                if (tid + 256 * i < total_units) hs_lds[tid + 256 * i] = i < 8 ? rsum[i & 7] : hsx[(i - 8) & 15];
+        }
+    }
+    }
 
     if (want_rs && (tid & 15) == 0) {
 #pragma unroll
         for (int i = 0; i < 8; ++i) {
             const int m = m0 + (tid >> 4) + 16 * i;
             if (m < p.M) p.rowsum[(size_t)m * p.nsplit + split] = rsum[i];
+        }
+    }
+    if constexpr (NT == 2) {
+        if (want_hrs) {
+            __syncthreads();
+            for (int chn = wave; chn < nc; chn += 4) {
+                float s = 0.f;
+                for (int j = lane; j < hs_per; j += 64) s += hs_lds[chn * hs_per + j];
+                s = sat_wave_sum(s);
+                if (lane == 0 && n_base + chn < p.N) p.hi_rowsum[(size_t)(n_base + chn) * p.nsplit + split] = s;
+            }
         }
     }
     if (wave_on) {
@@ -797,9 +842,17 @@
     int sl, nt;
     return sat_wgs_plan(B, M, N, Tlo, K, stride, &pl, &sl, &nt) ? pl.nsplit : -1;
 }
+extern "C" int sat_conv_wgrad_bf16x3_rs(const float* lo, const float* hi, const float* alpha, const float* beta, int snake_on,
+                                        float* partial, long long so_m, long long so_n, long long so_k, int B, int M, int N,
+                                        int Tlo, int Thi, int K, int stride, int pad, float* lo_rowsum, float* hi_rowsum, void* stream);
 extern "C" int sat_conv_wgrad_bf16x3(const float* lo, const float* hi, const float* alpha, const float* beta, int snake_on,
                                      float* partial, long long so_m, long long so_n, long long so_k, int B, int M, int N,
                                      int Tlo, int Thi, int K, int stride, int pad, float* lo_rowsum, void* stream) {
+    return sat_conv_wgrad_bf16x3_rs(lo, hi, alpha, beta, snake_on, partial, so_m, so_n, so_k, B, M, N, Tlo, Thi, K, stride, pad, lo_rowsum, nullptr, stream);
+}
+extern "C" int sat_conv_wgrad_bf16x3_rs(const float* lo, const float* hi, const float* alpha, const float* beta, int snake_on,
+                                        float* partial, long long so_m, long long so_n, long long so_k, int B, int M, int N,
+                                        int Tlo, int Thi, int K, int stride, int pad, float* lo_rowsum, float* hi_rowsum, void* stream) {
     SatWgBfPlan pl;
     int sl, nt;
     if (!sat_wgs_plan(B, M, N, Tlo, K, stride, &pl, &sl, &nt)) {
@@ -809,8 +862,13 @@
     if (Thi <= 0 || pad < 0) { sat_set_error("sat_conv_wgrad_bf16x3: bad shape"); return 1; }
     if (alpha && (snake_on != 1 && snake_on != 2)) { sat_set_error("sat_conv_wgrad_bf16x3: snake_on must be 1 (lo) or 2 (hi)"); return 1; }
     if ((alpha == nullptr) != (beta == nullptr)) { sat_set_error("sat_conv_wgrad_bf16x3: alpha/beta must both be given"); return 1; }
+    if (hi_rowsum && lo_rowsum) { sat_set_error("sat_conv_wgrad_bf16x3_rs: row sums of lo or of hi, not both in one launch"); return 1; }
+    if (hi_rowsum && (nt != 2 || Thi > ((pl.nT * SAT_WS_TT + 1) << sl) - pad)) {
+        sat_set_error("sat_conv_wgrad_bf16x3_rs: hi_rowsum needs K == 2*stride and Thi <= (64 * ceil(Tlo / 64) + 1) * stride - pad");
+        return 1;
+    }
     SatWgSmallParams p{lo, hi, alpha, beta, partial, (long long)M * N * K, so_m, so_n, so_k,
-                       B, M, N, Tlo, Thi, pad, alpha ? snake_on : 0, sl, pl.cps, pl.nchunks, pl.nT, lo_rowsum, pl.nsplit};
+                       B, M, N, Tlo, Thi, pad, alpha ? snake_on : 0, sl, pl.cps, pl.nchunks, pl.nT, lo_rowsum, pl.nsplit, hi_rowsum};
     dim3 grid(sat_cdiv(M, SAT_CO_T), sat_cdiv(N << sl, SAT_CO_T), pl.nsplit);
     if (nt == 1) SAT_LAUNCH(sat_wgrad_small_bf16x3_kernel<1>, grid, dim3(256), stream, p);
     else SAT_LAUNCH(sat_wgrad_small_bf16x3_kernel<2>, grid, dim3(256), stream, p);
diff --git a/stable_audio_tools_amd/functional.py b/stable_audio_tools_amd/functional.py
--- a/stable_audio_tools_amd/functional.py
+++ b/stable_audio_tools_amd/functional.py
@@ -68,7 +68,14 @@
         return dv, dg.view(ctx.g_shape), None
 
 
-def _conv_dgrad(ops, dy, w, k, stride, dil, pad, cin, tin, dsnake, res=None, out=None, emit=None):
+def _conv_dgrad(ops, dy, w, k, stride, dil, pad, cin, tin, dsnake, res=None, out=None, emit=None, y_rowsum=None, skip_y=False):
+    if y_rowsum or skip_y:
+        if stride == 1 and dsnake is not None and ops.bf16x3_ok(k, 1, dil) and k <= 4 and (emit or not ops.edge_ok(w.shape[0], cin, k, 1, dil, (k - 1) * dil - pad)):
+            return ops.conv1d_bf16x3(dy, ops.pack_bf16x3(w, mode=1), cin, k, 1, dil, (k - 1) * dil - pad, tout=tin, dsnake=dsnake, res=res, out=out,
+                                     emit=emit, y_rowsum=y_rowsum, skip_y=skip_y)
+        if skip_y:
+            raise ValueError("_conv_dgrad(skip_y=True): only the K <= 4 bf16x3 data-gradient can leave its fp32 result unwritten")
+        return (*_conv_dgrad(ops, dy, w, k, stride, dil, pad, cin, tin, dsnake, res=res, out=out, emit=emit), None)
     if stride == 1:
         if (res is None and out is None and not emit and ops.edge_ok(w.shape[0], cin, k, 1, dil, (k - 1) * dil - pad) and tin == dy.shape[2]
                 and (dsnake is None or w.shape[0] <= 2)):
@@ -222,9 +229,10 @@
         cin, cout, k = w.shape
         dy = dy.contiguous()
         snake = (alpha, beta) if has_snake else None
-        dbias = ops.rowsum(dy) if has_bias else None
-        dw = ops.conv_wgrad(x, dy, k, stride, 1, pad, snake=snake, snake_on=1, raw=bool(wn))
-        dg = None
+        dw = ops.conv_wgrad(x, dy, k, stride, 1, pad, snake=snake, snake_on=1, raw=bool(wn), hi_rowsum=has_bias)
+        dbias = dg = None
+        if has_bias:
+            dw, dbias = dw
         if wn:
             dw, dg = _wn_backward(ops, dw, wn, ctx.g_shape)
         dx = da = db = None
@@ -302,13 +310,30 @@
             if dw is None:
                 return _conv_wgrad(ops, dh, x, k1, 1, dil, pad1, (a1, b1), bias_grad=bias_grad, raw=bool(wn1))
             return (dw, ops.rowsum(dh, partial=bool(wn1))) if bias_grad else dw
+
+        def dgrad1(dh):
+            return _conv_dgrad(ops, dh, w1, k1, 1, dil, pad1, c, t, (x, a1, b1), res=dy)
         if k2 == 1 and w2.shape[0] == c and w1.shape[0] == c and ops.ru_k1_bwd_ok(dy.shape[0], c, t):
             skip_dh = bool(kept is not None and ops.ru_k1_bwd_skip_dh)
             dh, da2, db2, dw2, dbias2, dbias1 = ops.ru_k1_bwd(dy, h, w2, (a2, b2), emit=want_emit, raw=bool(wn2), skip_dh=skip_dh)
             try:
                 dw1 = wgrad1(dh, False)
                 if skip_dh:
-                    dx, da1, db1 = _conv_dgrad(ops, dh, w1, k1, 1, dil, pad1, c, t, (x, a1, b1), res=dy)
+                    dx, da1, db1 = dgrad1(dh)
+            finally:
+                ops.dh_written()
+        elif ops.k1_dgrad_rowsum:
+            dw2, dbias2 = ops.conv_wgrad(dy, h, k2, 1, 1, 0, snake=(a2, b2), snake_on=2, lo_rowsum=True, raw=bool(wn2))
+            skip_dh = bool(kept is not None and ops.k1_dgrad_skip_dh)
+            dh, da2, db2, dbias1 = _conv_dgrad(ops, dy, w2, k2, 1, 1, 0, c, t, (h, a2, b2), emit=want_emit,
+                                               y_rowsum="partial" if wn1 else True, skip_y=skip_dh)
+            try:
+                if dbias1 is None:
+                    dw1, dbias1 = wgrad1(dh, True)
+                else:
+                    dw1 = wgrad1(dh, False)
+                if skip_dh:
+                    dx, da1, db1 = dgrad1(dh)
             finally:
                 ops.dh_written()
         else:
@@ -327,7 +352,7 @@
             else:
                 dw2, dg2 = _wn_backward(ops, dw2, wn2, gs2)
         if not skip_dh:
-            dx, da1, db1 = _conv_dgrad(ops, dh, w1, k1, 1, dil, pad1, c, t, (x, a1, b1), res=dy)
+            dx, da1, db1 = dgrad1(dh)
         return dx, da1, db1, dw1, dbias1, da2, db2, dw2, dbias2, None, None, None, None, None, None, dg1, dg2
 
 
diff --git a/stable_audio_tools_amd/ops.py b/stable_audio_tools_amd/ops.py
--- a/stable_audio_tools_amd/ops.py
+++ b/stable_audio_tools_amd/ops.py
@@ -171,22 +171,29 @@
 
     def _sum_pair(self, pda, pdb):
         c, r = pda.shape
-        both = self.rowsum(pda._base.view(1, 2 * c, r) if pda._base is not None else torch.stack([pda, pdb]).view(1, 2 * c, r))
+        base = pda._base[:2] if pda._base is not None else torch.stack([pda, pdb])
+        both = self.rowsum(base.view(1, 2 * c, r))
         return both[:c], both[c:]
 
     def _sum_last(self, partial):
         c, r = partial.shape
         return self.rowsum(partial.view(1, c, r))
 
-    def _dsnake_args(self, dsnake, cout, rows, device):
+    def _dsnake_args(self, dsnake, cout, rows, device, rowsum=False):
         if dsnake is None:
             return None, None, None, None, None
         x2, a2, b2 = dsnake
         self._f32(x2, a2, b2)
-        return (x2, a2, b2, *torch.empty(2, cout, rows, dtype=torch.float32, device=device).unbind(0))
-
-    def _dsnake_result(self, y, pda, pdb):
-        return y if pda is None else (y, *self._sum_pair(pda, pdb))
+        return (x2, a2, b2, *torch.empty(3 if rowsum else 2, cout, rows, dtype=torch.float32, device=device).unbind(0))
+
+    def _dsnake_result(self, y, pda, pdb, prs=None, partial=False):
+        if pda is None:
+            return y
+        if prs is None or partial:
+            return (y, *self._sum_pair(pda, pdb)) + (() if prs is None else (prs,))
+        c, r = pda.shape
+        sums = self.rowsum(pda._base.view(1, 3 * c, r))
+        return y, sums[:c], sums[c:2 * c], sums[2 * c:]
 
     def conv1d(self, x, w_packed, cout, k, stride=1, dil=1, pad=0, tout=None, bias=None, snake=None, res=None,
                tanh_out=False, dsnake=None, out=None):
@@ -296,24 +303,33 @@
         self._f32(out)
         return out
 
-    def _bf16x3_call(self, fn, rows, x, w_planes, cout, tout, dims, bias, snake, res, tanh_out, dsnake, out=None, sconsts=None, emit=None):
+    def _bf16x3_call(self, fn, rows, x, w_planes, cout, tout, dims, bias, snake, res, tanh_out, dsnake, out=None, sconsts=None, emit=None,
+                     y_rowsum=None, skip_y=False):
         b, cin, tin = x.shape
         self._f32(x, bias, res)
+        if (y_rowsum or skip_y) and (dsnake is None or fn is not self.lib.sat_conv1d_bf16x3 or (skip_y and not emit)):
+            raise ValueError("y_rowsum / skip_y belong to a conv1d_bf16x3 data-gradient (dsnake=...), and skip_y needs emit")
         sa = sib = None
         if snake is not None:
             sa, sib = sconsts if sconsts is not None else self.snake_consts(snake[0], snake[1])
         y = self._conv_out(out, b, cout, tout, x.device)
-        x2, a2, b2, pda, pdb = self._dsnake_args(dsnake, cout, rows, x.device)
+        x2, a2, b2, pda, pdb, *prs = self._dsnake_args(dsnake, cout, rows, x.device, rowsum=bool(y_rowsum))
+        prs = prs[0] if prs else None
         ep, ea, eib = self._emit_args(emit, b, cout, tout, x.device, self._stream(x))
         args = (_ptr(x), _ptr(w_planes[0]), _ptr(w_planes[1]), _ptr(bias), _ptr(sa), _ptr(sib),
-                _ptr(res), _ptr(y), _ptr(x2), _ptr(a2), _ptr(b2), _ptr(pda), _ptr(pdb),
+                _ptr(res), None if skip_y else _ptr(y), _ptr(x2), _ptr(a2), _ptr(b2), _ptr(pda), _ptr(pdb),
                 b, cin, cout, tin, tout, *dims, int(tanh_out))
-        if emit:
+        if y_rowsum or skip_y:
+            self._dh_unwritten = y.data_ptr() if skip_y else None
+            self._chk(self.lib.sat_conv1d_bf16x3_dgrad(*args, _ptr(ep.hi), _ptr(ep.lo), _ptr(ea), _ptr(eib), ep.rows, _ptr(prs), self._stream(x)))
+        elif emit:
             self._chk(self.lib.sat_conv1d_bf16x3_emit(*args, _ptr(ep.hi), _ptr(ep.lo), _ptr(ea), _ptr(eib), ep.rows, self._stream(x)))
         else:
             self._chk(fn(*args, self._stream(x)))
         self._emit_done(emit, y, ep)
-        return self._dsnake_result(y, pda, pdb)
+        if skip_y and self._emitted is None:
+            raise RuntimeError("conv1d_bf16x3: y was skipped but its planes cannot be tracked")
+        return self._dsnake_result(y, pda, pdb, prs, partial=y_rowsum == "partial")
 
     ru_fused = True
 
@@ -355,7 +371,10 @@
     k7_emit = True
     wgrad7_planes = True
     wgrad7_planes_budget_gib = 16.0
+    wgrad_hi_rowsum = True
     ru_k1_bwd_skip_dh = True
+    k1_dgrad_rowsum = True
+    k1_dgrad_skip_dh = True
 
     def emit_ok(self, cout, k, stride, tout, consumer_dil):
         if not (self.k7_emit and self.use_bf16x3 and self.k7q_applicable(cout, 7, 1, consumer_dil, 3 * consumer_dil, cout)):
@@ -437,13 +456,13 @@
 
     def _check_written(self, t):
         if t is not None and self._dh_unwritten is not None and t.data_ptr() == self._dh_unwritten:
-            raise RuntimeError("this tensor is a dh that sat_ru_k1_bwd did not write (skip_dh): only its planes exist")
+            raise RuntimeError("this tensor is a dh that its kernel did not write (skip_dh): only its planes exist")
 
     def dh_written(self):
         self._dh_unwritten = None
 
     def conv1d_bf16x3(self, x, w_planes, cout, k, stride=1, dil=1, pad=0, tout=None, bias=None, snake=None, res=None,
-                      tanh_out=False, dsnake=None, out=None, sconsts=None, emit=None, keep_planes=False):
+                      tanh_out=False, dsnake=None, out=None, sconsts=None, emit=None, keep_planes=False, y_rowsum=None, skip_y=False):
         b, cin, tin = x.shape
         if tout is None:
             tout = (tin + 2 * pad - dil * (k - 1) - 1) // stride + 1
@@ -451,9 +470,11 @@
         if len(w_planes) == 3:
             if not (stride == 1 and 5 <= k <= 7 and 0 <= pad <= 32 and (k - 1) * dil <= 62):
                 raise ValueError("conv1d_bf16x3: q-packed weights need stride 1, 5 <= K <= 7, pad <= 32, (K-1)*dil <= 62")
+            if y_rowsum or skip_y:
+                raise ValueError("conv1d_bf16x3: y_rowsum / skip_y are not served by the k7 kernels")
             return self._k7_planes_call(rows, x, w_planes, cout, tout, k, dil, pad, bias, snake, res, tanh_out, dsnake, out, sconsts, keep_planes)
         y = self._bf16x3_call(self.lib.sat_conv1d_bf16x3, rows, x, w_planes, cout, tout, (k, stride, dil, pad),
-                              bias, snake, res, tanh_out, dsnake, out, sconsts, emit)
+                              bias, snake, res, tanh_out, dsnake, out, sconsts, emit, y_rowsum, skip_y)
         return (y, None) if keep_planes else y
 
     def _k7_planes_call(self, prows, x, w_planes, cout, tout, k, dil, pad, bias, snake, res, tanh_out, dsnake, out=None, sconsts=None,
@@ -508,7 +529,7 @@
                                         b, cin, cout, tin, tout, k, stride, pad, int(tanh_out), self._stream(x)))
         return self._dsnake_result(y, pda, pdb)
 
-    def conv_wgrad(self, lo, hi, k, stride=1, dil=1, pad=0, snake=None, snake_on=0, lo_rowsum=False, raw=False):
+    def conv_wgrad(self, lo, hi, k, stride=1, dil=1, pad=0, snake=None, snake_on=0, lo_rowsum=False, raw=False, hi_rowsum=False):
         bsz, m, tlo = lo.shape
         _, n, thi = hi.shape
         alpha, beta = snake if snake is not None else (None, None)
@@ -522,18 +543,28 @@
             raise RuntimeError("sat_conv_wgrad: receptive field too large")
         partial = torch.empty(nsplit, m * n * k, dtype=torch.float32, device=lo.device)
         so_m, so_n, so_k = n * k, k, 1
-        rs = None
+        rs = hrs = None
         if x3:
             fused = lo_rowsum and not (snake is not None and snake_on == 1)
             rs = torch.empty(m, nsplit, dtype=torch.float32, device=lo.device) if fused else None
-            self._chk(self.lib.sat_conv_wgrad_bf16x3(_ptr(lo), _ptr(hi), _ptr(alpha), _ptr(beta),
-                                                     snake_on if snake is not None else 0, _ptr(partial), so_m, so_n, so_k,
-                                                     bsz, m, n, tlo, thi, k, stride, pad, _ptr(rs), self._stream(lo)))
+            fused_hi = (hi_rowsum and self.wgrad_hi_rowsum and not fused and stride >= 2 and k == 2 * stride and not (snake is not None and snake_on == 2)
+                        and thi <= (64 * ((tlo + 63) // 64) + 1) * stride - pad)
+            args = (_ptr(lo), _ptr(hi), _ptr(alpha), _ptr(beta), snake_on if snake is not None else 0, _ptr(partial), so_m, so_n, so_k,
+                    bsz, m, n, tlo, thi, k, stride, pad, _ptr(rs))
+            if fused_hi:
+                hrs = torch.empty(n, nsplit, dtype=torch.float32, device=lo.device)
+                self._chk(self.lib.sat_conv_wgrad_bf16x3_rs(*args, _ptr(hrs), self._stream(lo)))
+            else:
+                self._chk(self.lib.sat_conv_wgrad_bf16x3(*args, self._stream(lo)))
         else:
             self._chk(self.lib.sat_conv_wgrad(_ptr(lo), _ptr(hi), _ptr(alpha), _ptr(beta), snake_on if snake is not None else 0,
                                               _ptr(partial), so_m, so_n, so_k, bsz, m, n, tlo, thi, k, stride, dil, pad,
                                               self._stream(lo)))
-        return self._wgrad_result(WgradSlabs(partial, nsplit, (m, n, k), (so_m, so_n, so_k)), raw, lo, lo_rowsum, rs)
+        out = self._wgrad_result(WgradSlabs(partial, nsplit, (m, n, k), (so_m, so_n, so_k)), raw, lo, lo_rowsum, rs)
+        if not hi_rowsum:
+            return out
+        hsum = self._sum_last(hrs) if hrs is not None else self.rowsum(hi)
+        return (*out, hsum) if lo_rowsum else (out, hsum)
 
     ru_k1_fused = True
 
```

Result: no change. 8.235, median of 6 (+0.5%).
